# Circuitscape/Circuitscape.jl

Measured on NVIDIA H100. Metric: pair_solves_per_sec, higher is better.
Workload: dtype f64

## Files before the change

circuitscape_b200/_lib.py:

```python
from __future__ import annotations

import ctypes as C
import os

import numpy as np

_HERE = os.path.dirname(os.path.abspath(__file__))
LIB_PATH = os.path.join(_HERE, "lib", "libcsb200.so")

OK, ERR_ARG, ERR_CUDA, ERR_RESIDUAL, ERR_MAXITER, ERR_UNSUPPORTED = 0, -1, -2, -3, -4, -5
F32, F64 = 0, 1
PRECOND_JACOBI, PRECOND_AMG = 0, 1


class B200Unavailable(RuntimeError):
    pass


class B200Error(RuntimeError):
    def __init__(self, code, msg):
        super().__init__(msg)
        self.code = code


class Opts(C.Structure):
    _fields_ = [("precond", C.c_int32), ("panel_width", C.c_int32), ("check_every", C.c_int32),
                ("use_graph", C.c_int32), ("atol", C.c_double), ("resid_gate", C.c_double),
                ("log_transform", C.c_int32), ("window", C.c_int32), ("mixed", C.c_int32), ("setup", C.c_int32),
                ("stencil", C.c_int32), ("reserved", C.c_int32 * 3)]


class Stats(C.Structure):
    _fields_ = [("setup_ms", C.c_double), ("solve_ms", C.c_double), ("kernel_ms", C.c_double),
                ("iterations", C.c_int64), ("spmm_launches", C.c_int64),
                ("kernel_launches", C.c_int64), ("h2d_bytes", C.c_double), ("d2h_bytes", C.c_double)]

    def as_dict(self):
        return {k: getattr(self, k) for k, _ in self._fields_}


_H = C.c_void_p
_PROTOS = {
    "cs_b200_version": (C.c_int, []),
    "cs_b200_last_error": (C.c_char_p, [_H]),
    "cs_b200_create": (C.c_int, [C.c_int64, C.c_int64, C.c_void_p, C.c_void_p, C.c_void_p, C.c_int,
                                 C.c_int, C.c_int, C.c_int, C.POINTER(Opts), C.POINTER(_H)]),
    "cs_b200_create_from_device": (C.c_int, [C.c_int64, C.c_int64, C.c_void_p, C.c_void_p, C.c_void_p,
                                             C.c_int, C.c_int, C.POINTER(Opts), C.POINTER(_H)]),
    "cs_b200_create_from_raster": (C.c_int, [C.c_int64, C.c_int64, C.c_void_p, C.c_int, C.c_int, C.c_int, C.c_int,
                                             C.POINTER(Opts), C.POINTER(_H), C.POINTER(C.c_int64),
                                             C.POINTER(C.c_int64)]),
    "cs_b200_get_csr": (C.c_int, [_H, C.c_void_p, C.c_void_p, C.c_void_p]),
    "cs_b200_set_grounds": (C.c_int, [_H, C.c_void_p, C.c_void_p]),
    "cs_b200_level_info": (C.c_int, [_H, C.c_int, C.c_int, C.POINTER(C.c_int64), C.POINTER(C.c_int64),
                                     C.POINTER(C.c_int64), C.POINTER(C.c_double), C.POINTER(C.c_int)]),
    "cs_b200_level_csr": (C.c_int, [_H, C.c_int, C.c_int, C.c_void_p, C.c_void_p, C.c_void_p]),
    "cs_b200_level_stencil": (C.c_int, [_H, C.c_int, C.POINTER(C.c_int)]),
    "cs_b200_create_from_raster_poly": (C.c_int, [C.c_int64, C.c_int64, C.c_void_p, C.c_void_p, C.c_int, C.c_int, C.c_int,
                                                  C.c_int, C.POINTER(Opts), C.POINTER(_H), C.POINTER(C.c_int64),
                                                  C.POINTER(C.c_int64), C.c_void_p]),
    "cs_b200_get_dims": (C.c_int, [_H, C.POINTER(C.c_int64), C.POINTER(C.c_int64)]),
    "cs_b200_destroy": (None, [_H]),
    "cs_b200_spmv": (C.c_int, [_H, C.c_void_p, C.c_void_p, C.c_int, C.POINTER(C.c_double)]),
    "cs_b200_spmm": (C.c_int, [_H, C.c_int, C.c_void_p, C.c_void_p]),
    "cs_b200_apply_precond": (C.c_int, [_H, C.c_int, C.c_void_p, C.c_void_p, C.c_void_p]),
    "cs_b200_bench_spmm": (C.c_int, [_H, C.c_int, C.c_int, C.c_int, C.POINTER(C.c_double)]),
    "cs_b200_bench_cg_iter": (C.c_int, [_H, C.c_int, C.c_int, C.POINTER(C.c_double)]),
    "cs_b200_solve_rhs": (C.c_int, [_H, C.c_int64, C.c_void_p, C.c_void_p, C.c_double, C.c_int64,
                                    C.c_void_p, C.c_void_p]),
    "cs_b200_solve_pairs": (C.c_int, [_H, C.c_int64, C.c_void_p, C.c_void_p, C.c_void_p, C.c_double,
                                      C.c_int64, C.c_void_p, C.c_void_p, C.c_void_p, C.c_int,
                                      C.c_void_p, C.c_void_p]),
    "cs_b200_solve_pairs_superposed": (C.c_int, [_H, C.c_int64, C.c_void_p, C.c_int64, C.c_void_p, C.c_void_p,
                                                 C.c_void_p, C.c_double, C.c_int64, C.c_void_p, C.c_void_p,
                                                 C.c_void_p, C.c_int, C.c_void_p, C.c_void_p]),
    "cs_b200_solve_region_pairs": (C.c_int, [_H, C.c_int64, C.c_void_p, C.c_void_p, C.c_int64, C.c_void_p,
                                             C.c_void_p, C.c_void_p, C.c_double, C.c_int64, C.c_void_p,
                                             C.c_void_p, C.c_void_p, C.c_int, C.c_void_p, C.c_void_p]),
    "cs_b200_solve_grounded": (C.c_int, [_H, C.c_int64, C.c_void_p, C.c_void_p, C.c_int64, C.c_void_p,
                                         C.c_void_p, C.c_void_p, C.c_void_p, C.c_void_p, C.c_double,
                                         C.c_int64, C.c_void_p, C.c_void_p, C.c_void_p, C.c_int, C.c_void_p,
                                         C.c_void_p]),
    "cs_b200_solve_advanced": (C.c_int, [_H, C.c_int64, C.c_void_p, C.c_void_p, C.c_int64, C.c_void_p,
                                         C.c_void_p, C.c_void_p, C.c_void_p, C.c_void_p, C.c_double,
                                         C.c_int64, C.c_void_p, C.c_void_p, C.c_int, C.c_void_p, C.c_void_p]),
    "cs_b200_solve_sources": (C.c_int, [_H, C.c_int64, C.c_void_p, C.c_void_p, C.c_void_p, C.c_void_p,
                                        C.c_void_p, C.c_double, C.c_int64, C.c_int64, C.c_void_p,
                                        C.c_void_p, C.c_void_p, C.c_void_p, C.c_int, C.c_void_p,
                                        C.c_void_p]),
    "cs_b200_solve_advanced_batch": (C.c_int, [C.c_int64, C.c_int64, C.c_int64, C.c_void_p, C.c_void_p,
                                               C.c_void_p, C.c_int, C.c_int, C.c_int, C.c_double, C.c_int64,
                                               C.c_void_p, C.c_void_p, C.c_void_p, C.c_void_p,
                                               C.POINTER(C.c_int64)]),
    "cs_b200_solve_advanced_network": (C.c_int, [_H, C.c_int64, C.c_void_p, C.c_void_p, C.c_int64, C.c_void_p,
                                                 C.c_void_p, C.c_void_p, C.c_void_p, C.c_void_p, C.c_double,
                                                 C.c_int64, C.c_void_p, C.c_void_p, C.c_void_p, C.c_void_p,
                                                 C.c_void_p]),
    "cs_b200_solve_pairs_branch": (C.c_int, [_H, C.c_int64, C.c_void_p, C.c_void_p, C.c_void_p, C.c_double,
                                             C.c_int64, C.c_void_p, C.c_void_p, C.c_void_p, C.c_int, C.c_void_p,
                                             C.c_void_p, C.c_void_p]),
    "cs_b200_branch_index": (C.c_int, [_H, C.POINTER(C.c_int64), C.c_void_p, C.c_void_p]),
    "cs_b200_read_branch_currents": (C.c_int, [_H, C.c_void_p]),
    "cs_b200_components": (C.c_int, [_H, C.POINTER(C.c_int64), C.c_void_p]),
    "cs_b200_read_currents": (C.c_int, [_H, C.c_void_p, C.c_void_p]),
    "cs_b200_reset_currents": (C.c_int, [_H]),
    "cs_b200_currents_device_ptrs": (C.c_int, [_H, C.POINTER(C.c_void_p), C.POINTER(C.c_void_p)]),
    "cs_b200_get_stats": (C.c_int, [_H, C.POINTER(Stats)]),
    "cs_b200_stream": (C.c_int, [_H, C.POINTER(C.c_void_p)]),
    "cs_b200_profile_spmm": (C.c_int, [_H, C.c_int, C.POINTER(C.c_double), C.POINTER(C.c_int64)]),
    "cs_b200_profile_classes": (C.c_int, [_H, C.c_void_p, C.c_void_p, C.c_void_p]),
    "cs_b200_profile_bytes": (C.c_int, [_H, C.POINTER(C.c_double)]),
    "cs_b200_comm_unique_id": (C.c_int, [C.c_void_p]),
    "cs_b200_comm_init": (C.c_int, [C.c_int, C.c_int, C.c_int, C.c_void_p, C.POINTER(_H)]),
    "cs_b200_comm_destroy": (None, [_H]),
    "cs_b200_comm_last_error": (C.c_char_p, [_H]),
    "cs_b200_create_bcast": (C.c_int, [_H, C.c_int, C.c_int64, C.c_int64, C.c_void_p, C.c_void_p, C.c_void_p,
                                       C.c_int, C.c_int, C.c_int, C.POINTER(Opts), C.POINTER(_H)]),
    "cs_b200_comm_reduce_currents": (C.c_int, [_H, _H]),
    "cs_b200_comm_gather_pairs": (C.c_int, [_H, C.c_int64, C.c_void_p, C.c_int64, C.c_void_p, C.c_void_p]),
    "cs_b200_comm_max_double": (C.c_int, [_H, C.c_void_p, C.c_int]),
    "cs_b200_comm_barrier": (C.c_int, [_H]),
}
EXPORTED_SYMBOLS = tuple(_PROTOS)

_lib = None


def load():
    global _lib
    if _lib is not None:
        return _lib
    if not os.path.isfile(LIB_PATH):
        raise B200Unavailable(
            f"{LIB_PATH} not built -- run `python -c 'import __graft_entry__ as g; g.build()'` "
            "(the CUDA path has no CPU fallback)")
    lib = C.CDLL(LIB_PATH)
    for name, (res, args) in _PROTOS.items():
        fn = getattr(lib, name)
        fn.restype = res
        fn.argtypes = args
    _lib = lib
    return lib


def _ptr(a):
    return None if a is None else a.ctypes.data_as(C.c_void_p)


def np_dtype(dtype_code):
    return np.float64 if dtype_code == F64 else np.float32


def dtype_code(dt):
    dt = np.dtype(dt)
    if dt == np.float64:
        return F64
    if dt == np.float32:
        return F32
    raise TypeError(f"unsupported dtype {dt}")


def check(lib, h, rc, allow=()):
    if rc == OK or rc in allow:
        return rc
    msg = lib.cs_b200_last_error(h)
    msg = msg.decode() if msg else f"libcsb200 error {rc}"
    if rc == ERR_CUDA and "no CUDA device" in msg:
        raise B200Unavailable(msg)
    raise B200Error(rc, msg)
```

circuitscape_b200/csrc/cs_b200.cu:

```cuda
#include "../../include/cs_b200.h"

#include <cuda_runtime.h>
#include <cub/device/device_scan.cuh>

#include <algorithm>
#include <chrono>
#include <cmath>
#include <cstdarg>
#include <cstdio>
#include <cstdlib>
#include <cstring>
#include <limits>
#include <string>
#include <type_traits>
#include <vector>

#include "amg_host.hpp"
#include "win_host.hpp"
#include "kernels.cuh"
#include "raster_assembly.cuh"
#include "setup_device.hpp"

using namespace csb;

namespace {

thread_local std::string g_create_error;

constexpr int PROF_CLASSES = 18;
constexpr int PROF_CGF = 8;

struct GraphSlot {
  cudaGraphExec_t exec = nullptr;
  int chunk = 0;
  int64_t kernels = 0, spmms = 0;
  cudaGraphExec_t loop_exec = nullptr;
  int64_t loop_kernels = 0, loop_spmms = 0;
};

}

struct DevCsr {
  int* rowptr = nullptr;
  int* colidx = nullptr;
  void* vals = nullptr;
  int* bstart = nullptr;
  int nblocks = 0;
  int nrows = 0;
  int64_t nnz = 0;
  int lpr = 1;
  WinMeta* win_meta = nullptr;
  unsigned char* blob = nullptr;
  int has_dinv = 0;
  int64_t win_blocks = 0;
  int win_nblocks = 0;
  void* dia = nullptr;
  size_t dia_ld = 0;
  int dia_nr = 0;
  int dia_half = 0;
  int* ell_col = nullptr;
  void* ell_val = nullptr;
  size_t ell_ld = 0;
};

struct DevLevel {
  int64_t n = 0, n_pad = 0;
  DevCsr A, P, R;
  void* dinv = nullptr;
  double omega = 2.0 / 3.0;
  void *x = nullptr, *b = nullptr, *t = nullptr, *y = nullptr;
};

struct cs_b200_handle {
  int device = 0;
  int dtype = CS_B200_F64;
  int64_t n = 0, n_pad = 0, nnz = 0;
  int* d_rowptr = nullptr;
  int* d_colidx = nullptr;
  void* d_vals = nullptr;
  bool owns_matrix = true;
  void* d_vals0 = nullptr;
  void* d_fg = nullptr;
  void* d_dinv = nullptr;
  int* d_bstart = nullptr;
  int nblocks = 0;
  int ktmax = 8;
  void *X = nullptr, *R = nullptr, *P = nullptr, *AP = nullptr, *B = nullptr, *stage = nullptr;
  void* Z = nullptr;
  void* P2 = nullptr;
  DevCsr A0;
  std::vector<DevLevel> lv;
  double* d_pinv = nullptr;
  double amg_opc = 0.0;
  bool amg = false;
  bool mixed = false;
  std::vector<DevLevel> lv32;
  void *R32 = nullptr, *X32 = nullptr, *T32 = nullptr, *Z32 = nullptr;
  void *d_cum = nullptr, *d_max = nullptr;
  int* d_bptr = nullptr;
  int64_t nb = 0;
  void* d_cum_branch = nullptr;
  void* d_branch_stage = nullptr;
  PanelCtl* d_ctl = nullptr;
  PanelCtl* h_ctl = nullptr;
  double* d_partials = nullptr;
  float* d_flush = nullptr;
  size_t flush_elems = 0;
  cudaStream_t stream = nullptr;
  cudaEvent_t ev0 = nullptr, ev1 = nullptr, ev2 = nullptr, ev3 = nullptr;
  long long* d_sp_rows = nullptr;
  double* d_sp_vals = nullptr;
  int* d_sp_ptr = nullptr;
  size_t sp_cap = 0;
  long long* d_probe = nullptr;
  void* d_probe_out = nullptr;
  size_t probe_cap = 0;
  cudaStream_t s_in = nullptr, s_out = nullptr;
  void* io_in[2] = {nullptr, nullptr};
  void* io_out[2] = {nullptr, nullptr};
  cudaEvent_t ev_in[2] = {nullptr, nullptr}, ev_used[2] = {nullptr, nullptr};
  cudaEvent_t ev_ready[2] = {nullptr, nullptr}, ev_out[2] = {nullptr, nullptr};
  int num_sms = 132;
  int grid_spmm = 132, grid_ew = 132;
  cs_b200_opts opts{};
  cs_b200_stats stats{};
  GraphSlot graphs[4];
  bool rg_on = false;
  int* d_rg_seg = nullptr;
  int* d_rg_rows = nullptr;
  size_t rg_cap = 0;
  GraphSlot rgraphs[4];
  int profile = 0;
  std::vector<cudaEvent_t> prof_ev;
  size_t prof_used = 0;
  double prof_ms = 0.0;
  double prof_bytes = 0.0;
  int64_t prof_launches = 0;
  std::vector<int> prof_slot;
  std::vector<double> prof_pair_bytes;
  double prof_slot_ms[PROF_CLASSES] = {}, prof_slot_bytes[PROF_CLASSES] = {};
  int64_t prof_slot_launches[PROF_CLASSES] = {};
  std::string err;
  size_t esize() const { return dtype == CS_B200_F64 ? 8 : 4; }
};

namespace {

struct Tick {
  bool on = std::getenv("CS_B200_VERBOSE") != nullptr;
  std::chrono::steady_clock::time_point t0 = std::chrono::steady_clock::now();
  void operator()(const char* what) {
    if (!on) return;
    const auto t1 = std::chrono::steady_clock::now();
    std::fprintf(stderr, "[cs_b200 setup] %-28s %8.1f ms\n", what,
                 std::chrono::duration<double, std::milli>(t1 - t0).count());
    t0 = t1;
  }
};

int set_err(cs_b200_handle* h, int code, const char* fmt, ...) {
  char buf[1024];
  va_list ap;
  va_start(ap, fmt);
  vsnprintf(buf, sizeof buf, fmt, ap);
  va_end(ap);
  if (h) h->err = buf; else g_create_error = buf;
  return code;
}

#define CK(h, call)                                                                      \
  do {                                                                                   \
    cudaError_t _e = (call);                                                             \
    if (_e != cudaSuccess)                                                               \
      return set_err(h, CS_B200_ERR_CUDA, "CUDA error %s at %s:%d (%s)",                 \
                     cudaGetErrorString(_e), __FILE__, __LINE__, #call);                 \
  } while (0)

cudaError_t h2d(cs_b200_handle* h, void* dst, const void* src, size_t bytes) {
  if (bytes == 0) return cudaSuccess;
  cudaError_t e = cudaMemcpyAsync(dst, src, bytes, cudaMemcpyHostToDevice, h->stream);
  if (e != cudaSuccess) return e;
  return cudaStreamSynchronize(h->stream);
}

int kt_index(int kt) { return kt == 1 ? 0 : kt == 2 ? 1 : kt == 4 ? 2 : 3; }

void build_row_blocks(const std::vector<int>& rowptr, int64_t n, std::vector<int>& bstart,
                      int max_rows = NT) {
  bstart.clear();
  bstart.push_back(0);
  int64_t r = 0;
  while (r < n) {
    int64_t r1 = r + 1;
    const int64_t base = rowptr[r];
    while (r1 < n && (r1 - r) < max_rows && (int64_t)rowptr[r1 + 1] - base <= NNZ_CAP) ++r1;
    bstart.push_back((int)r1);
    r = r1;
  }
}

template <typename T>
int build_windowed(cs_b200_handle* h, DevCsr& d, const int* rowptr, const int* colidx, int64_t ncols_pad,
                   const T* d_dinv = nullptr);

int win_mask() {
  const char* e = getenv("CS_B200_WIN_MASK");
  return e ? atoi(e) : 15;
}

template <typename T>
int upload_csr(cs_b200_handle* h, const csb_amg::Csr& m, DevCsr& d, bool windowed, const T* d_dinv = nullptr) {
  d.nrows = (int)m.nrows;
  d.nnz = m.nnz();
  d.lpr = (m.nrows > 0 && (double)d.nnz / (double)m.nrows >= 20.0) ? 4 : 1;
  const int unit = d.lpr == 4 ? 8 : 32;
  int max_rows = (int)((m.nrows + 4 * h->num_sms - 1) / (4 * h->num_sms));
  max_rows = std::min(NT, std::max(unit, (max_rows + unit - 1) / unit * unit));
  std::vector<int> bstart;
  build_row_blocks(m.ptr, m.nrows, bstart, max_rows);
  d.nblocks = (int)bstart.size() - 1;
  std::vector<T> v(m.val.begin(), m.val.end());
  CK(h, cudaMalloc(&d.rowptr, (size_t)(m.nrows + 1) * sizeof(int)));
  CK(h, cudaMalloc(&d.colidx, std::max<size_t>(1, (size_t)d.nnz) * sizeof(int)));
  CK(h, cudaMalloc(&d.vals, std::max<size_t>(1, (size_t)d.nnz) * sizeof(T)));
  CK(h, cudaMalloc(&d.bstart, bstart.size() * sizeof(int)));
  CK(h, h2d(h, d.rowptr, m.ptr.data(), (size_t)(m.nrows + 1) * sizeof(int)));
  CK(h, h2d(h, d.colidx, m.idx.data(), (size_t)d.nnz * sizeof(int)));
  CK(h, h2d(h, d.vals, v.data(), (size_t)d.nnz * sizeof(T)));
  CK(h, h2d(h, d.bstart, bstart.data(), bstart.size() * sizeof(int)));
  if (h->opts.window >= 0 && windowed) {
    const int64_t ncols_pad = (m.ncols + 3) / 4 * 4;
    return build_windowed<T>(h, d, m.ptr.data(), m.idx.data(), ncols_pad, d_dinv);
  }
  return CS_B200_OK;
}

void free_win(DevCsr& d) {
  cudaFree(d.win_meta); cudaFree(d.blob); cudaFree(d.dia); cudaFree(d.ell_col); cudaFree(d.ell_val);
  d.win_meta = nullptr; d.blob = nullptr; d.dia = nullptr; d.ell_col = nullptr; d.ell_val = nullptr;
  d.dia_half = 0;
}

// ... 95 lines not shown
  tick("host hierarchy");
  h->amg_opc = hier.operator_complexity();
  const int nl = (int)hier.levels.size();
  h->mixed = nl > 1 && sizeof(T) == 8 && h->opts.mixed >= 0;
  int rc = h->mixed ? upload_levels<float>(h, hier, h->lv32, true) : CS_B200_OK;
  if (rc) return rc;
  tick("levels: windows + upload");
  if (h->mixed) {
    h->lv.resize(nl);
    for (int l = 0; l < nl; ++l) { h->lv[l].n = hier.levels[l].A.nrows; h->lv[l].omega = hier.levels[l].omega; }
    h->lv[0].A = h->A0;
    h->lv[0].dinv = h->d_dinv;
    const size_t pe = (size_t)h->n_pad * h->ktmax * sizeof(float);
    void** bufs[] = {&h->R32, &h->X32, &h->T32, &h->Z32};
    for (void** bp : bufs) {
      CK(h, cudaMalloc(bp, pe));
      CK(h, cudaMemsetAsync(*bp, 0, pe, h->stream));
    }
  } else {
    rc = upload_levels<T>(h, hier, h->lv, false);
    if (rc) return rc;
    const size_t pe = (size_t)h->n_pad * h->ktmax * sizeof(T);
    CK(h, cudaMalloc(&h->Z, pe));
    CK(h, cudaMemsetAsync(h->Z, 0, pe, h->stream));
  }
  const size_t nc = (size_t)hier.levels.back().A.nrows;
  if (hier.coarse_pinv.size() == nc * nc && nc > 0) {
    CK(h, cudaMalloc(&h->d_pinv, nc * nc * sizeof(double)));
    CK(h, h2d(h, h->d_pinv, hier.coarse_pinv.data(), nc * nc * sizeof(double)));
  }
  CK(h, cudaStreamSynchronize(h->stream));
  h->amg = nl > 1;
  return CS_B200_OK;
}

template <typename T>
int alloc_common(cs_b200_handle* h) {
  const size_t pe = (size_t)h->n_pad * h->ktmax;
  void** bufs[] = {&h->X, &h->R, &h->P, &h->AP, &h->B, &h->stage};
  const char* ve = std::getenv("CS_B200_VERBOSE");
  const bool v2 = ve && std::atoi(ve) >= 2;
  auto t0 = std::chrono::steady_clock::now();
  auto stamp = [&](const char* what) {
    if (!v2) return;
    cudaStreamSynchronize(h->stream);
    const auto t1 = std::chrono::steady_clock::now();
    std::fprintf(stderr, "[cs_b200 setup/stamp]        %-34s %8.2f ms\n", what,
                 std::chrono::duration<double, std::milli>(t1 - t0).count());
    t0 = t1;
  };
  stamp("alloc_common: entry (pending work)");
  for (void** b : bufs) {
    CK(h, cudaMalloc(b, pe * sizeof(T)));
    CK(h, cudaMemsetAsync(*b, 0, pe * sizeof(T), h->stream));
  }
  stamp("alloc_common: 6 panels");
  CK(h, cudaMalloc(&h->d_dinv, (size_t)h->n_pad * sizeof(T)));
  CK(h, cudaMalloc(&h->d_cum, (size_t)h->n_pad * sizeof(T)));
  CK(h, cudaMalloc(&h->d_max, (size_t)h->n_pad * sizeof(T)));
  CK(h, cudaMalloc(&h->d_ctl, sizeof(PanelCtl)));
  CK(h, cudaMemsetAsync(h->d_ctl, 0, sizeof(PanelCtl), h->stream));
  stamp("alloc_common: dinv/cum/max/ctl");
  CK(h, cudaMallocHost(&h->h_ctl, sizeof(PanelCtl)));
  stamp("alloc_common: cudaMallocHost");
  const int maxgrid = h->num_sms * 8;
  CK(h, cudaMalloc(&h->d_partials, (size_t)maxgrid * 2 * MAXKT * sizeof(double)));
  k_dinv<T><<<std::min<int64_t>((h->n_pad + 255) / 256, 4096), 256, 0, h->stream>>>(
      (int)h->n, (int)h->n_pad, h->d_rowptr, h->d_colidx, (const T*)h->d_vals, (T*)h->d_dinv);
  CK(h, cudaGetLastError());
  stamp("alloc_common: k_dinv");
  return CS_B200_OK;
}

template <typename T>
int finish_setup(cs_b200_handle* h, const std::vector<int>& h_rowptr, const std::vector<int>* h_colidx,
                 const T* h_vals) {
  std::vector<int> bstart;
  build_row_blocks(h_rowptr, h->n, bstart);
  h->nblocks = (int)bstart.size() - 1;
  CK(h, cudaMalloc(&h->d_bstart, bstart.size() * sizeof(int)));
  CK(h, cudaMemcpyAsync(h->d_bstart, bstart.data(), bstart.size() * sizeof(int),
                        cudaMemcpyHostToDevice, h->stream));
  h->A0 = DevCsr{h->d_rowptr, h->d_colidx, h->d_vals, h->d_bstart, h->nblocks, (int)h->n, h->nnz, 1};
  int rc0 = alloc_common<T>(h);
  if (rc0) return rc0;
  CK(h, cudaStreamSynchronize(h->stream));
  std::vector<int> ci_local;
  std::vector<T> v_local;
  const bool want_win = h->opts.window >= 0 && (h->opts.window > 0 || h->n >= 20000) && (win_mask() & 1);
  const bool want_amg = h->opts.precond == CS_B200_PRECOND_AMG;
  if (!h_colidx && (want_win || want_amg)) {
    ci_local.resize(h->nnz);
    CK(h, cudaMemcpy(ci_local.data(), h->d_colidx, (size_t)h->nnz * sizeof(int), cudaMemcpyDeviceToHost));
    h_colidx = &ci_local;
    if (want_amg) {
      v_local.resize(h->nnz);
      CK(h, cudaMemcpy(v_local.data(), h->d_vals, (size_t)h->nnz * sizeof(T), cudaMemcpyDeviceToHost));
      h_vals = v_local.data();
    }
  }
  Tick tick;
  if (want_win) {
    int rc = build_windowed<T>(h, h->A0, h_rowptr.data(), h_colidx->data(), h->n_pad, (const T*)h->d_dinv);
    if (rc) return rc;
    tick("finest operator: windows");
  }
  if (want_amg) {
    int rc = setup_amg<T>(h, h_rowptr, *h_colidx, h_vals);
    if (rc) return rc;
  }
  return cs_b200_reset_currents(h);
}

int rc_dev(cs_b200_handle* h, int rc) {
  (void)h;
  if (rc == 0) return CS_B200_OK;
  return rc == -5 ? CS_B200_ERR_UNSUPPORTED : CS_B200_ERR_CUDA;
}

int device_row_blocks(cs_b200_handle* h, DevCsr& d, int max_rows) {
  int* bs = nullptr;
  int nb = 0;
  int rc = csb_dev::row_blocks(h->stream, d.rowptr, d.nrows, max_rows, NNZ_CAP, &bs, &nb, h->err);
  if (rc) return rc_dev(h, rc);
  d.bstart = bs;
  d.nblocks = nb;
  return CS_B200_OK;
}

template <typename T>
int device_windows(cs_b200_handle* h, DevCsr& d, int64_t ncols_pad, const T* d_dinv) {
  csb_dev::DWin w;
  int rc = csb_dev::build_windowed<T>(h->stream, d.rowptr, d.colidx, (const T*)d.vals, d.nrows, ncols_pad,
                                      d.lpr == 4 ? W_WCAP_WIDE : W_WCAP, d_dinv, w, h->err);
  if (rc) return rc_dev(h, rc);
  d.has_dinv = d_dinv != nullptr ? 1 : 0;
  d.win_blocks = w.windowed_blocks;
  d.win_nblocks = w.nblocks;
  d.win_meta = reinterpret_cast<WinMeta*>(w.meta);
  d.blob = w.blob;
  return CS_B200_OK;
}

inline bool stencil_pipe() {
  static const bool off = std::getenv("CS_B200_NO_STENCIL_PIPE") != nullptr;
  return !off;
}

inline bool full_stencil() {
  static const bool on = std::getenv("CS_B200_FULL_STENCIL") != nullptr;
  return on || !stencil_pipe();
}

template <typename T>
DiaDev<T> dia_view(const DevCsr& m) {
  return DiaDev<T>{(const T*)m.dia, m.dia_ld, m.nrows, m.dia_nr, m.dia_half};
}

[[noreturn]] inline void refuse_half(const char* kernel) {
  std::fprintf(stderr, "cs_b200: %s was handed a half-form (5-slot) stencil; it reads 9 slots\n", kernel);
  std::abort();
}

template <typename T>
int device_stencil(cs_b200_handle* h, DevCsr& d) {
  static const bool env_off = std::getenv("CS_B200_NO_STENCIL") != nullptr;
  if (h->opts.stencil < 0 || env_off) return CS_B200_OK;
  if (h->opts.stencil == 0 && d.nrows < 20000) return CS_B200_OK;
  T* dia = nullptr;
  int nr = 0;
  size_t ld = 0;
  int rc = csb_dev::build_dia<T>(h->stream, d.rowptr, d.colidx, (const T*)d.vals, d.nrows, &dia, &nr, &ld, h->err);
  if (rc) return rc_dev(h, rc);
  if (dia && !full_stencil()) {
    rc = csb_dev::halve_dia<T>(h->stream, &dia, d.nrows, nr, ld, &d.dia_half, h->err);
    if (rc) { cudaFree(dia); return rc_dev(h, rc); }
  }
  d.dia = dia;
  d.dia_nr = nr;
  d.dia_ld = ld;
  return CS_B200_OK;
}

template <typename TV>
int adopt_csr(cs_b200_handle* h, csb_dev::DCsr& src, bool duplicate, DevCsr& d, bool windowed, const TV* d_dinv) {
  d.nrows = (int)src.nrows;
  d.nnz = src.nnz;
  d.lpr = (src.nrows > 0 && (double)d.nnz / (double)src.nrows >= 20.0) ? 4 : 1;
  const size_t np = (size_t)src.nrows + 1, ne = std::max<size_t>(1, (size_t)src.nnz);
  if (duplicate) {
    CK(h, cudaMalloc(&d.rowptr, np * sizeof(int)));
    CK(h, cudaMalloc(&d.colidx, ne * sizeof(int)));
    CK(h, cudaMemcpyAsync(d.rowptr, src.ptr, np * sizeof(int), cudaMemcpyDeviceToDevice, h->stream));
    CK(h, cudaMemcpyAsync(d.colidx, src.idx, (size_t)src.nnz * sizeof(int), cudaMemcpyDeviceToDevice, h->stream));
  } else {
    d.rowptr = src.ptr; src.ptr = nullptr;
    d.colidx = src.idx; src.idx = nullptr;
  }
  if (sizeof(TV) == 8 && !duplicate) {
    d.vals = src.val; src.val = nullptr;
  } else {
    CK(h, cudaMalloc(&d.vals, ne * sizeof(TV)));
    if (sizeof(TV) == 8) {
      CK(h, cudaMemcpyAsync(d.vals, src.val, (size_t)src.nnz * sizeof(double), cudaMemcpyDeviceToDevice, h->stream));
    } else if (csb_dev::convert_values(h->stream, src.val, (float*)d.vals, src.nnz)) {
      return set_err(h, CS_B200_ERR_CUDA, "value conversion launch failed");
    }
    if (!duplicate) {
      CK(h, cudaStreamSynchronize(h->stream));
      cudaFree(src.val); src.val = nullptr;
    }
  }
  const int unit = d.lpr == 4 ? 8 : 32;
  int max_rows = (int)((src.nrows + 4 * h->num_sms - 1) / (4 * h->num_sms));
  max_rows = std::min(NT, std::max(unit, (max_rows + unit - 1) / unit * unit));
  int rc = device_row_blocks(h, d, max_rows);
  if (rc) return rc;
  if (src.nrows == src.ncols && d_dinv != nullptr) {
    rc = device_stencil<TV>(h, d);
    if (rc) return rc;
    if (d.dia) return CS_B200_OK;
  }
  if (h->opts.window >= 0 && windowed) {
    const int64_t ncols_pad = (src.ncols + 3) / 4 * 4;
    return device_windows<TV>(h, d, ncols_pad, d_dinv);
  }
  return CS_B200_OK;
}

template <typename TV>
int adopt_levels(cs_b200_handle* h, csb_dev::DHierarchy& hier, std::vector<DevLevel>& lv, bool own0) {
  const int nl = (int)hier.levels.size();
  lv.resize(nl);
  Tick lt;
  auto mark = [&](int l, const char* what) {
    if (!lt.on) return;
    cudaStreamSynchronize(h->stream);
    char buf[64];
    snprintf(buf, sizeof buf, "  L%d %s", l, what);
    lt(buf);
  };
  for (int l = 0; l < nl; ++l) {
    csb_dev::DLevel& hl = hier.levels[l];
    DevLevel& L = lv[l];
    L.n = hl.A.nrows;
    L.n_pad = (L.n + 3) / 4 * 4;
    L.omega = hl.omega;
    if (l == 0 && !own0) {
      L.A = h->A0;
      L.dinv = h->d_dinv;
    } else {
      CK(h, cudaMalloc(&L.dinv, (size_t)L.n_pad * sizeof(TV)));
      CK(h, cudaMemsetAsync(L.dinv, 0, (size_t)L.n_pad * sizeof(TV), h->stream));
      if (sizeof(TV) == 8) {
        CK(h, cudaMemcpyAsync(L.dinv, hl.dinv, (size_t)L.n * sizeof(double), cudaMemcpyDeviceToDevice, h->stream));
      } else if (csb_dev::convert_values(h->stream, hl.dinv, (float*)L.dinv, L.n)) {
        return set_err(h, CS_B200_ERR_CUDA, "dinv conversion launch failed");
      }
      const bool win = h->opts.window > 0 || (L.n >= 20000 && (win_mask() & (l == 0 ? 1 : 2)));
      int rc = adopt_csr<TV>(h, hl.A, l == 0, L.A, win, (const TV*)L.dinv);
      if (rc) return rc;
      mark(l, "A: copy/convert, blocks, windows");
      if (l > 0) {
        const size_t pe = (size_t)L.n_pad * h->ktmax * sizeof(TV);
        void** bufs[] = {&L.x, &L.b, &L.t, &L.y};
        for (void** bp : bufs) {
          CK(h, cudaMalloc(bp, pe));
          CK(h, cudaMemsetAsync(*bp, 0, pe, h->stream));
        }
      }
    }
    if (l + 1 < nl) {
      int rc = adopt_csr<TV>(h, hl.P, false, L.P, L.n >= 20000 && (win_mask() & 4), (const TV*)nullptr);
      if (rc) return rc;
      if (L.A.dia) {
        int* ec = nullptr;
        TV* ev = nullptr;
        size_t eld = 0;
        int rce = csb_dev::build_ell4<TV>(h->stream, L.P.rowptr, L.P.colidx, (const TV*)L.P.vals, L.P.nrows, &ec, &ev, &eld, h->err);
        if (rce) return rc_dev(h, rce);
        L.P.ell_col = ec; L.P.ell_val = ev; L.P.ell_ld = eld;
      }
      mark(l, "P");
      rc = adopt_csr<TV>(h, hl.R, false, L.R, L.n >= 20000 && (win_mask() & 8), (const TV*)nullptr);
      if (rc) return rc;
      mark(l, "R");
    }
  }
  return CS_B200_OK;
}

template <typename T>
int setup_amg_device(cs_b200_handle* h, const csb_dev::HostPattern& hp, csb_dev::SeedJob* job,
                     const csb_dev::DeviceSeed* dseed) {
  const bool verbose = std::getenv("CS_B200_VERBOSE") != nullptr;
  csb_dev::DCsr a0;
  a0.nrows = a0.ncols = h->n;
  a0.nnz = h->nnz;
  a0.ptr = h->d_rowptr;
  a0.idx = h->d_colidx;
  double* tmp64 = nullptr;
  if (sizeof(T) == 8) {
    a0.val = (double*)h->d_vals;
  } else {
    cudaError_t e = cudaMalloc(&tmp64, std::max<size_t>(1, (size_t)h->nnz) * sizeof(double));
    if (e != cudaSuccess) {
      csb_dev::seed_discard(job);
      return set_err(h, CS_B200_ERR_CUDA, "CUDA error %s (fp64 copy of the matrix)", cudaGetErrorString(e));
    }
    csb_dev::convert_values(h->stream, (const float*)h->d_vals, tmp64, h->nnz);
    a0.val = tmp64;
  }
  Tick tick;
  csb_dev::DHierarchy hier;
  int rc = csb_dev::build_hierarchy(h->stream, a0, hp, job, dseed, 12, 200, hier, h->err, verbose);
  auto done = [&](int code) {
    cudaStreamSynchronize(h->stream);
    csb_dev::free_hierarchy(hier);
    cudaFree(tmp64);
    return code;
  };
  if (rc) return done(rc_dev(h, rc));
  tick("device hierarchy");
  h->amg_opc = hier.operator_complexity;
  const int nl = (int)hier.levels.size();
  h->mixed = nl > 1 && sizeof(T) == 8 && h->opts.mixed >= 0;
  if (h->mixed) {
    rc = adopt_levels<float>(h, hier, h->lv32, true);
    if (rc) return done(rc);
    h->lv.resize(nl);
    for (int l = 0; l < nl; ++l) { h->lv[l].n = hier.levels[l].A.nrows; h->lv[l].omega = hier.levels[l].omega; }
    h->lv[0].A = h->A0;
    h->lv[0].dinv = h->d_dinv;
    const size_t pe = (size_t)h->n_pad * h->ktmax * sizeof(float);
    void** bufs[] = {&h->R32, &h->X32, &h->T32, &h->Z32};
    for (void** bp : bufs) {
      cudaError_t e = cudaMalloc(bp, pe);
      if (e == cudaSuccess) e = cudaMemsetAsync(*bp, 0, pe, h->stream);
      if (e != cudaSuccess) return done(set_err(h, CS_B200_ERR_CUDA, "CUDA error %s (fp32 panels)", cudaGetErrorString(e)));
    }
  } else {
    rc = adopt_levels<T>(h, hier, h->lv, false);
    if (rc) return done(rc);
    const size_t pe = (size_t)h->n_pad * h->ktmax * sizeof(T);
    cudaError_t e = cudaMalloc(&h->Z, pe);
    if (e == cudaSuccess) e = cudaMemsetAsync(h->Z, 0, pe, h->stream);
    if (e != cudaSuccess) return done(set_err(h, CS_B200_ERR_CUDA, "CUDA error %s (Z panel)", cudaGetErrorString(e)));
  }
  tick("levels: row blocks + windows");
  csb_dev::coarse_pinv_wait(hier);
  tick("coarse pseudo-inverse (wait)");
  const size_t nc = (size_t)hier.levels.back().A.nrows;
  if (hier.coarse_pinv.size() == nc * nc && nc > 0) {
    cudaError_t e = cudaMalloc(&h->d_pinv, nc * nc * sizeof(double));
    if (e == cudaSuccess) e = h2d(h, h->d_pinv, hier.coarse_pinv.data(), nc * nc * sizeof(double));
    if (e != cudaSuccess) return done(set_err(h, CS_B200_ERR_CUDA, "CUDA error %s (coarse pseudo-inverse)", cudaGetErrorString(e)));
  }
  h->amg = nl > 1;
  return done(CS_B200_OK);
}

template <typename T>
int build_operators(cs_b200_handle* h, const csb_dev::HostPattern& hp, csb_dev::SeedJob* job,
                    const csb_dev::DeviceSeed* dseed);

template <typename T>
int finish_setup_device(cs_b200_handle* h, const csb_dev::HostPattern& hp, csb_dev::SeedJob* job,
                        const csb_dev::DeviceSeed* dseed = nullptr) {
  h->A0 = DevCsr{h->d_rowptr, h->d_colidx, h->d_vals, nullptr, 0, (int)h->n, h->nnz, 1};
  Tick tick0;
  int rc = device_row_blocks(h, h->A0, NT);
  if (rc) { csb_dev::seed_discard(job); return rc; }
  h->d_bstart = h->A0.bstart;
  h->nblocks = h->A0.nblocks;
  rc = alloc_common<T>(h);
  if (rc) { csb_dev::seed_discard(job); return rc; }
  if (tick0.on) { cudaStreamSynchronize(h->stream); tick0("row blocks + panels"); }
  rc = build_operators<T>(h, hp, job, dseed);
  if (rc) return rc;
  return cs_b200_reset_currents(h);
}

template <typename T>
int build_operators(cs_b200_handle* h, const csb_dev::HostPattern& hp, csb_dev::SeedJob* job,
                    const csb_dev::DeviceSeed* dseed) {
  int rc = CS_B200_OK;
  k_dinv<T><<<std::min<int64_t>((h->n_pad + 255) / 256, 4096), 256, 0, h->stream>>>(
      (int)h->n, (int)h->n_pad, h->d_rowptr, h->d_colidx, (const T*)h->d_vals, (T*)h->d_dinv);
  const bool want_win = h->opts.window >= 0 && (h->opts.window > 0 || h->n >= 20000) && (win_mask() & 1);
  const bool want_amg = h->opts.precond == CS_B200_PRECOND_AMG;
  Tick tick;
  if (want_win || h->opts.stencil > 0) {
    rc = device_stencil<T>(h, h->A0);
    if (!rc && !h->A0.dia && want_win) rc = device_windows<T>(h, h->A0, h->n_pad, (const T*)h->d_dinv);
    if (rc) { csb_dev::seed_discard(job); return rc; }
    tick(h->A0.dia ? "finest operator: stencil form" : "finest operator: windows");
  }
  if (want_amg) {
    rc = setup_amg_device<T>(h, hp, job, dseed);
    if (rc) return rc;
    if (h->amg && h->A0.dia && !h->P2) {
      const size_t pe = (size_t)h->n_pad * h->ktmax * sizeof(T);
      cudaError_t e = cudaMalloc(&h->P2, pe);
      if (e == cudaSuccess) e = cudaMemsetAsync(h->P2, 0, pe, h->stream);
      if (e != cudaSuccess) return set_err(h, CS_B200_ERR_CUDA, "CUDA error %s (second p panel)", cudaGetErrorString(e));
    }
  } else {
    csb_dev::seed_discard(job);
  }
  Tick tick1;
  csb_dev::trim_pool(h->device);
  tick1("scratch pool released");
  return CS_B200_OK;
}

int common_create(cs_b200_handle* h, const cs_b200_opts* opts) {
  if (opts) h->opts = *opts;
  if (h->opts.panel_width == 0) h->opts.panel_width = 8;
  if (h->opts.check_every <= 0) h->opts.check_every = 16;
  if (h->opts.resid_gate <= 0) h->opts.resid_gate = 1e-4;
  if (h->opts.use_graph == 0) h->opts.use_graph = 1;
  const int pw = h->opts.panel_width;
  if (pw != 1 && pw != 2 && pw != 4 && pw != 8)
    return set_err(h, CS_B200_ERR_ARG, "panel_width must be 1, 2, 4 or 8 (got %d)", pw);
  h->ktmax = pw;
  if (h->opts.precond != CS_B200_PRECOND_JACOBI && h->opts.precond != CS_B200_PRECOND_AMG)
    return set_err(h, CS_B200_ERR_UNSUPPORTED, "unknown preconditioner %d", h->opts.precond);
  int ndev = 0;
  cudaError_t e = cudaGetDeviceCount(&ndev);
  if (e != cudaSuccess || ndev == 0)
    return set_err(h, CS_B200_ERR_CUDA,
                   "no CUDA device available (%s): libcsb200 has no CPU fallback",
                   cudaGetErrorString(e));
  if (h->device < 0 || h->device >= ndev)
    return set_err(h, CS_B200_ERR_ARG, "device %d out of range (0..%d)", h->device, ndev - 1);
  CK(h, cudaSetDevice(h->device));
  cudaDeviceProp prop;
  CK(h, cudaGetDeviceProperties(&prop, h->device));
  h->num_sms = prop.multiProcessorCount;
  h->grid_spmm = h->num_sms * 8;
  h->grid_ew = h->num_sms * 4;
  CK(h, cudaStreamCreateWithFlags(&h->stream, cudaStreamNonBlocking));
  CK(h, cudaEventCreate(&h->ev0));
  CK(h, cudaEventCreate(&h->ev1));
  CK(h, cudaEventCreate(&h->ev2));
  CK(h, cudaEventCreate(&h->ev3));
  h->n_pad = (h->n + 3) / 4 * 4;
  return CS_B200_OK;
}

template <typename I>
void narrow_indices(const I* src, int64_t count, int base, std::vector<int>& dst) {
  dst.resize(count);
  for (int64_t i = 0; i < count; ++i) dst[i] = (int)(src[i] - base);
}

template <typename T>
CsrDev<T> view(const DevCsr& m) {
  return CsrDev<T>{m.rowptr, m.colidx, (const T*)m.vals, m.bstart, m.nblocks, m.nrows};
}

template <typename T, int KT, int MODE, bool HALF>
void launch_stencil_pipe(cs_b200_handle* h, const DiaDev<T>& a, const T* X, T* Y, const SpmmEpi<T>& ep, int sg) {
  constexpr int SMEM = StPipe<T, KT, MODE, HALF>::D::BYTES;
  static bool once[64] = {};
  bool& set = once[h->device & 63];
  if (!set) { cudaFuncSetAttribute(k_stencil_pipe<T, KT, MODE, HALF>, cudaFuncAttributeMaxDynamicSharedMemorySize, SMEM); set = true; }
  k_stencil_pipe<T, KT, MODE, HALF><<<sg, NT, SMEM, h->stream>>>(a, X, Y, ep);
}

template <typename T, int KT, int MODE>
void launch_stencil(cs_b200_handle* h, const DiaDev<T>& a, const T* X, T* Y, const SpmmEpi<T>& ep, int sg) {
  if (!stencil_pipe()) {
    if (a.half) refuse_half("k_stencil");
    k_stencil<T, KT, MODE><<<sg, NT, 0, h->stream>>>(a, X, Y, ep);
    return;
  }
  if (a.half) launch_stencil_pipe<T, KT, MODE, true>(h, a, X, Y, ep, sg);
  else launch_stencil_pipe<T, KT, MODE, false>(h, a, X, Y, ep, sg);
}

template <typename T, int KT, int MODE>
void launch_spmm_on(cs_b200_handle* h, const DevCsr& m, const T* X, T* Y, const T* B, const T* dinv,
                    double omega, bool timed) {
  const int grid = std::max(1, std::min(h->grid_spmm, m.nblocks));
  cudaEvent_t e0 = nullptr, e1 = nullptr;
  const bool prof = h->profile && timed;
  if (prof) {
    if (h->prof_used + 2 > h->prof_ev.size()) {
      for (int i = 0; i < 2; ++i) { cudaEvent_t e; cudaEventCreate(&e); h->prof_ev.push_back(e); }
    }
    e0 = h->prof_ev[h->prof_used++];
    e1 = h->prof_ev[h->prof_used++];
    double bytes = (double)m.nnz * (sizeof(T) + 4) + (double)(m.nrows + 1) * 4 +
                   2.0 * (double)m.nrows * KT * sizeof(T);
    if (MODE == SP_RESNORM || MODE == SP_RES || MODE == SP_JACOBI || MODE == SP_JACOBI_DOT)
      bytes += (double)m.nrows * KT * sizeof(T);
    if (MODE == SP_JACOBI || MODE == SP_JACOBI_DOT) bytes += (double)m.nrows * sizeof(T);
    h->prof_bytes += bytes;
    h->prof_slot.push_back(2 * MODE + (sizeof(T) == 4 ? 1 : 0));
    h->prof_pair_bytes.push_back(bytes);
    cudaEventRecord(e0, h->stream);
  }
  const SpmmEpi<T> ep{B, dinv, (T)omega, h->d_ctl, h->d_partials};
  if (m.dia && MODE != SP_ADD) {
    if constexpr (MODE != SP_ADD) {
      const DiaDev<T> a = dia_view<T>(m);
      constexpr int V16 = 16 / (int)sizeof(T);
      constexpr int CGn = KT / (KT < V16 ? KT : V16);
      const int rpp = NT / CGn;
      const long long ntiles = (long long)((m.dia_nr + rpp - 1) / rpp) *
                               ((((long long)m.nrows + m.dia_nr - 1) / m.dia_nr + ST_TC - 1) / ST_TC);
      const int sg = (int)std::max<long long>(1, std::min<long long>(h->grid_spmm, ntiles));
      launch_stencil<T, KT, MODE>(h, a, X, Y, ep, sg);
    }
  } else if (m.win_meta) {
    const WinCsr<T> w{m.win_meta, m.blob, m.has_dinv, m.rowptr, m.colidx, (const T*)m.vals, m.win_nblocks};
    if (m.lpr == 4) {
      constexpr int SMEM = WinSmem2<T, KT, MODE, true>::TOTAL;
      constexpr int SB = WinMap<T, KT, true>::SB;
      const int wg = std::max(1, std::min(h->num_sms, (m.win_nblocks + SB - 1) / SB));
      static bool once[64] = {};
      bool& set = once[h->device & 63];
      if (!set) { cudaFuncSetAttribute(k_spmm_win<T, KT, MODE, true>, cudaFuncAttributeMaxDynamicSharedMemorySize, SMEM); set = true; }
      k_spmm_win<T, KT, MODE, true><<<wg, WTT, SMEM, h->stream>>>(w, X, Y, ep);
    } else {
      constexpr int SMEM = WinSmem2<T, KT, MODE, false>::TOTAL;
      constexpr int SB = WinMap<T, KT, false>::SB;
      const int wg = std::max(1, std::min(h->num_sms, (m.win_nblocks + SB - 1) / SB));
      static bool once[64] = {};
      bool& set = once[h->device & 63];
      if (!set) { cudaFuncSetAttribute(k_spmm_win<T, KT, MODE, false>, cudaFuncAttributeMaxDynamicSharedMemorySize, SMEM); set = true; }
      k_spmm_win<T, KT, MODE, false><<<wg, WTT, SMEM, h->stream>>>(w, X, Y, ep);
    }
  } else if (m.lpr == 4 && KT * 4 <= 32) {
    k_spmm<T, KT, MODE, (KT * 4 <= 32 ? 4 : 1)><<<grid, NT, 0, h->stream>>>(view<T>(m), X, Y, ep);
  } else {
    k_spmm<T, KT, MODE, 1><<<grid, NT, 0, h->stream>>>(view<T>(m), X, Y, ep);
  }
  if (prof) cudaEventRecord(e1, h->stream);
  h->stats.kernel_launches++;
  if (timed) h->stats.spmm_launches++;
}

template <typename T, int KT, int MODE>
void launch_spmm(cs_b200_handle* h, const T* X, T* Y, const T* B) {
  launch_spmm_on<T, KT, MODE>(h, h->A0, X, Y, B, (const T*)h->d_dinv, 0.0, true);
}

void harvest_profile(cs_b200_handle* h) {
  for (size_t i = 0; i + 1 < h->prof_used; i += 2) {
    float ms = 0;
    if (cudaEventElapsedTime(&ms, h->prof_ev[i], h->prof_ev[i + 1]) == cudaSuccess) {
      h->prof_ms += ms;
      h->prof_launches++;
      if (i / 2 < h->prof_slot.size()) {
        const int sl = h->prof_slot[i / 2];
        h->prof_slot_ms[sl] += ms;
        h->prof_slot_bytes[sl] += h->prof_pair_bytes[i / 2];
        h->prof_slot_launches[sl]++;
      }
    }
  }
  h->prof_used = 0;
  h->prof_slot.clear();
  h->prof_pair_bytes.clear();
}

template <typename T, int KT>
int ew_grid(cs_b200_handle* h) {
  const size_t nelem = (size_t)h->n_pad * KT;
  const size_t per = (size_t)NT * Vec<T>::N;
  return (int)std::min<size_t>(h->grid_ew, (nelem + per - 1) / per);
}

template <typename T, int KT>
int ew_grid_n(cs_b200_handle* h, int64_t n_pad) {
  const size_t nelem = (size_t)n_pad * KT;
  const size_t per = (size_t)NT * Vec<T>::N;
  return (int)std::max<size_t>(1, std::min<size_t>(h->grid_ew, (nelem + per - 1) / per));
}

inline bool implicit_x0(const DevLevel& L) {
  static const bool off = std::getenv("CS_B200_NO_IMPLICIT_X0") != nullptr || std::getenv("CS_B200_NO_FUSED_PROLONG") != nullptr;
  return L.A.dia != nullptr && !off;
}

template <typename T, int KT>
void launch_stencil_res0(cs_b200_handle* h, DevLevel& L, const T* B, T* Tout, bool timed) {
  const DevCsr& m = L.A;
  const DiaDev<T> a = dia_view<T>(m);
  const SpmmEpi<T> ep{B, (const T*)L.dinv, (T)L.omega, h->d_ctl, h->d_partials};
  constexpr int V16 = 16 / (int)sizeof(T);
  constexpr int CGn = KT / (KT < V16 ? KT : V16);
  const int rpp = NT / CGn;
  const long long ntiles = (long long)((m.dia_nr + rpp - 1) / rpp) *
                           ((((long long)m.nrows + m.dia_nr - 1) / m.dia_nr + ST_TC - 1) / ST_TC);
  const int sg = (int)std::max<long long>(1, std::min<long long>(h->grid_spmm, ntiles));
  cudaEvent_t e0 = nullptr, e1 = nullptr;
  const bool prof = h->profile && timed;
  if (prof) {
    if (h->prof_used + 2 > h->prof_ev.size())
      for (int i = 0; i < 2; ++i) { cudaEvent_t e; cudaEventCreate(&e); h->prof_ev.push_back(e); }
    e0 = h->prof_ev[h->prof_used++];
    e1 = h->prof_ev[h->prof_used++];
    const double fb = (double)m.nnz * (sizeof(T) + 4) + (double)(m.nrows + 1) * 4 + 3.0 * (double)m.nrows * KT * sizeof(T);
    h->prof_bytes += fb;
    h->prof_slot.push_back(2 * (int)SP_RES + (sizeof(T) == 4 ? 1 : 0));
    h->prof_pair_bytes.push_back(fb);
    cudaEventRecord(e0, h->stream);
  }
  launch_stencil<T, KT, SP_RES0>(h, a, nullptr, Tout, ep, sg);
  if (prof) cudaEventRecord(e1, h->stream);
  h->stats.kernel_launches++;
  if (timed) h->stats.spmm_launches++;
}

template <typename T, int KT, int MODE>
void launch_prolong_jacobi(cs_b200_handle* h, DevLevel& L, const T* Yc, const T* X0, T* Yout, const T* B, bool timed) {
  const DevCsr& m = L.A;
  const DiaDev<T> a = dia_view<T>(m);
  const CsrP<T> p{L.P.rowptr, L.P.colidx, (const T*)L.P.vals, L.P.ell_col, (const T*)L.P.ell_val, L.P.ell_ld};
  const SpmmEpi<T> ep{B, (const T*)L.dinv, (T)L.omega, h->d_ctl, h->d_partials};
  using S = PjShape<T, KT>;
  constexpr int SMEM = S::SMEM;
  constexpr int MINB = sizeof(T) == 4 ? PJ_MINB_F32 : PJ_MINB_F64;
  static_assert(SMEM <= 48 * 1024, "the strip buffers fit the default dynamic shared memory");
  int occ = 0;
  cudaOccupancyMaxActiveBlocksPerMultiprocessor(&occ, k_stencil_prolong_jacobi<T, KT, MODE, MINB>, NT, SMEM);
  occ = std::max(1, occ);
  const long long nsteps = (long long)((m.dia_nr + S::RPS - 1) / S::RPS) *
                           (((long long)m.nrows + m.dia_nr - 1) / m.dia_nr);
  const int grid = (int)std::max<long long>(1, std::min<long long>(std::min(h->grid_spmm, h->num_sms * occ), nsteps));
  cudaEvent_t e0 = nullptr, e1 = nullptr;
  const bool prof = h->profile && timed;
  if (prof) {
    if (h->prof_used + 2 > h->prof_ev.size())
      for (int i = 0; i < 2; ++i) { cudaEvent_t e; cudaEventCreate(&e); h->prof_ev.push_back(e); }
    e0 = h->prof_ev[h->prof_used++];
    e1 = h->prof_ev[h->prof_used++];
    const double fb = (double)m.nnz * (sizeof(T) + 4) + (double)(m.nrows + 1) * 4 + 3.0 * (double)m.nrows * KT * sizeof(T) +
                      (double)m.nrows * sizeof(T) + (double)L.P.nnz * (sizeof(T) + 4) + (double)(m.nrows + 1) * 4 +
                      2.0 * (double)m.nrows * KT * sizeof(T);
    h->prof_bytes += fb;
    h->prof_slot.push_back(2 * 7 + (sizeof(T) == 4 ? 1 : 0));
    h->prof_pair_bytes.push_back(fb);
    cudaEventRecord(e0, h->stream);
  }
  k_stencil_prolong_jacobi<T, KT, MODE, MINB><<<grid, NT, SMEM, h->stream>>>(a, p, Yc, X0, Yout, ep);
  if (prof) cudaEventRecord(e1, h->stream);
  h->stats.kernel_launches++;
  if (timed) h->stats.spmm_launches++;
}

struct VcBufs { void *b0, *x0, *t0, *y0; };

template <typename T, int KT>
void launch_vcycle_on(cs_b200_handle* h, std::vector<DevLevel>& lv, const VcBufs& vb, bool level0_presmoothed) {
  const int nl = (int)lv.size();
  auto B = [&](int l) { return l == 0 ? (T*)vb.b0 : (T*)lv[l].b; };
  auto X = [&](int l) { return l == 0 ? (T*)vb.x0 : (T*)lv[l].x; };
  auto Tm = [&](int l) { return l == 0 ? (T*)vb.t0 : (T*)lv[l].t; };
  auto Y = [&](int l) { return l == 0 ? (T*)vb.y0 : (T*)lv[l].y; };
  for (int l = 0; l < nl - 1; ++l) {
    DevLevel& L = lv[l];
    const size_t nelem = (size_t)L.n_pad * KT;
    if (implicit_x0(L)) {
      launch_stencil_res0<T, KT>(h, L, B(l), Tm(l), l == 0);
    } else {
      if (!(l == 0 && level0_presmoothed)) {
        k_jacobi0<T, KT><<<ew_grid_n<T, KT>(h, L.n_pad), NT, 0, h->stream>>>(
            nelem, B(l), (const T*)L.dinv, (T)L.omega, X(l));
        h->stats.kernel_launches++;
      }
      launch_spmm_on<T, KT, SP_RES>(h, L.A, X(l), Tm(l), B(l), nullptr, 0.0, l == 0);
    }
    launch_spmm_on<T, KT, SP_PLAIN>(h, L.R, Tm(l), B(l + 1), nullptr, nullptr, 0.0, false);
  }
  {
    DevLevel& C = lv[nl - 1];
    if (h->d_pinv) {
      k_coarse_dense<T, KT><<<((int)C.n * KT + NT - 1) / NT, NT, 0, h->stream>>>((int)C.n, h->d_pinv, (const T*)B(nl - 1), Y(nl - 1));
      h->stats.kernel_launches++;
    } else {
      const int l = nl - 1;
      k_jacobi0<T, KT><<<ew_grid_n<T, KT>(h, C.n_pad), NT, 0, h->stream>>>(
          (size_t)C.n_pad * KT, B(l), (const T*)C.dinv, (T)C.omega, X(l));
      h->stats.kernel_launches++;
      launch_spmm_on<T, KT, SP_JACOBI>(h, C.A, X(l), Y(l), B(l), (const T*)C.dinv, C.omega, false);
      launch_spmm_on<T, KT, SP_JACOBI>(h, C.A, Y(l), X(l), B(l), (const T*)C.dinv, C.omega, false);
      launch_spmm_on<T, KT, SP_JACOBI>(h, C.A, X(l), Y(l), B(l), (const T*)C.dinv, C.omega, false);
    }
  }
  static const bool fuse_off = std::getenv("CS_B200_NO_FUSED_PROLONG") != nullptr;
  for (int l = nl - 2; l >= 0; --l) {
    DevLevel& L = lv[l];
    if (L.A.dia && !fuse_off) {
      const T* x0 = implicit_x0(L) ? nullptr : X(l);
      if (l == 0) launch_prolong_jacobi<T, KT, SP_JACOBI_DOT>(h, L, Y(l + 1), x0, Y(l), B(l), true);
      else launch_prolong_jacobi<T, KT, SP_JACOBI>(h, L, Y(l + 1), x0, Y(l), B(l), false);
      continue;
    }
    launch_spmm_on<T, KT, SP_ADD>(h, L.P, Y(l + 1), X(l), X(l) , nullptr, 0.0, false);
    if (l == 0)
      launch_spmm_on<T, KT, SP_JACOBI_DOT>(h, L.A, X(l), Y(l), B(l), (const T*)L.dinv, L.omega, true);
    else
      launch_spmm_on<T, KT, SP_JACOBI>(h, L.A, X(l), Y(l), B(l), (const T*)L.dinv, L.omega, false);
  }
}

template <typename T, int KT>
void launch_vcycle(cs_b200_handle* h, bool level0_presmoothed) {
  if (h->mixed) {
    const VcBufs vb{h->R32, h->X32, h->T32, h->Z32};
    launch_vcycle_on<float, KT>(h, h->lv32, vb, level0_presmoothed);
  } else {
    const VcBufs vb{h->R, h->stage, h->AP, h->Z};
    launch_vcycle_on<T, KT>(h, h->lv, vb, level0_presmoothed);
  }
}

template <typename T, int KT>
void launch_seg_set(cs_b200_handle* h, void* panel, int set_b_only, T v) {
  k_seg_set<T, KT><<<2 * KT, NT, 0, h->stream>>>((T*)panel, h->d_rg_seg, h->d_rg_rows, set_b_only, v);
  h->stats.kernel_launches++;
}

template <typename T, int KT>
void mask_z(cs_b200_handle* h) {
  if (!h->rg_on) return;
  if (h->mixed) launch_seg_set<float, KT>(h, h->Z32, 0, 0.0f);
  else launch_seg_set<T, KT>(h, h->Z, 0, T(0));
}

inline GraphSlot& graph_slot(cs_b200_handle* h, int kt) {
  return (h->rg_on ? h->rgraphs : h->graphs)[kt_index(kt)];
}

void drop_graphs(GraphSlot* slots) {
  for (int i = 0; i < 4; ++i) {
    if (slots[i].exec) cudaGraphExecDestroy(slots[i].exec);
    if (slots[i].loop_exec) cudaGraphExecDestroy(slots[i].loop_exec);
    slots[i] = GraphSlot{};
  }
}

inline bool fused_cg(const cs_b200_handle* h) {
  static const bool off = std::getenv("CS_B200_NO_FUSED_CG") != nullptr;
  return h->amg && h->A0.dia && h->P2 && !off;
}

template <typename T, int KT, typename TV, bool HALF>
void launch_stencil_cg_pipe(cs_b200_handle* h, const DiaDev<T>& a, const TV* Z, int sg) {
  constexpr int SMEM = StPipeCg<T, KT, TV, HALF>::D::BYTES;
  static bool once[64] = {};
  bool& set = once[h->device & 63];
  if (!set) { cudaFuncSetAttribute(k_stencil_cg_pipe<T, KT, TV, HALF>, cudaFuncAttributeMaxDynamicSharedMemorySize, SMEM); set = true; }
  k_stencil_cg_pipe<T, KT, TV, HALF><<<sg, NT, SMEM, h->stream>>>(a, Z, (T*)h->P2, (T*)h->P, (T*)h->X, (T*)h->AP,
                                                                  h->d_ctl, h->d_partials);
}

template <typename T, int KT, typename TV>
void launch_stencil_cg(cs_b200_handle* h, const TV* Z) {
  const DevCsr& m = h->A0;
  const DiaDev<T> a = dia_view<T>(m);
  constexpr int V16 = 16 / (int)sizeof(T);
  constexpr int CGn = KT / (KT < V16 ? KT : V16);
  const int rpp = NT / CGn;
  const long long ntiles = (long long)((m.dia_nr + rpp - 1) / rpp) *
                           ((((long long)m.nrows + m.dia_nr - 1) / m.dia_nr + ST_TC - 1) / ST_TC);
  const int sg = (int)std::max<long long>(1, std::min<long long>(h->grid_spmm, ntiles));
  cudaEvent_t e0 = nullptr, e1 = nullptr;
  if (h->profile) {
    if (h->prof_used + 2 > h->prof_ev.size())
      for (int i = 0; i < 2; ++i) { cudaEvent_t e; cudaEventCreate(&e); h->prof_ev.push_back(e); }
    e0 = h->prof_ev[h->prof_used++];
    e1 = h->prof_ev[h->prof_used++];
    const double pe = (double)m.nrows * KT * sizeof(T);
    const double fb = (double)m.nrows * 9 * sizeof(T) + (double)m.nrows * KT * sizeof(TV) + 3.0 * pe + 1.5 * pe;
    h->prof_bytes += fb;
    h->prof_slot.push_back(2 * PROF_CGF + (sizeof(T) == 4 ? 1 : 0));
    h->prof_pair_bytes.push_back(fb);
    cudaEventRecord(e0, h->stream);
  }
  if (stencil_pipe()) {
    if (a.half) launch_stencil_cg_pipe<T, KT, TV, true>(h, a, Z, sg);
    else launch_stencil_cg_pipe<T, KT, TV, false>(h, a, Z, sg);
  } else {
    if (a.half) refuse_half("k_stencil_cg");
    k_stencil_cg<T, KT, TV><<<sg, NT, 0, h->stream>>>(a, Z, (T*)h->P2, (T*)h->P, (T*)h->X, (T*)h->AP, h->d_ctl,
                                                       h->d_partials);
  }
  if (h->profile) cudaEventRecord(e1, h->stream);
  h->stats.kernel_launches++;
  h->stats.spmm_launches++;
}

template <typename T, int KT>
void launch_iteration(cs_b200_handle* h) {
  const size_t nelem = (size_t)h->n_pad * KT;
  const int g = ew_grid<T, KT>(h);
  const bool fused = fused_cg(h);
  if (fused) {
    if (h->mixed) launch_stencil_cg<T, KT, float>(h, (const float*)h->Z32);
    else launch_stencil_cg<T, KT, T>(h, (const T*)h->Z);
  } else {
    launch_spmm<T, KT, SP_CG>(h, (const T*)h->P, (T*)h->AP, nullptr);
  }
  if (h->rg_on) launch_seg_set<T, KT>(h, h->AP, 0, T(0));
  if (!h->amg) {
    k_cg_update_r<T, KT><<<g, NT, 0, h->stream>>>(nelem, (const T*)h->AP, (const T*)h->d_dinv,
                                                  (T*)h->R, h->d_ctl, h->d_partials);
    k_cg_update_xp<T, KT><<<g, NT, 0, h->stream>>>(nelem, (const T*)h->R, (const T*)h->d_dinv,
                                                   (T*)h->X, (T*)h->P, h->d_ctl);
    h->stats.kernel_launches += 2;
  } else {
    if (h->mixed) {
      k_cg_update_r0<T, KT, float><<<g, NT, 0, h->stream>>>(nelem, (const T*)h->AP, (const T*)h->d_dinv,
                                                            (T)h->lv[0].omega, (T*)h->R,
                                                            implicit_x0(h->lv32[0]) ? nullptr : (float*)h->X32,
                                                            (float*)h->R32, h->d_ctl);
      launch_vcycle<T, KT>(h, true);
      mask_z<T, KT>(h);
      if (!fused)
        k_cg_update_xp2<T, KT, float><<<g, NT, 0, h->stream>>>(nelem, (const float*)h->Z32, (T*)h->X, (T*)h->P,
                                                               h->d_ctl);
    } else {
      k_cg_update_r0<T, KT, T><<<g, NT, 0, h->stream>>>(nelem, (const T*)h->AP, (const T*)h->d_dinv,
                                                        (T)h->lv[0].omega, (T*)h->R,
                                                        implicit_x0(h->lv[0]) ? nullptr : (T*)h->stage, nullptr,
                                                        h->d_ctl);
      launch_vcycle<T, KT>(h, true);
      mask_z<T, KT>(h);
      if (!fused)
        k_cg_update_xp2<T, KT, T><<<g, NT, 0, h->stream>>>(nelem, (const T*)h->Z, (T*)h->X, (T*)h->P, h->d_ctl);
    }
    h->stats.kernel_launches += fused ? 1 : 2;
  }
}

template <typename T, int KT>
void finish_x(cs_b200_handle* h) {
  if (!fused_cg(h)) return;
  k_cg_x_tail<T, KT><<<ew_grid<T, KT>(h), NT, 0, h->stream>>>((size_t)h->n_pad * KT, (const T*)h->P2, (const T*)h->P,
                                                             (T*)h->X, h->d_ctl);
  h->stats.kernel_launches++;
}

template <typename T, int KT>
int run_chunk(cs_b200_handle* h, int chunk) {
  GraphSlot& gs = graph_slot(h, KT);
  if (h->opts.use_graph > 0 && !h->profile) {
    if (!gs.exec || gs.chunk != chunk) {
      if (gs.exec) cudaGraphExecDestroy(gs.exec);
      gs.exec = nullptr;
      cudaGraph_t graph;
      const int64_t kl = h->stats.kernel_launches, sl = h->stats.spmm_launches;
      CK(h, cudaStreamBeginCapture(h->stream, cudaStreamCaptureModeThreadLocal));
      for (int i = 0; i < chunk; ++i) launch_iteration<T, KT>(h);
      CK(h, cudaStreamEndCapture(h->stream, &graph));
      gs.kernels = h->stats.kernel_launches - kl;
      gs.spmms = h->stats.spmm_launches - sl;
      h->stats.kernel_launches = kl;
      h->stats.spmm_launches = sl;
      CK(h, cudaGraphInstantiate(&gs.exec, graph, 0));
      cudaGraphDestroy(graph);
      gs.chunk = chunk;
    }
    CK(h, cudaGraphLaunch(gs.exec, h->stream));
    h->stats.kernel_launches += gs.kernels;
    h->stats.spmm_launches += gs.spmms;
  } else {
    for (int i = 0; i < chunk; ++i) launch_iteration<T, KT>(h);
    CK(h, cudaGetLastError());
  }
  return CS_B200_OK;
}

template <typename T, int KT>
int run_loop(cs_b200_handle* h) {
  GraphSlot& gs = graph_slot(h, KT);
  if (!gs.loop_exec) {
    cudaGraph_t graph;
    CK(h, cudaGraphCreate(&graph, 0));
    cudaGraphConditionalHandle cond;
    CK(h, cudaGraphConditionalHandleCreate(&cond, graph, 0, cudaGraphCondAssignDefault));
    cudaGraphNode_t n_pre, n_while;
    PanelCtl* ctl = h->d_ctl;
    void* args[] = {&cond, &ctl};
    cudaKernelNodeParams kp = {};
    kp.func = (void*)k_loop_cond;
    kp.gridDim = dim3(1);
    kp.blockDim = dim3(1);
    kp.kernelParams = args;
    CK(h, cudaGraphAddKernelNode(&n_pre, graph, nullptr, 0, &kp));
    cudaGraphNodeParams cp = {cudaGraphNodeTypeConditional};
    cp.conditional.handle = cond;
    cp.conditional.type = cudaGraphCondTypeWhile;
    cp.conditional.size = 1;
    CK(h, cudaGraphAddNode(&n_while, graph, &n_pre, 1, &cp));
    cudaGraph_t body = cp.conditional.phGraph_out[0];
    const int64_t kl = h->stats.kernel_launches, sl = h->stats.spmm_launches;
    CK(h, cudaStreamBeginCaptureToGraph(h->stream, body, nullptr, nullptr, 0, cudaStreamCaptureModeThreadLocal));
    launch_iteration<T, KT>(h);
    k_loop_cond<<<1, 1, 0, h->stream>>>(cond, h->d_ctl);
    CK(h, cudaStreamEndCapture(h->stream, nullptr));
    gs.loop_kernels = h->stats.kernel_launches - kl + 1;
    gs.loop_spmms = h->stats.spmm_launches - sl;
    h->stats.kernel_launches = kl;
    h->stats.spmm_launches = sl;
    CK(h, cudaGraphInstantiate(&gs.loop_exec, graph, 0));
    cudaGraphDestroy(graph);
  }
  CK(h, cudaGraphLaunch(gs.loop_exec, h->stream));
  return CS_B200_OK;
}

template <typename T, int KT>
int solve_panel(cs_b200_handle* h, double rtol, int64_t itmax) {
  const size_t nelem = (size_t)h->n_pad * KT;
  const double atol = h->opts.atol > 0 ? h->opts.atol
                      : h->opts.atol < 0 ? 0.0
                      : std::sqrt(std::numeric_limits<double>::epsilon());
  const int g = ew_grid<T, KT>(h);
  const int imax = (int)std::min<int64_t>(itmax, std::numeric_limits<int>::max() - 1);
  CK(h, cudaEventRecord(h->ev2, h->stream));
  if (!h->amg) {
    k_set_stall<<<1, 1, 0, h->stream>>>(h->d_ctl, 2000);
    k_cg_init<T, KT><<<g, NT, 0, h->stream>>>(nelem, (const T*)h->B, (const T*)h->d_dinv, (T*)h->X,
                                              (T*)h->R, (T*)h->P, h->d_ctl, h->d_partials, rtol, atol,
                                              imax);
    h->stats.kernel_launches++;
  } else {
    const bool fused = fused_cg(h);
    CK(h, cudaMemsetAsync(h->X, 0, nelem * sizeof(T), h->stream));
    CK(h, cudaMemsetAsync(h->P, 0, nelem * sizeof(T), h->stream));
    CK(h, cudaMemcpyAsync(h->R, h->B, nelem * sizeof(T), cudaMemcpyDeviceToDevice, h->stream));
    k_set_ctl<<<1, 1, 0, h->stream>>>(h->d_ctl, rtol, atol, imax, 40);
    if (h->mixed) {
      k_convert<T, float><<<g, NT, 0, h->stream>>>(nelem, (const T*)h->R, (float*)h->R32);
      launch_vcycle<T, KT>(h, false);
      mask_z<T, KT>(h);
      if (!fused)
        k_cg_update_xp2<T, KT, float><<<g, NT, 0, h->stream>>>(nelem, (const float*)h->Z32, (T*)h->X, (T*)h->P,
                                                               h->d_ctl);
      h->stats.kernel_launches++;
    } else {
      launch_vcycle<T, KT>(h, false);
      mask_z<T, KT>(h);
      if (!fused)
        k_cg_update_xp2<T, KT, T><<<g, NT, 0, h->stream>>>(nelem, (const T*)h->Z, (T*)h->X, (T*)h->P, h->d_ctl);
    }
    h->stats.kernel_launches += fused ? 1 : 2;
  }
  CK(h, cudaGetLastError());
  const int chunk = h->amg ? std::min(h->opts.check_every, 4) : h->opts.check_every;
  const bool device_loop = h->opts.use_graph == 1 && !h->profile;
  if (device_loop) {
    int rc = run_loop<T, KT>(h);
    if (rc) return rc;
  }
  for (;;) {
    CK(h, cudaMemcpyAsync(h->h_ctl, h->d_ctl, sizeof(PanelCtl), cudaMemcpyDeviceToHost, h->stream));
    CK(h, cudaStreamSynchronize(h->stream));
    if (h->profile) harvest_profile(h);
    if (device_loop) {
      GraphSlot& gs = graph_slot(h, KT);
      h->stats.kernel_launches += 1 + gs.loop_kernels * h->h_ctl->iter;
      h->stats.spmm_launches += gs.loop_spmms * h->h_ctl->iter;
      break;
    }
    if (h->h_ctl->nactive == 0) break;
    int rc = run_chunk<T, KT>(h, chunk);
    if (rc) return rc;
  }
  if (h->amg) finish_x<T, KT>(h);
  if (h->rg_on) {
    launch_spmm<T, KT, SP_RES>(h, (const T*)h->X, (T*)h->AP, (const T*)h->B);
    launch_seg_set<T, KT>(h, h->AP, 0, T(0));
    k_resnorm<T, KT><<<g, NT, 0, h->stream>>>(nelem, (size_t)h->n * KT, (const T*)h->AP, (const T*)h->B, h->d_ctl, h->d_partials);
    h->stats.kernel_launches++;
  } else {
    launch_spmm<T, KT, 2>(h, (const T*)h->X, (T*)h->AP, (const T*)h->B);
  }
  CK(h, cudaGetLastError());
  CK(h, cudaEventRecord(h->ev3, h->stream));
  CK(h, cudaMemcpyAsync(h->h_ctl, h->d_ctl, sizeof(PanelCtl), cudaMemcpyDeviceToHost, h->stream));
  CK(h, cudaStreamSynchronize(h->stream));
  if (h->profile) harvest_profile(h);
  float ms = 0;
// ... 1075 lines not shown
  cudaSetDevice(h->device);
  CK(h, cudaStreamSynchronize(h->stream));
  if (rowptr) CK(h, cudaMemcpy(rowptr, h->d_rowptr, (size_t)(h->n + 1) * sizeof(int), cudaMemcpyDeviceToHost));
  if (colidx) CK(h, cudaMemcpy(colidx, h->d_colidx, (size_t)h->nnz * sizeof(int), cudaMemcpyDeviceToHost));
  if (vals) CK(h, cudaMemcpy(vals, h->d_vals, (size_t)h->nnz * h->esize(), cudaMemcpyDeviceToHost));
  return CS_B200_OK;
}

static const DevCsr* pick_level(cs_b200_handle* h, int level, int which, bool* is_f32, double* omega,
                                int64_t* ncols) {
  if (!h || level < 0 || which < 0 || which > 2) return nullptr;
  std::vector<DevLevel>& lv = h->mixed ? h->lv32 : h->lv;
  if (lv.empty() && level == 0 && which == 0) {
    *is_f32 = h->dtype == CS_B200_F32;
    *omega = 0.0;
    *ncols = h->n;
    return &h->A0;
  }
  if (level >= (int)lv.size()) return nullptr;
  if (which > 0 && level + 1 >= (int)lv.size()) return nullptr;
  *is_f32 = h->mixed || h->dtype == CS_B200_F32;
  *omega = lv[level].omega;
  const DevCsr* m = which == 0 ? &lv[level].A : which == 1 ? &lv[level].P : &lv[level].R;
  *ncols = which == 0 ? lv[level].n : which == 1 ? lv[level + 1].n : lv[level].n;
  if (which == 2) *ncols = lv[level].n;
  return m;
}

int cs_b200_level_info(cs_b200_handle* h, int level, int which, int64_t* nrows, int64_t* ncols,
                       int64_t* nnz, double* omega, int* windowed) {
  bool f32 = false;
  double om = 0.0;
  int64_t nc = 0;
  const DevCsr* m = pick_level(h, level, which, &f32, &om, &nc);
  if (!m) return CS_B200_ERR_ARG;
  if (nrows) *nrows = m->nrows;
  if (ncols) *ncols = nc;
  if (nnz) *nnz = m->nnz;
  if (omega) *omega = om;
  if (windowed) *windowed = m->dia ? 2 : (m->win_meta ? 1 : 0);
  return CS_B200_OK;
}

int cs_b200_level_stencil(cs_b200_handle* h, int level, int* slots) {
  bool f32 = false;
  double om = 0.0;
  int64_t nc = 0;
  const DevCsr* m = pick_level(h, level, 0, &f32, &om, &nc);
  if (!m || !slots) return CS_B200_ERR_ARG;
  *slots = !m->dia ? 0 : m->dia_half ? 5 : 9;
  return CS_B200_OK;
}

int cs_b200_level_csr(cs_b200_handle* h, int level, int which, int32_t* rowptr, int32_t* colidx,
                      double* vals) {
  bool f32 = false;
  double om = 0.0;
  int64_t nc = 0;
  const DevCsr* m = pick_level(h, level, which, &f32, &om, &nc);
  if (!m) return CS_B200_ERR_ARG;
  cudaSetDevice(h->device);
  CK(h, cudaStreamSynchronize(h->stream));
  if (rowptr) CK(h, cudaMemcpy(rowptr, m->rowptr, (size_t)(m->nrows + 1) * sizeof(int), cudaMemcpyDeviceToHost));
  if (colidx) CK(h, cudaMemcpy(colidx, m->colidx, (size_t)m->nnz * sizeof(int), cudaMemcpyDeviceToHost));
  if (vals) {
    if (f32) {
      std::vector<float> tmp((size_t)m->nnz);
      CK(h, cudaMemcpy(tmp.data(), m->vals, (size_t)m->nnz * sizeof(float), cudaMemcpyDeviceToHost));
      for (int64_t i = 0; i < m->nnz; ++i) vals[i] = (double)tmp[i];
    } else {
      CK(h, cudaMemcpy(vals, m->vals, (size_t)m->nnz * sizeof(double), cudaMemcpyDeviceToHost));
    }
  }
  return CS_B200_OK;
}

int cs_b200_set_grounds(cs_b200_handle* h, const void* finite_g, const uint8_t* dirichlet) {
  if (!h) return CS_B200_ERR_ARG;
  if (h->opts.setup == 1)
    return set_err(h, CS_B200_ERR_UNSUPPORTED, "cs_b200_set_grounds needs the device-side setup (opts.setup != 1)");
  if (!h->owns_matrix)
    return set_err(h, CS_B200_ERR_UNSUPPORTED, "cs_b200_set_grounds: the handle borrows its matrix (create_from_device)");
  cudaSetDevice(h->device);
  h->err.clear();
  const size_t es = h->esize();
  const size_t vb = std::max<size_t>(1, (size_t)h->nnz) * es;
  cudaEventRecord(h->ev0, h->stream);
  cudaFree(h->d_fg);
  h->d_fg = nullptr;
  if (!h->d_vals0) {
    CK(h, cudaMalloc(&h->d_vals0, vb));
    CK(h, cudaMemcpyAsync(h->d_vals0, h->d_vals, vb, cudaMemcpyDeviceToDevice, h->stream));
  } else {
    CK(h, cudaMemcpyAsync(h->d_vals, h->d_vals0, vb, cudaMemcpyDeviceToDevice, h->stream));
  }
  void* d_g = nullptr;
  unsigned char* d_m = nullptr;
  auto cleanup = [&]() { cudaFree(d_g); cudaFree(d_m); };
  if (finite_g) {
    cudaError_t e = cudaMalloc(&d_g, (size_t)h->n * es);
    if (e == cudaSuccess) e = h2d(h, d_g, finite_g, (size_t)h->n * es);
    if (e != cudaSuccess) { cleanup(); return set_err(h, CS_B200_ERR_CUDA, "CUDA error %s (finite grounds)", cudaGetErrorString(e)); }
  }
  if (dirichlet) {
    cudaError_t e = cudaMalloc(&d_m, (size_t)h->n);
    if (e == cudaSuccess) e = h2d(h, d_m, dirichlet, (size_t)h->n);
    if (e != cudaSuccess) { cleanup(); return set_err(h, CS_B200_ERR_CUDA, "CUDA error %s (Dirichlet mask)", cudaGetErrorString(e)); }
  }
  if (finite_g || dirichlet) {
    const int g = (int)std::min<int64_t>((h->n + 255) / 256, (int64_t)h->num_sms * 32);
    if (h->dtype == CS_B200_F64)
      k_apply_grounds<double><<<g, 256, 0, h->stream>>>((int)h->n, h->d_rowptr, h->d_colidx, (double*)h->d_vals,
                                                        (const double*)d_g, d_m);
    else
      k_apply_grounds<float><<<g, 256, 0, h->stream>>>((int)h->n, h->d_rowptr, h->d_colidx, (float*)h->d_vals,
                                                       (const float*)d_g, d_m);
  }
  cudaError_t e = cudaGetLastError();
  if (e == cudaSuccess) e = cudaStreamSynchronize(h->stream);
  if (e == cudaSuccess) {
    h->d_fg = d_g;
    d_g = nullptr;
  }
  cleanup();
  if (e != cudaSuccess) return set_err(h, CS_B200_ERR_CUDA, "CUDA error %s applying the grounds", cudaGetErrorString(e));
  teardown_operators(h);
  const csb_dev::HostPattern none{};
  int rc = h->dtype == CS_B200_F64 ? build_operators<double>(h, none, nullptr, nullptr)
                                   : build_operators<float>(h, none, nullptr, nullptr);
  if (rc) return rc;
  cudaEventRecord(h->ev1, h->stream);
  cudaEventSynchronize(h->ev1);
  float ms = 0;
  cudaEventElapsedTime(&ms, h->ev0, h->ev1);
  h->stats.setup_ms = ms;
  return CS_B200_OK;
}

int cs_b200_get_dims(const cs_b200_handle* h, int64_t* n, int64_t* nnz) {
  if (!h) return CS_B200_ERR_ARG;
  if (n) *n = h->n;
  if (nnz) *nnz = h->nnz;
  return CS_B200_OK;
}

void cs_b200_destroy(cs_b200_handle* h) {
  if (!h) return;
  cudaSetDevice(h->device);
  teardown_operators(h);
  if (h->owns_matrix) { cudaFree(h->d_rowptr); cudaFree(h->d_colidx); cudaFree(h->d_vals); }
  cudaFree(h->d_vals0);
  cudaFree(h->d_fg);
  cudaFree(h->d_bptr); cudaFree(h->d_cum_branch); cudaFree(h->d_branch_stage);
  void* bufs[] = {h->d_dinv, h->d_bstart, h->X, h->R, h->P, h->P2, h->AP, h->B, h->stage,
                  h->d_cum, h->d_max, h->d_ctl, h->d_partials, h->d_flush};
  for (void* b : bufs) if (b) cudaFree(b);
  if (h->h_ctl) cudaFreeHost(h->h_ctl);
  cudaFree(h->d_sp_rows); cudaFree(h->d_sp_vals); cudaFree(h->d_sp_ptr);
  cudaFree(h->d_probe); cudaFree(h->d_probe_out);
  cudaFree(h->d_rg_seg); cudaFree(h->d_rg_rows);
  for (int i = 0; i < 2; ++i) {
    cudaFree(h->io_in[i]); cudaFree(h->io_out[i]);
    cudaEvent_t evs[] = {h->ev_in[i], h->ev_used[i], h->ev_ready[i], h->ev_out[i]};
    for (cudaEvent_t e : evs) if (e) cudaEventDestroy(e);
  }
  if (h->s_in) cudaStreamDestroy(h->s_in);
  if (h->s_out) cudaStreamDestroy(h->s_out);
  for (cudaEvent_t e : h->prof_ev) cudaEventDestroy(e);
  if (h->ev0) cudaEventDestroy(h->ev0);
  if (h->ev1) cudaEventDestroy(h->ev1);
  if (h->ev2) cudaEventDestroy(h->ev2);
  if (h->ev3) cudaEventDestroy(h->ev3);
  if (h->stream) cudaStreamDestroy(h->stream);
  delete h;
}

int cs_b200_reset_currents(cs_b200_handle* h) {
  if (!h) return CS_B200_ERR_ARG;
  cudaSetDevice(h->device);
  CK(h, cudaMemsetAsync(h->d_cum, 0, (size_t)h->n_pad * h->esize(), h->stream));
  const int g = (int)std::min<int64_t>(4096, (h->n_pad + 255) / 256);
  if (h->dtype == CS_B200_F64)
    k_fill<double><<<g, 256, 0, h->stream>>>((double*)h->d_max, (size_t)h->n_pad, -9999.0);
  else
    k_fill<float><<<g, 256, 0, h->stream>>>((float*)h->d_max, (size_t)h->n_pad, -9999.0f);
  if (h->d_cum_branch)
    CK(h, cudaMemsetAsync(h->d_cum_branch, 0, (size_t)std::max<int64_t>(h->nb, 1) * h->esize(), h->stream));
  CK(h, cudaGetLastError());
  CK(h, cudaStreamSynchronize(h->stream));
  return CS_B200_OK;
}

int cs_b200_read_currents(cs_b200_handle* h, void* cum, void* max) {
  if (!h) return CS_B200_ERR_ARG;
  cudaSetDevice(h->device);
  if (cum) CK(h, cudaMemcpyAsync(cum, h->d_cum, (size_t)h->n * h->esize(), cudaMemcpyDeviceToHost, h->stream));
  if (max) CK(h, cudaMemcpyAsync(max, h->d_max, (size_t)h->n * h->esize(), cudaMemcpyDeviceToHost, h->stream));
  CK(h, cudaStreamSynchronize(h->stream));
  return CS_B200_OK;
}

int cs_b200_read_branch_currents(cs_b200_handle* h, void* cum_branch) {
  if (!h || !cum_branch) return set_err(h, CS_B200_ERR_ARG, "bad read_branch_currents arguments");
  cudaSetDevice(h->device);
  if (int rc = ensure_branch_index(h)) return rc;
  const size_t bytes = (size_t)h->nb * h->esize();
  if (h->d_cum_branch)
    CK(h, cudaMemcpyAsync(cum_branch, h->d_cum_branch, bytes, cudaMemcpyDeviceToHost, h->stream));
  else
    std::memset(cum_branch, 0, bytes);
  CK(h, cudaStreamSynchronize(h->stream));
  return CS_B200_OK;
}

int cs_b200_branch_index(cs_b200_handle* h, int64_t* nb, int64_t* lo, int64_t* hi) {
  if (!h || !nb) return set_err(h, CS_B200_ERR_ARG, "bad branch_index arguments");
  cudaSetDevice(h->device);
  if (int rc = ensure_branch_index(h)) return rc;
  *nb = h->nb;
  if ((!lo && !hi) || h->nb == 0) return CS_B200_OK;
  DevScratch ends;
  CK(h, cudaMalloc(&ends.p, (size_t)h->nb * 2 * sizeof(long long)));
  long long* d_lo = (long long*)ends.p;
  long long* d_hi = d_lo + h->nb;
  const int g = (int)std::min<int64_t>((h->n + 255) / 256, (int64_t)h->num_sms * 32);
  k_branch_ends<<<g, 256, 0, h->stream>>>((int)h->n, h->d_rowptr, h->d_colidx, h->d_bptr, d_lo, d_hi);
  CK(h, cudaGetLastError());
  if (lo) CK(h, cudaMemcpyAsync(lo, d_lo, (size_t)h->nb * sizeof(int64_t), cudaMemcpyDeviceToHost, h->stream));
  if (hi) CK(h, cudaMemcpyAsync(hi, d_hi, (size_t)h->nb * sizeof(int64_t), cudaMemcpyDeviceToHost, h->stream));
  CK(h, cudaStreamSynchronize(h->stream));
  return CS_B200_OK;
}

int cs_b200_components(cs_b200_handle* h, int64_t* ncomp, int32_t* comp_of) {
  if (!h || !ncomp) return set_err(h, CS_B200_ERR_ARG, "bad components arguments");
  cudaSetDevice(h->device);
  h->err.clear();
  const int n = (int)h->n;
  *ncomp = 0;
  if (n == 0) return CS_B200_OK;
  size_t tb = 0;
  CK(h, cub::DeviceScan::ExclusiveSum(nullptr, tb, (const int*)nullptr, (int*)nullptr, n, h->stream));
  const size_t ib = (size_t)n * sizeof(int), ia = (ib + 255) & ~(size_t)255;
  const size_t off_root = ia, off_idx = 2 * ia, off_lab = 3 * ia, off_tmp = 4 * ia;
  char* s = nullptr;
  CK(h, cudaMallocAsync((void**)&s, off_tmp + std::max<size_t>(tb, 1), h->stream));
  int* parent = (int*)s;
  int* root = (int*)(s + off_root);
  int* idx = (int*)(s + off_idx);
  int* lab = (int*)(s + off_lab);
  const int g = (int)std::min<int64_t>((h->n + 255) / 256, (int64_t)h->num_sms * 32);
  constexpr int CHUNK = 16;
  const int ge = (int)std::max<int64_t>(1, std::min<int64_t>((h->nnz / CHUNK + 255) / 256, (int64_t)h->num_sms * 32));
  const void* vals = h->d_vals0 ? h->d_vals0 : h->d_vals;
  k_cc_init<<<g, 256, 0, h->stream>>>(n, parent);
  if (h->dtype == CS_B200_F64)
    k_cc_hook<double><<<ge, 256, 0, h->stream>>>(n, (int)h->nnz, h->d_rowptr, h->d_colidx, (const double*)vals,
                                                 parent, CHUNK);
  else
    k_cc_hook<float><<<ge, 256, 0, h->stream>>>(n, (int)h->nnz, h->d_rowptr, h->d_colidx, (const float*)vals,
                                                parent, CHUNK);
  k_cc_compress<<<g, 256, 0, h->stream>>>(n, parent, lab, root);
  cudaError_t e = cub::DeviceScan::ExclusiveSum(s + off_tmp, tb, root, idx, n, h->stream);
  int total = 0, last_flag = 0;
  if (e == cudaSuccess) {
    if (comp_of) k_cc_label<<<g, 256, 0, h->stream>>>(n, lab, idx);
    e = cudaGetLastError();
  }
  if (e == cudaSuccess) e = cudaMemcpyAsync(&total, idx + n - 1, sizeof(int), cudaMemcpyDeviceToHost, h->stream);
  if (e == cudaSuccess) e = cudaMemcpyAsync(&last_flag, root + n - 1, sizeof(int), cudaMemcpyDeviceToHost, h->stream);
  if (e == cudaSuccess && comp_of) e = cudaMemcpyAsync(comp_of, lab, ib, cudaMemcpyDeviceToHost, h->stream);
  cudaFreeAsync(s, h->stream);
  if (e == cudaSuccess) e = cudaStreamSynchronize(h->stream);
  if (e != cudaSuccess) return set_err(h, CS_B200_ERR_CUDA, "CUDA error %s (components)", cudaGetErrorString(e));
  h->stats.kernel_launches += comp_of ? 5 : 4;
  *ncomp = (int64_t)total + last_flag;
  return CS_B200_OK;
}

int cs_b200_currents_device_ptrs(cs_b200_handle* h, void** d_cum, void** d_max) {
  if (!h) return CS_B200_ERR_ARG;
  if (d_cum) *d_cum = h->d_cum;
  if (d_max) *d_max = h->d_max;
  return CS_B200_OK;
}

int cs_b200_stream(cs_b200_handle* h, void** stream) {
  if (!h || !stream) return CS_B200_ERR_ARG;
  *stream = (void*)h->stream;
  return CS_B200_OK;
}

int cs_b200_profile_spmm(cs_b200_handle* h, int enable, double* total_ms, int64_t* launches) {
  if (!h) return CS_B200_ERR_ARG;
  if (total_ms) *total_ms = h->prof_ms;
  if (launches) *launches = h->prof_launches;
  if (enable >= 0) {
    h->profile = enable ? 1 : 0;
    h->prof_ms = 0.0;
    h->prof_launches = 0;
    h->prof_used = 0;
    h->prof_bytes = 0.0;
    h->prof_slot.clear();
    h->prof_pair_bytes.clear();
    for (int i = 0; i < PROF_CLASSES; ++i) { h->prof_slot_ms[i] = 0.0; h->prof_slot_bytes[i] = 0.0; h->prof_slot_launches[i] = 0; }
  }
  return CS_B200_OK;
}

int cs_b200_profile_classes(cs_b200_handle* h, double* ms18, double* bytes18, int64_t* launches18) {
  if (!h) return CS_B200_ERR_ARG;
  for (int i = 0; i < PROF_CLASSES; ++i) {
    if (ms18) ms18[i] = h->prof_slot_ms[i];
    if (bytes18) bytes18[i] = h->prof_slot_bytes[i];
    if (launches18) launches18[i] = h->prof_slot_launches[i];
  }
  return CS_B200_OK;
}

int cs_b200_profile_bytes(cs_b200_handle* h, double* algorithmic_bytes) {
  if (!h || !algorithmic_bytes) return CS_B200_ERR_ARG;
  *algorithmic_bytes = h->prof_bytes;
  return CS_B200_OK;
}

int cs_b200_get_stats(const cs_b200_handle* h, cs_b200_stats* out) {
  if (!h || !out) return CS_B200_ERR_ARG;
  *out = h->stats;
  return CS_B200_OK;
}

int cs_b200_spmv(cs_b200_handle* h, const void* x, void* y, int reps, double* ms_per_rep) {
  if (!h || !x || !y || reps < 1) return set_err(h, CS_B200_ERR_ARG, "bad spmv arguments");
  begin_call(h);
  const size_t bytes = (size_t)h->n * h->esize();
  CK(h, cudaMemcpyAsync(h->X, x, bytes, cudaMemcpyHostToDevice, h->stream));
  CK(h, cudaEventRecord(h->ev2, h->stream));
  for (int r = 0; r < reps; ++r) {
    if (h->dtype == CS_B200_F64)
      launch_spmm<double, 1, 0>(h, (const double*)h->X, (double*)h->AP, nullptr);
    else
      launch_spmm<float, 1, 0>(h, (const float*)h->X, (float*)h->AP, nullptr);
  }
  CK(h, cudaGetLastError());
  CK(h, cudaEventRecord(h->ev3, h->stream));
  CK(h, cudaMemcpyAsync(y, h->AP, bytes, cudaMemcpyDeviceToHost, h->stream));
  CK(h, cudaStreamSynchronize(h->stream));
  float ms = 0;
  CK(h, cudaEventElapsedTime(&ms, h->ev2, h->ev3));
  if (ms_per_rep) *ms_per_rep = ms / reps;
  h->stats.kernel_ms = ms;
  h->stats.h2d_bytes = h->stats.d2h_bytes = (double)bytes;
  end_call(h);
  return CS_B200_OK;
}

int cs_b200_spmm(cs_b200_handle* h, int k, const void* x, void* y) {
  const bool add = getenv("CS_B200_SPMM_ADD") != nullptr;
  if (!h || !x || !y || (k != 1 && k != 2 && k != 4 && k != 8) || k > h->ktmax)
    return set_err(h, CS_B200_ERR_ARG, "bad spmm arguments");
  begin_call(h);
  const size_t bytes = (size_t)h->n * k * h->esize();
  const size_t nelem = (size_t)h->n_pad * k;
  const int tg = (int)std::min<size_t>(4096, (nelem + 255) / 256);
  CK(h, cudaMemcpyAsync(h->stage, x, bytes, cudaMemcpyHostToDevice, h->stream));
  CK(h, cudaMemsetAsync(h->X, 0, nelem * h->esize(), h->stream));
  const bool f64 = h->dtype == CS_B200_F64;
  if (f64) { DISPATCH_KT(k, (k_cm_to_panel<double, KT><<<tg, 256, 0, h->stream>>>((int)h->n, (size_t)h->n, (const double*)h->stage, (double*)h->X, KT))); }
  else { DISPATCH_KT(k, (k_cm_to_panel<float, KT><<<tg, 256, 0, h->stream>>>((int)h->n, (size_t)h->n, (const float*)h->stage, (float*)h->X, KT))); }
  if (add) {
    CK(h, cudaMemcpyAsync(h->AP, h->X, nelem * h->esize(), cudaMemcpyDeviceToDevice, h->stream));
    if (f64) { DISPATCH_KT(k, (launch_spmm<double, KT, SP_ADD>(h, (const double*)h->X, (double*)h->AP, (const double*)h->AP))); }
    else { DISPATCH_KT(k, (launch_spmm<float, KT, SP_ADD>(h, (const float*)h->X, (float*)h->AP, (const float*)h->AP))); }
  } else {
  if (f64) { DISPATCH_KT(k, (launch_spmm<double, KT, SP_PLAIN>(h, (const double*)h->X, (double*)h->AP, nullptr))); }
  else { DISPATCH_KT(k, (launch_spmm<float, KT, SP_PLAIN>(h, (const float*)h->X, (float*)h->AP, nullptr))); }
  }
  if (f64) { DISPATCH_KT(k, (k_panel_to_cm<double, KT><<<tg, 256, 0, h->stream>>>((int)h->n, (size_t)h->n, (const double*)h->AP, (double*)h->stage, h->d_ctl, 0))); }
  else { DISPATCH_KT(k, (k_panel_to_cm<float, KT><<<tg, 256, 0, h->stream>>>((int)h->n, (size_t)h->n, (const float*)h->AP, (float*)h->stage, h->d_ctl, 0))); }
  CK(h, cudaGetLastError());
  CK(h, cudaMemcpyAsync(y, h->stage, bytes, cudaMemcpyDeviceToHost, h->stream));
  CK(h, cudaStreamSynchronize(h->stream));
  end_call(h);
  return CS_B200_OK;
}

int cs_b200_apply_precond(cs_b200_handle* h, int k, const void* r, void* z, double* rz) {
  if (!h || !r || !z || (k != 1 && k != 2 && k != 4 && k != 8) || k > h->ktmax)
    return set_err(h, CS_B200_ERR_ARG, "bad apply_precond arguments");
  if (!h->amg) return set_err(h, CS_B200_ERR_UNSUPPORTED, "apply_precond: the handle has no multigrid preconditioner");
  begin_call(h);
  int rc = CS_B200_OK;
  if (h->dtype == CS_B200_F64) { DISPATCH_KT(k, (rc = apply_precond_t<double, KT>(h, r, z, rz))); }
  else { DISPATCH_KT(k, (rc = apply_precond_t<float, KT>(h, r, z, rz))); }
  end_call(h);
  return rc;
}

int cs_b200_bench_spmm(cs_b200_handle* h, int k, int reps, int flush_l2, double* ms_per_rep) {
  if (!h || reps < 1 || (k != 1 && k != 2 && k != 4 && k != 8) || k > h->ktmax)
    return set_err(h, CS_B200_ERR_ARG, "bad bench_spmm arguments");
  begin_call(h);
  if (flush_l2) { int rc = ensure_flush(h); if (rc) return rc; }
  const size_t pe = (size_t)h->n_pad * k;
  const int g = (int)std::min<size_t>(4096, (pe + 255) / 256);
  if (h->dtype == CS_B200_F64) k_fill<double><<<g, 256, 0, h->stream>>>((double*)h->X, pe, 1.0);
  else k_fill<float><<<g, 256, 0, h->stream>>>((float*)h->X, pe, 1.0f);
  double total = 0;
  auto one = [&]() {
    if (h->dtype == CS_B200_F64) { DISPATCH_KT(k, (launch_spmm<double, KT, 0>(h, (const double*)h->X, (double*)h->AP, nullptr))); }
    else { DISPATCH_KT(k, (launch_spmm<float, KT, 0>(h, (const float*)h->X, (float*)h->AP, nullptr))); }
  };
  one();
  if (flush_l2) {
    for (int r = 0; r < reps; ++r) {
      k_flush<<<h->num_sms * 8, 256, 0, h->stream>>>(h->d_flush, h->flush_elems);
      CK(h, cudaEventRecord(h->ev2, h->stream));
      one();
      CK(h, cudaEventRecord(h->ev3, h->stream));
      CK(h, cudaEventSynchronize(h->ev3));
      float ms = 0;
      CK(h, cudaEventElapsedTime(&ms, h->ev2, h->ev3));
      total += ms;
    }
  } else {
    CK(h, cudaEventRecord(h->ev2, h->stream));
    for (int r = 0; r < reps; ++r) one();
    CK(h, cudaEventRecord(h->ev3, h->stream));
    CK(h, cudaEventSynchronize(h->ev3));
    float ms = 0;
    CK(h, cudaEventElapsedTime(&ms, h->ev2, h->ev3));
    total = ms;
  }
  CK(h, cudaGetLastError());
  if (ms_per_rep) *ms_per_rep = total / reps;
  h->stats.kernel_ms = total;
  end_call(h);
  return CS_B200_OK;
}

int cs_b200_bench_cg_iter(cs_b200_handle* h, int k, int reps, double* ms_per_rep) {
  if (!h || reps < 1 || (k != 1 && k != 2 && k != 4 && k != 8) || k > h->ktmax)
    return set_err(h, CS_B200_ERR_ARG, "bad bench_cg_iter arguments");
  begin_call(h);
  PanelCtl* hc = h->h_ctl;
  std::memset(hc, 0, sizeof(PanelCtl));
  for (int c = 0; c < k; ++c) {
    hc->src[c] = (c * 7919) % h->n;
    hc->dst[c] = h->n - 1 - (c * 104729) % (h->n / 2 + 1);
    if (hc->dst[c] == hc->src[c]) hc->dst[c] = (hc->src[c] + 1) % h->n;
    hc->weight[c] = 1.0;
  }
  CK(h, cudaMemcpyAsync(h->d_ctl, hc, sizeof(PanelCtl), cudaMemcpyHostToDevice, h->stream));
  const size_t nelem = (size_t)h->n_pad * k;
  CK(h, cudaMemsetAsync(h->B, 0, nelem * h->esize(), h->stream));
  const bool f64 = h->dtype == CS_B200_F64;
#define BOTH(CALLD, CALLF) do { if (f64) { DISPATCH_KT(k, CALLD); } else { DISPATCH_KT(k, CALLF); } } while (0)
  BOTH((k_pair_rhs<double, KT><<<1, 32, 0, h->stream>>>((double*)h->B, h->d_ctl)),
       (k_pair_rhs<float, KT><<<1, 32, 0, h->stream>>>((float*)h->B, h->d_ctl)));
  BOTH((k_cg_init<double, KT><<<ew_grid<double, KT>(h), NT, 0, h->stream>>>(nelem, (const double*)h->B, (const double*)h->d_dinv, (double*)h->X, (double*)h->R, (double*)h->P, h->d_ctl, h->d_partials, 0.0, 0.0, 1 << 30)),
       (k_cg_init<float, KT><<<ew_grid<float, KT>(h), NT, 0, h->stream>>>(nelem, (const float*)h->B, (const float*)h->d_dinv, (float*)h->X, (float*)h->R, (float*)h->P, h->d_ctl, h->d_partials, 0.0, 0.0, 1 << 30)));
  for (int w = 0; w < 3; ++w) BOTH((launch_iteration<double, KT>(h)), (launch_iteration<float, KT>(h)));
  CK(h, cudaEventRecord(h->ev2, h->stream));
  for (int r = 0; r < reps; ++r) BOTH((launch_iteration<double, KT>(h)), (launch_iteration<float, KT>(h)));
  CK(h, cudaEventRecord(h->ev3, h->stream));
  CK(h, cudaEventSynchronize(h->ev3));
  CK(h, cudaGetLastError());
  float ms = 0;
// ... 558 lines not shown
```

circuitscape_b200/csrc/kernels.cuh:

```cuda
#pragma once
#include <cuda_runtime.h>
#include <stdint.h>

namespace csb {

constexpr int NT = 256;
constexpr int NWARP = NT / 32;
constexpr int NNZ_CAP = 2304;
constexpr int MAXKT = 8;

struct PanelCtl {
  double rho[MAXKT];
  double pap[MAXKT];
  double alpha[MAXKT];
  double beta[MAXKT];
  double tol[MAXKT];
  double rho0[MAXKT];
  double resid[MAXKT];
  double bnorm[MAXKT];
  double xsrc[MAXKT];
  double xdst[MAXKT];
  double maxpos[MAXKT];
  double maxneg[MAXKT];
  double weight[MAXKT];
// ... 887 lines not shown
        } else if (MODE == SP_RES0) {
          out[i] = xo - acc[i];
        } else {
          const T yn = xo + dv * (bb[i] - acc[i]);
          out[i] = yn;
          if (MODE == SP_JACOBI_DOT) dot0[i] += (double)bb[i] * (double)yn;
        }
      }
      stvec<T, CPT>(Y + o, out);
    }
  }
  if (MODE == SP_CG) {
    CSB_REDUCE_SMEM(1, KT)
    double v[1][CPT];
#pragma unroll
    for (int i = 0; i < CPT; ++i) v[0][i] = dot0[i];
    if (grid_reduce<KT, CPT, 1, false>(v, ep.partials, &ep.ctl->ticket, s_warp, s_tree, s_out)) {
      if (tid < KT) {
        const double pap = s_out[tid];
        ep.ctl->pap[tid] = pap;
        ep.ctl->alpha[tid] = (ep.ctl->active[tid] && pap > 0.0) ? ep.ctl->rho[tid] / pap : 0.0;
      }
    }
  } else if (MODE == SP_RESNORM) {
    CSB_REDUCE_SMEM(2, KT)
    double v[2][CPT];
#pragma unroll
    for (int i = 0; i < CPT; ++i) { v[0][i] = dot0[i]; v[1][i] = dot1[i]; }
    if (grid_reduce<KT, CPT, 2, false>(v, ep.partials, &ep.ctl->ticket, s_warp, s_tree, s_out)) {
      if (tid < KT) {
        ep.ctl->resid[tid] = s_out[tid];
        ep.ctl->bnorm[tid] = s_out[KT + tid];
      }
    }
  } else if (MODE == SP_JACOBI_DOT) {
    CSB_REDUCE_SMEM(1, KT)
    double v[1][CPT];
#pragma unroll
    for (int i = 0; i < CPT; ++i) v[0][i] = dot0[i];
    if (grid_reduce<KT, CPT, 1, false>(v, ep.partials, &ep.ctl->ticket, s_warp, s_tree, s_out))
      cg_after_precond<KT>(ep.ctl, s_out);
  }
}

constexpr int CGF_MINB = 2;

template <typename T, int KT, typename TV>
__device__ __forceinline__ void stencil_cg_body(const DiaDev<T>& A, const TV* __restrict__ Z, const T* __restrict__ Pold,
                                                T* __restrict__ Pd, T* __restrict__ X, T* __restrict__ Y,
                                                PanelCtl* ctl, double* partials, int it) {
  constexpr int V16 = 16 / (int)sizeof(T);
  constexpr int CPT = KT < V16 ? KT : V16;
  constexpr int CG = KT / CPT;
  constexpr int RPP = NT / CG;
  const int tid = threadIdx.x;
  const int cg = tid % CG, rl = tid / CG, c0 = cg * CPT;
  const int n = A.n, nr = A.nr;
  const int ncol = (n + nr - 1) / nr;
  const int nrc = (nr + RPP - 1) / RPP;
  const int ntc = (ncol + ST_TC - 1) / ST_TC;
  const long long ntiles = (long long)nrc * ntc;
  const bool pair = it & 1;
  T be[CPT], a1[CPT], a2[CPT];
#pragma unroll
  for (int i = 0; i < CPT; ++i) {
    be[i] = (T)ctl->beta[c0 + i];
    a1[i] = (T)ctl->alpha_ring[(it + 2) % 3][c0 + i];
    a2[i] = (T)ctl->alpha_ring[(it + 1) % 3][c0 + i];
  }
  double dot0[CPT];
#pragma unroll
  for (int i = 0; i < CPT; ++i) dot0[i] = 0.0;

  for (long long t = blockIdx.x; t < ntiles; t += gridDim.x) {
    const int tc = (int)(t / nrc), rc = (int)(t % nrc);
    const int r = rc * RPP + rl;
    if (r >= nr) continue;
    const int cend = min(ncol, (tc + 1) * ST_TC);
    for (int c = tc * ST_TC; c < cend; ++c) {
      const long long row_l = (long long)c * nr + r;
      if (row_l >= n) break;
      const int row = (int)row_l;
      T v[9];
#pragma unroll
      for (int s = 0; s < 9; ++s) v[s] = __ldcs(A.vals + (size_t)s * A.ld + row);
      TV zv[9][CPT];
      T pv[9][CPT];
#pragma unroll
      for (int s = 0; s < 9; ++s) {
        int j = row + (s / 3 - 1) * nr + (s % 3 - 1);
        j = max(0, min(n - 1, j));
        ldvec<TV, CPT>(Z + (size_t)j * KT + c0, zv[s]);
        ldvec<T, CPT, true>(Pold + (size_t)j * KT + c0, pv[s]);
      }
      const size_t o = (size_t)row * KT + c0;
      T xo[CPT], pd[CPT], po[CPT];
      if (pair) {
        ldvec<T, CPT>(X + o, xo);
        ldvec<T, CPT>(Pd + o, pd);
      }
#pragma unroll
      for (int i = 0; i < CPT; ++i) po[i] = pv[4][i];
#pragma unroll
      for (int s = 0; s < 9; ++s)
#pragma unroll
        for (int i = 0; i < CPT; ++i) pv[s][i] = (T)zv[s][i] + be[i] * pv[s][i];
      T acc[CPT];
#pragma unroll
      for (int i = 0; i < CPT; ++i) acc[i] = T(0);
#pragma unroll
      for (int s = 0; s < 9; ++s)
#pragma unroll
        for (int i = 0; i < CPT; ++i) acc[i] += v[s] * pv[s][i];
#pragma unroll
      for (int i = 0; i < CPT; ++i) dot0[i] += (double)acc[i] * (double)pv[4][i];
      stvec<T, CPT>(Y + o, acc);
      stvec<T, CPT>(Pd + o, pv[4]);
      if (pair) {
#pragma unroll
        for (int i = 0; i < CPT; ++i) {
          xo[i] += a2[i] * pd[i];
          xo[i] += a1[i] * po[i];
        }
        stvec<T, CPT>(X + o, xo);
      }
    }
  }
  CSB_REDUCE_SMEM(1, KT)
  double v[1][CPT];
#pragma unroll
  for (int i = 0; i < CPT; ++i) v[0][i] = dot0[i];
  if (grid_reduce<KT, CPT, 1, false>(v, partials, &ctl->ticket, s_warp, s_tree, s_out)) {
    if (tid < KT) {
      const double pap = s_out[tid];
      const double al = (ctl->active[tid] && pap > 0.0) ? ctl->rho[tid] / pap : 0.0;
      ctl->pap[tid] = pap;
      ctl->alpha[tid] = al;
      ctl->alpha_ring[it % 3][tid] = al;
    }
  }
}

template <typename T, int KT, typename TV>
__global__ void __launch_bounds__(NT, CGF_MINB)
k_stencil_cg(const DiaDev<T> A, const TV* __restrict__ Z, T* Pb0, T* Pb1, T* __restrict__ X, T* __restrict__ Y,
             PanelCtl* ctl, double* partials) {
  const int it = ctl->iter;
  stencil_cg_body<T, KT, TV>(A, Z, (it & 1) ? Pb0 : Pb1, (it & 1) ? Pb1 : Pb0, X, Y, ctl, partials, it);
}

constexpr int ST_SMAX = 4;
constexpr int st_a16(int b) { return (b + 15) & ~15; }

template <int PANEL, int OWN, int MINB> struct StDepth {
  static constexpr int BUDGET = 228 * 1024 / MINB - 1024 - 3 * 1024;
  static constexpr int FIT = (BUDGET - 3 * PANEL - OWN) / (PANEL + OWN);
  static constexpr int S = FIT < 1 ? 1 : (FIT > ST_SMAX ? ST_SMAX : FIT);
  static constexpr int BYTES = (S + 3) * PANEL + (S + 1) * OWN;
};

template <int B>
__device__ __forceinline__ void cp_async_zfill(void* dst, const void* src, bool ok) {
  const int sz = ok ? B : 0;
  if constexpr (B == 16)
    asm volatile("cp.async.cg.shared.global [%0], [%1], 16, %2;" ::"r"(smem_u32(dst)), "l"(src), "r"(sz) : "memory");
  else
    asm volatile("cp.async.ca.shared.global [%0], [%1], %2, %3;" ::"r"(smem_u32(dst)), "l"(src), "n"(B), "r"(sz)
                 : "memory");
}
__device__ __forceinline__ void cp_async_commit() { asm volatile("cp.async.commit_group;" ::: "memory"); }
template <int N> __device__ __forceinline__ void cp_async_wait() {
  asm volatile("cp.async.wait_group %0;" ::"n"(N) : "memory");
}

template <typename U, int W, int NROWS>
__device__ __forceinline__ void cp_rows(U* dst, const U* src, long long g0, int n) {
  constexpr int RB = W * (int)sizeof(U);
  constexpr int CH = RB < 16 ? RB : 16;
  constexpr int CPR = RB / CH;
  constexpr int NCH = NROWS * CPR;
#pragma unroll 1
  for (int q0 = 0; q0 < NCH; q0 += NT) {
    const int q = q0 + (int)threadIdx.x;
    if (NCH % NT == 0 || q < NCH) {
      const long long g = g0 + q / CPR;
      const bool ok = g >= 0 && g < n;
      cp_async_zfill<CH>(reinterpret_cast<char*>(dst) + q * CH,
                         reinterpret_cast<const char*>(src + (ok ? g : 0) * W) + (q % CPR) * CH, ok);
    }
  }
}

template <typename T, int RPP>
__device__ __forceinline__ void cp_diag(T* dst, const DiaDev<T>& A, long long row0) {
  constexpr int NCH = 9 * RPP;
#pragma unroll 1
  for (int q0 = 0; q0 < NCH; q0 += NT) {
    const int q = q0 + (int)threadIdx.x;
    if (NCH % NT == 0 || q < NCH) {
      const long long g = row0 + q % RPP;
      const bool ok = g < A.n;
      cp_async_zfill<(int)sizeof(T)>(dst + q, A.run(q / RPP) + (ok ? g : 0), ok);
    }
  }
}

template <typename T, int RPP>
__device__ __forceinline__ void cp_diag_half(T* dst, const DiaDev<T>& A, long long g0, int u0, int u1) {
  constexpr int RW = RPP + 2;
  const int nch = (u1 - u0) * RW;
#pragma unroll 1
  for (int q = (int)threadIdx.x; q < nch; q += NT) {
    const int u = u0 + q / RW, rr = q % RW;
    const long long g = g0 + rr;
    const bool ok = g >= 0 && g < A.n;
    cp_async_zfill<(int)sizeof(T)>(dst + u * RW + rr, A.run(4 + u) + (ok ? g : 0), ok);
  }
}

struct StStep {
  long long t;
  int cs, ce, c, r0;
  __device__ __forceinline__ void start(long long t_, int nrc, int ncol, int rpp) {
    t = t_;
    r0 = (int)(t % nrc) * rpp;
    cs = (int)(t / nrc) * ST_TC;
    ce = min(ncol, cs + ST_TC);
    c = cs - 1;
  }
  __device__ __forceinline__ void next(int nrc, int ncol, int rpp) {
    if (++c > ce) start(t + gridDim.x, nrc, ncol, rpp);
  }
  __device__ __forceinline__ void half_runs(int& u0, int& u1) const {
    u0 = c >= cs ? 0 : 2;
    u1 = c < ce ? 5 : 2;
  }
};

template <typename T, int RPP>
__device__ __forceinline__ T st_half_val(const T* const (&ds)[3], int s9, int rl) {
  return s9 < 4 ? ds[s9 / 3][(4 - s9) * (RPP + 2) + rl + s9 % 3] : ds[1][(s9 - 4) * (RPP + 2) + rl + 1];
}

template <int S, int RPP, class Issue, class Compute>
__device__ __forceinline__ void stencil_pipe(int n, int nr, Issue&& issue, Compute&& compute) {
  constexpr int RP = S + 3, RO = S + 1;
  const int ncol = (n + nr - 1) / nr;
  const int nrc = (nr + RPP - 1) / RPP;
  const long long ntiles = (long long)nrc * ((ncol + ST_TC - 1) / ST_TC);
  StStep ld, st;
  ld.start(blockIdx.x, nrc, ncol, RPP);
  st = ld;
  int lp = 0, lo = 0, sp = 0, so = 0;
#pragma unroll 1
  for (int k = 0; k < S; ++k) {
    if (ld.t < ntiles) issue(ld, lp, lo);
    cp_async_commit();
    ld.next(nrc, ncol, RPP);
    lp = lp + 1 == RP ? 0 : lp + 1;
    lo = lo + 1 == RO ? 0 : lo + 1;
  }
#pragma unroll 1
  while (st.t < ntiles) {
    cp_async_wait<S - 1>();
    __syncthreads();
    if (ld.t < ntiles) issue(ld, lp, lo);
    cp_async_commit();
    ld.next(nrc, ncol, RPP);
    lp = lp + 1 == RP ? 0 : lp + 1;
    lo = lo + 1 == RO ? 0 : lo + 1;
    if (st.c > st.cs) compute(st, sp, so);
    st.next(nrc, ncol, RPP);
    sp = sp + 1 == RP ? 0 : sp + 1;
    so = so + 1 == RO ? 0 : so + 1;
  }
  cp_async_wait<0>();
}

template <typename T, int KT, int MODE, bool HALF> struct StPipe {
  static constexpr int V16 = 16 / (int)sizeof(T);
  static constexpr int CPT = KT < V16 ? KT : V16;
  static constexpr int RPP = NT / (KT / CPT);
  static constexpr bool NEEDB = (MODE == SP_RESNORM || MODE == SP_RES || MODE == SP_JACOBI || MODE == SP_JACOBI_DOT);
  static constexpr bool NEEDD = (MODE == SP_JACOBI || MODE == SP_JACOBI_DOT);
  static constexpr int PX = st_a16((RPP + 2) * KT * (int)sizeof(T));
  static constexpr int PDG = PX + (MODE == SP_RES0 ? st_a16((RPP + 2) * (int)sizeof(T)) : 0);
  static constexpr int PANEL = PDG + (HALF ? st_a16(5 * (RPP + 2) * (int)sizeof(T)) : 0);
  static constexpr int OD = HALF ? 0 : st_a16(9 * RPP * (int)sizeof(T));
  static constexpr int OB = NEEDB ? st_a16(RPP * KT * (int)sizeof(T)) : 0;
  static constexpr int OWN = OD + OB + (NEEDD ? st_a16(RPP * (int)sizeof(T)) : 0);
  using D = StDepth<PANEL, OWN, 3>;
};

template <typename T, int KT, int MODE, bool HALF>
__global__ void __launch_bounds__(NT, 3)
k_stencil_pipe(const DiaDev<T> A, const T* __restrict__ X, T* __restrict__ Y, const SpmmEpi<T> ep) {
  using SP = StPipe<T, KT, MODE, HALF>;
  constexpr int CPT = SP::CPT, RPP = SP::RPP, S = SP::D::S;
  constexpr int RP = S + 3;
  extern __shared__ __align__(128) unsigned char st_sm[];
  unsigned char* const pring = st_sm;
  unsigned char* const oring = st_sm + RP * SP::PANEL;
  const int tid = threadIdx.x;
  const int cg = tid % (KT / CPT), rl = tid / (KT / CPT), c0 = cg * CPT;
  const int n = A.n, nr = A.nr;
  double dot0[CPT], dot1[CPT];
#pragma unroll
  for (int i = 0; i < CPT; ++i) dot0[i] = dot1[i] = 0.0;

  const T* const G = MODE == SP_RES0 ? ep.B : X;
  auto issue = [&](const StStep& s, int lp, int lo) {
    unsigned char* ps = pring + lp * SP::PANEL;
    const long long g0 = (long long)s.c * nr + s.r0 - 1;
    cp_rows<T, KT, RPP + 2>(reinterpret_cast<T*>(ps), G, g0, n);
    if (MODE == SP_RES0) cp_rows<T, 1, RPP + 2>(reinterpret_cast<T*>(ps + SP::PX), ep.dinv, g0, n);
    if (HALF) {
      int u0, u1;
      s.half_runs(u0, u1);
      cp_diag_half<T, RPP>(reinterpret_cast<T*>(ps + SP::PDG), A, g0, u0, u1);
    }
    if (s.c > s.cs) {
      unsigned char* os = oring + lo * SP::OWN;
      const long long row0 = (long long)(s.c - 1) * nr + s.r0;
      if (!HALF) cp_diag<T, RPP>(reinterpret_cast<T*>(os), A, row0);
      if (SP::NEEDB) cp_rows<T, KT, RPP>(reinterpret_cast<T*>(os + SP::OD), ep.B, row0, n);
      if (SP::NEEDD) cp_rows<T, 1, RPP>(reinterpret_cast<T*>(os + SP::OD + SP::OB), ep.dinv, row0, n);
    }
  };
  auto compute = [&](const StStep& s, int sp, int so) {
    const int c = s.c - 1, r = s.r0 + rl;
    const long long row_l = (long long)c * nr + r;
    if (r >= nr || row_l >= n) return;
    const int row = (int)row_l;
    const T* xs[3];
    const T* ws[3];
    const T* ds[3];
#pragma unroll
    for (int d = 0; d < 3; ++d) {
      const int k = sp + d + RP - 2;
      const unsigned char* p = pring + (k >= RP ? k - RP : k) * SP::PANEL;
      xs[d] = reinterpret_cast<const T*>(p);
      ws[d] = reinterpret_cast<const T*>(p + SP::PX);
      ds[d] = reinterpret_cast<const T*>(p + SP::PDG);
    }
    const unsigned char* os = oring + so * SP::OWN;
    const T* dg = reinterpret_cast<const T*>(os);
    T acc[CPT], xo[CPT];
#pragma unroll
    for (int i = 0; i < CPT; ++i) acc[i] = T(0);
#pragma unroll
    for (int s9 = 0; s9 < 9; ++s9) {
      T xv[CPT];
      ldvec<T, CPT>(xs[s9 / 3] + (rl + s9 % 3) * KT + c0, xv);
      if (s9 == 4) {
#pragma unroll
        for (int i = 0; i < CPT; ++i) xo[i] = xv[i];
      }
      const T a9 = HALF ? st_half_val<T, RPP>(ds, s9, rl) : dg[s9 * RPP + rl];
      const T vs = MODE == SP_RES0 ? a9 * (ep.omega * ws[s9 / 3][rl + s9 % 3]) : a9;
#pragma unroll
      for (int i = 0; i < CPT; ++i) acc[i] += vs * xv[i];
    }
    const size_t o = (size_t)row * KT + c0;
    T out[CPT], bb[CPT];
    if (SP::NEEDB) ldvec<T, CPT>(reinterpret_cast<const T*>(os + SP::OD) + rl * KT + c0, bb);
    T dv = T(0);
    if (SP::NEEDD) dv = ep.omega * reinterpret_cast<const T*>(os + SP::OD + SP::OB)[rl];
#pragma unroll
    for (int i = 0; i < CPT; ++i) {
      if (MODE == SP_PLAIN) {
        out[i] = acc[i];
      } else if (MODE == SP_CG) {
        out[i] = acc[i];
        dot0[i] += (double)acc[i] * (double)xo[i];
      } else if (MODE == SP_RESNORM) {
        const T rr = bb[i] - acc[i];
        out[i] = rr;
        dot0[i] += (double)rr * (double)rr;
        dot1[i] += (double)bb[i] * (double)bb[i];
      } else if (MODE == SP_RES) {
        out[i] = bb[i] - acc[i];
      } else if (MODE == SP_RES0) {
        out[i] = xo[i] - acc[i];
      } else {
        const T yn = xo[i] + dv * (bb[i] - acc[i]);
        out[i] = yn;
        if (MODE == SP_JACOBI_DOT) dot0[i] += (double)bb[i] * (double)yn;
      }
    }
    stvec<T, CPT>(Y + o, out);
  };
  stencil_pipe<S, RPP>(n, nr, issue, compute);

  if (MODE == SP_CG) {
    CSB_REDUCE_SMEM(1, KT)
    double v[1][CPT];
#pragma unroll
    for (int i = 0; i < CPT; ++i) v[0][i] = dot0[i];
    if (grid_reduce<KT, CPT, 1, false>(v, ep.partials, &ep.ctl->ticket, s_warp, s_tree, s_out)) {
      if (tid < KT) {
        const double pap = s_out[tid];
        ep.ctl->pap[tid] = pap;
        ep.ctl->alpha[tid] = (ep.ctl->active[tid] && pap > 0.0) ? ep.ctl->rho[tid] / pap : 0.0;
      }
    }
  } else if (MODE == SP_RESNORM) {
    CSB_REDUCE_SMEM(2, KT)
    double v[2][CPT];
#pragma unroll
    for (int i = 0; i < CPT; ++i) { v[0][i] = dot0[i]; v[1][i] = dot1[i]; }
    if (grid_reduce<KT, CPT, 2, false>(v, ep.partials, &ep.ctl->ticket, s_warp, s_tree, s_out)) {
      if (tid < KT) {
        ep.ctl->resid[tid] = s_out[tid];
        ep.ctl->bnorm[tid] = s_out[KT + tid];
      }
    }
  } else if (MODE == SP_JACOBI_DOT) {
    CSB_REDUCE_SMEM(1, KT)
    double v[1][CPT];
#pragma unroll
    for (int i = 0; i < CPT; ++i) v[0][i] = dot0[i];
    if (grid_reduce<KT, CPT, 1, false>(v, ep.partials, &ep.ctl->ticket, s_warp, s_tree, s_out))
      cg_after_precond<KT>(ep.ctl, s_out);
  }
}

constexpr int CGP_MINB = 3;

template <typename T, int KT, typename TV, bool HALF> struct StPipeCg {
  static constexpr int V16 = 16 / (int)sizeof(T);
  static constexpr int CPT = KT < V16 ? KT : V16;
  static constexpr int RPP = NT / (KT / CPT);
  static constexpr int PP = st_a16((RPP + 2) * KT * (int)sizeof(T));
  static constexpr int PDG = PP + st_a16((RPP + 2) * KT * (int)sizeof(TV));
  static constexpr int PANEL = PDG + (HALF ? st_a16(5 * (RPP + 2) * (int)sizeof(T)) : 0);
  static constexpr int OD = HALF ? 0 : st_a16(9 * RPP * (int)sizeof(T));
  static constexpr int OX = st_a16(RPP * KT * (int)sizeof(T));
  static constexpr int OWN = OD + 2 * OX;
  using D = StDepth<PANEL, OWN, CGP_MINB>;
};

template <typename T, int KT, typename TV, bool HALF>
__global__ void __launch_bounds__(NT, CGP_MINB)
k_stencil_cg_pipe(const DiaDev<T> A, const TV* __restrict__ Z, T* Pb0, T* Pb1, T* __restrict__ X, T* __restrict__ Y,
                  PanelCtl* ctl, double* partials) {
  using SP = StPipeCg<T, KT, TV, HALF>;
  constexpr int CPT = SP::CPT, RPP = SP::RPP, S = SP::D::S;
  constexpr int RP = S + 3;
  extern __shared__ __align__(128) unsigned char st_sm[];
  unsigned char* const pring = st_sm;
  unsigned char* const oring = st_sm + RP * SP::PANEL;
  const int it = ctl->iter;
  const T* const Pold = (it & 1) ? Pb0 : Pb1;
  T* const Pd = (it & 1) ? Pb1 : Pb0;
  const int tid = threadIdx.x;
  const int cg = tid % (KT / CPT), rl = tid / (KT / CPT), c0 = cg * CPT;
  const int n = A.n, nr = A.nr;
  const bool pair = it & 1;
  T be[CPT], a1[CPT], a2[CPT];
#pragma unroll
  for (int i = 0; i < CPT; ++i) {
    be[i] = (T)ctl->beta[c0 + i];
    a1[i] = (T)ctl->alpha_ring[(it + 2) % 3][c0 + i];
    a2[i] = (T)ctl->alpha_ring[(it + 1) % 3][c0 + i];
  }
  double dot0[CPT];
#pragma unroll
  for (int i = 0; i < CPT; ++i) dot0[i] = 0.0;

  auto issue = [&](const StStep& s, int lp, int lo) {
    unsigned char* ps = pring + lp * SP::PANEL;
    const long long g0 = (long long)s.c * nr + s.r0 - 1;
    cp_rows<T, KT, RPP + 2>(reinterpret_cast<T*>(ps), Pold, g0, n);
    cp_rows<TV, KT, RPP + 2>(reinterpret_cast<TV*>(ps + SP::PP), Z, g0, n);
    if (HALF) {
      int u0, u1;
      s.half_runs(u0, u1);
      cp_diag_half<T, RPP>(reinterpret_cast<T*>(ps + SP::PDG), A, g0, u0, u1);
    }
    if (s.c > s.cs) {
      unsigned char* os = oring + lo * SP::OWN;
      const long long row0 = (long long)(s.c - 1) * nr + s.r0;
      if (!HALF) cp_diag<T, RPP>(reinterpret_cast<T*>(os), A, row0);
      if (pair) {
        cp_rows<T, KT, RPP>(reinterpret_cast<T*>(os + SP::OD), X, row0, n);
        cp_rows<T, KT, RPP>(reinterpret_cast<T*>(os + SP::OD + SP::OX), Pd, row0, n);
      }
    }
  };
  auto compute = [&](const StStep& s, int sp, int so) {
    const int c = s.c - 1, r = s.r0 + rl;
    const long long row_l = (long long)c * nr + r;
    if (r >= nr || row_l >= n) return;
    const int row = (int)row_l;
    const T* ps[3];
    const TV* zs[3];
    const T* ds[3];
#pragma unroll
    for (int d = 0; d < 3; ++d) {
      const int k = sp + d + RP - 2;
      const unsigned char* p = pring + (k >= RP ? k - RP : k) * SP::PANEL;
      ps[d] = reinterpret_cast<const T*>(p);
      zs[d] = reinterpret_cast<const TV*>(p + SP::PP);
      ds[d] = reinterpret_cast<const T*>(p + SP::PDG);
    }
    const unsigned char* os = oring + so * SP::OWN;
    const T* dg = reinterpret_cast<const T*>(os);
    T acc[CPT], po[CPT], pc[CPT];
#pragma unroll
    for (int i = 0; i < CPT; ++i) acc[i] = T(0);
#pragma unroll
    for (int s9 = 0; s9 < 9; ++s9) {
      T pv[CPT];
      TV zv[CPT];
      ldvec<T, CPT>(ps[s9 / 3] + (rl + s9 % 3) * KT + c0, pv);
      ldvec<TV, CPT>(zs[s9 / 3] + (rl + s9 % 3) * KT + c0, zv);
      if (s9 == 4) {
#pragma unroll
        for (int i = 0; i < CPT; ++i) po[i] = pv[i];
      }
#pragma unroll
      for (int i = 0; i < CPT; ++i) pv[i] = (T)zv[i] + be[i] * pv[i];
      if (s9 == 4) {
#pragma unroll
        for (int i = 0; i < CPT; ++i) pc[i] = pv[i];
      }
      const T vs = HALF ? st_half_val<T, RPP>(ds, s9, rl) : dg[s9 * RPP + rl];
#pragma unroll
      for (int i = 0; i < CPT; ++i) acc[i] += vs * pv[i];
    }
#pragma unroll
    for (int i = 0; i < CPT; ++i) dot0[i] += (double)acc[i] * (double)pc[i];
    const size_t o = (size_t)row * KT + c0;
    stvec<T, CPT>(Y + o, acc);
    stvec<T, CPT>(Pd + o, pc);
    if (pair) {
      T xo[CPT], pd[CPT];
      ldvec<T, CPT>(reinterpret_cast<const T*>(os + SP::OD) + rl * KT + c0, xo);
      ldvec<T, CPT>(reinterpret_cast<const T*>(os + SP::OD + SP::OX) + rl * KT + c0, pd);
#pragma unroll
      for (int i = 0; i < CPT; ++i) {
        xo[i] += a2[i] * pd[i];
        xo[i] += a1[i] * po[i];
      }
      stvec<T, CPT>(X + o, xo);
    }
  };
  stencil_pipe<S, RPP>(n, nr, issue, compute);

  CSB_REDUCE_SMEM(1, KT)
  double v[1][CPT];
#pragma unroll
  for (int i = 0; i < CPT; ++i) v[0][i] = dot0[i];
  if (grid_reduce<KT, CPT, 1, false>(v, partials, &ctl->ticket, s_warp, s_tree, s_out)) {
    if (tid < KT) {
      const double pap = s_out[tid];
      const double al = (ctl->active[tid] && pap > 0.0) ? ctl->rho[tid] / pap : 0.0;
      ctl->pap[tid] = pap;
      ctl->alpha[tid] = al;
      ctl->alpha_ring[it % 3][tid] = al;
    }
  }
}

constexpr int PJ_RING = 4;
constexpr int PJ_MINB_F32 = 3;
constexpr int PJ_MINB_F64 = 2;

template <typename T> struct CsrP {
  const int* rowptr;
  const int* colidx;
  const T* vals;
  const int* ell_col;
  const T* ell_val;
  size_t ell_ld;
};

template <typename T, int KT> struct PjShape {
  static constexpr int V16 = 16 / (int)sizeof(T);
  static constexpr int CPT = KT < V16 ? KT : V16;
  static constexpr int CG = KT / CPT;
  static constexpr int RH = NT / CG;
  static constexpr int RPS = RH - 2;
  static constexpr bool VSMEM = sizeof(T) == 4;
  static constexpr int SMEM = (PJ_RING * RH * KT + 2 * NT * CPT + 2 * NT + (VSMEM ? 2 * 9 * RH : 0)) * (int)sizeof(T);
};

template <typename T, int KT, int MODE, int MINB>
__global__ void __launch_bounds__(NT, MINB)
k_stencil_prolong_jacobi(const DiaDev<T> A, const CsrP<T> P, const T* __restrict__ Yc, const T* __restrict__ X0,
                         T* __restrict__ Z, const SpmmEpi<T> ep) {
  static_assert(MODE == SP_JACOBI || MODE == SP_JACOBI_DOT, "post-smoothing modes only");
  using S = PjShape<T, KT>;
  constexpr int CPT = S::CPT, CG = S::CG, RH = S::RH, RPS = S::RPS;
  extern __shared__ __align__(16) unsigned char pj_smem[];
  T* xs = reinterpret_cast<T*>(pj_smem);
  T* bsm = xs + PJ_RING * RH * KT;
  T* wsm = bsm + 2 * NT * CPT;
  T* vsm = wsm + 2 * NT;
  const int tid = threadIdx.x;
  const int g = tid % CG, rr = tid / CG, c0 = g * CPT;
  const bool inner = rr >= 1 && rr <= RPS;
  const int n = A.n, nr = A.nr;
  const int ncol = (n + nr - 1) / nr;
  const int nstrip = (nr + RPS - 1) / RPS;
  const int nstep = nstrip * ncol;
  const int per = (nstep + (int)gridDim.x - 1) / (int)gridDim.x;
  const int s_beg = (int)min((long long)nstep, (long long)blockIdx.x * per);
  const int s_end = (int)min((long long)nstep, ((long long)blockIdx.x + 1) * per);
  const bool ell = P.ell_col != nullptr;
  double dot0[CPT];
#pragma unroll
  for (int i = 0; i < CPT; ++i) dot0[i] = 0.0;

  for (int s0 = s_beg; s0 < s_end;) {
    const int strip = s0 / ncol, cb = s0 % ncol;
    const int ce = min(ncol, cb + (s_end - s0));
    s0 += ce - cb;
    const int r = strip * RPS + rr - 1;
    const bool rok = r >= 0 && r < nr;
    auto row_of = [&](int c, int& row) {
      const long long rl = (long long)c * nr + r;
      const bool ok = rok && c >= 0 && c < ncol && rl < n;
      row = ok ? (int)rl : 0;
      return ok;
    };
    auto ell_row = [&](int row, int (&cj)[4], T (&pv)[4]) {
#pragma unroll
      for (int q = 0; q < 4; ++q) {
        cj[q] = __ldg(P.ell_col + (size_t)q * P.ell_ld + row);
        pv[q] = __ldg(P.ell_val + (size_t)q * P.ell_ld + row);
      }
    };
    int rowc, rowp = 0;
    bool okc = row_of(cb - 1, rowc), okp = false;
    int cj[4] = {0, 0, 0, 0};
    T pv[4] = {T(0), T(0), T(0), T(0)};
    if (ell) ell_row(rowc, cj, pv);
    __syncthreads();
    for (int c = cb - 1; c <= ce; ++c) {
      const int rel = c - (cb - 1);
      const bool zdo = inner && c > cb && okp;
      T v[9];
      if constexpr (S::VSMEM) {
        if (A.half) {
          if (g == 0) {
            const int u0 = c > cb ? 0 : 2, u1 = c >= cb ? 5 : 2;
            for (int u = u0; u < u1; ++u)
              cp_async_zfill<(int)sizeof(T)>(vsm + ((rel % 3) * 5 + u) * RH + rr, A.run(4 + u) + rowp, okp);
          }
        } else if (zdo && g == 0) {
#pragma unroll
          for (int s = 0; s < 9; ++s)
            asm volatile("cp.async.ca.shared.global [%0], [%1], %2;" ::"r"(smem_u32(vsm + ((rel & 1) * 9 + s) * RH + rr)),
                         "l"(A.run(s) + rowp), "n"((int)sizeof(T)) : "memory");
        }
      } else {
#pragma unroll
        for (int s = 0; s < 9; ++s)
          v[s] = zdo ? (A.half && s < 4 ? A.at(s, rowp) : __ldcs(A.run(s) + rowp)) : T(0);
      }
      int rown;
      const bool okn = row_of(c + 1, rown);
      int cjn[4] = {0, 0, 0, 0};
      T pvn[4] = {T(0), T(0), T(0), T(0)};
      if (ell && c < ce) ell_row(rown, cjn, pvn);
      T bc[CPT], x1[CPT];
      ldvec<T, CPT>(ep.B + (size_t)rowc * KT + c0, bc);
      const T wc = ep.omega * ep.dinv[rowc];
      if (X0) {
        ldvec<T, CPT>(X0 + (size_t)rowc * KT + c0, x1);
      } else {
#pragma unroll
        for (int i = 0; i < CPT; ++i) x1[i] = bc[i] * wc;
      }
      if (ell) {
        T yv[4][CPT];
#pragma unroll
        for (int q = 0; q < 4; ++q) ldvec<T, CPT>(Yc + (size_t)cj[q] * KT + c0, yv[q]);
#pragma unroll
        for (int i = 0; i < CPT; ++i) {
          T a = x1[i];
#pragma unroll
          for (int q = 0; q < 4; ++q) a += pv[q] * yv[q][i];
          x1[i] = okc ? a : T(0);
        }
      } else if (okc) {
        const int a = P.rowptr[rowc], b = P.rowptr[rowc + 1];
        int cq[4];
        T pq[4];
#pragma unroll
        for (int q = 0; q < 4; ++q) {
          const bool ok = a + q < b;
          cq[q] = ok ? __ldg(P.colidx + a + q) : 0;
          pq[q] = ok ? __ldg(P.vals + a + q) : T(0);
        }
        T yv[4][CPT];
#pragma unroll
        for (int q = 0; q < 4; ++q) ldvec<T, CPT>(Yc + (size_t)cq[q] * KT + c0, yv[q]);
#pragma unroll
        for (int q = 0; q < 4; ++q)
#pragma unroll
          for (int i = 0; i < CPT; ++i) x1[i] += pq[q] * yv[q][i];
        for (int j = a + 4; j < b; ++j) {
          const T pw = P.vals[j];
          T yw[CPT];
          ldvec<T, CPT>(Yc + (size_t)P.colidx[j] * KT + c0, yw);
#pragma unroll
          for (int i = 0; i < CPT; ++i) x1[i] += pw * yw[i];
        }
      } else {
#pragma unroll
        for (int i = 0; i < CPT; ++i) x1[i] = T(0);
      }
// ... 876 lines not shown
```

circuitscape_b200/solver.py:

```python
from __future__ import annotations

import ctypes as C
from dataclasses import dataclass

import numpy as np
import scipy.sparse as sp

from . import _lib

CUDAB200 = ["cuda", "gpu", "b200", "cg+jacobi+cuda", "cg+amg+cuda"]


@dataclass
class CUDASolver:
    bs: int = 1000
    precision: str = "double"
    device: int = 0
    rtol: float = 1e-6
    itmax: int = 100_000
    precond: str = "amg"
    panel_width: int = 8
    check_every: int = 16
    use_graph: object = True
    window: str = "auto"
# ... 67 lines not shown
        _lib.check(lib, None, rc)

    def _bind(self, solver):
        self._lib = _lib.load()
        self._h = C.c_void_p()
        self.io_dtype = np.dtype(solver.dtype)
        self.dtype = np.dtype(solver.device_dtype)
        self.solver = solver

    @staticmethod
    def _opts(solver, log_transform=False):
        opts = _lib.Opts()
        opts.precond = _lib.PRECOND_AMG if solver.precond == "amg" else _lib.PRECOND_JACOBI
        opts.panel_width = solver.panel_width
        opts.check_every = solver.check_every
        opts.use_graph = 2 if solver.use_graph == "chunk" else (1 if solver.use_graph else -1)
        opts.log_transform = 1 if log_transform else 0
        opts.window = {"auto": 0, "on": 1, "off": -1}[solver.window]
        opts.mixed = 0 if solver.mixed else -1
        opts.setup = {"auto": 0, "host": 1, "device": 2}[solver.setup]
        opts.stencil = {"auto": 0, "on": 1, "off": -1}[solver.stencil]
        return opts

    @classmethod
    def from_raster_polygons(cls, conductance, polymap, solver: "CUDASolver", four_neighbors=False, avg_res=False,
                             log_transform=False):
        f = cls.__new__(cls)
        f._bind(solver)
        lib = f._lib
        g = np.asfortranarray(conductance, dtype=f.dtype)
        pm = None if polymap is None else np.asfortranarray(polymap, dtype=np.int32)
        nodemap = np.zeros(g.shape, dtype=np.int32, order="F")
        n, nnz = C.c_int64(), C.c_int64()
        opts = cls._opts(solver, log_transform)
        rc = lib.cs_b200_create_from_raster_poly(g.shape[0], g.shape[1], _lib._ptr(g), _lib._ptr(pm),
                                                 _lib.dtype_code(f.dtype), 1 if four_neighbors else 0,
                                                 1 if avg_res else 0, solver.device, C.byref(opts), C.byref(f._h),
                                                 C.byref(n), C.byref(nnz), _lib._ptr(nodemap))
        _lib.check(lib, None, rc)
        f.n = n.value
        return f, nodemap

    @classmethod
    def from_raster(cls, conductance, solver: "CUDASolver", four_neighbors=False, avg_res=False,
                    log_transform=False):
        f = cls.__new__(cls)
        f._bind(solver)
        lib = f._lib
        g = np.asfortranarray(conductance, dtype=f.dtype)
        n, nnz = C.c_int64(), C.c_int64()
        opts = cls._opts(solver, log_transform)
        rc = lib.cs_b200_create_from_raster(g.shape[0], g.shape[1], _lib._ptr(g), _lib.dtype_code(f.dtype),
                                            1 if four_neighbors else 0, 1 if avg_res else 0, solver.device,
                                            C.byref(opts), C.byref(f._h), C.byref(n), C.byref(nnz))
        _lib.check(lib, None, rc)
        f.n = n.value
        return f

    def get_csr(self):
        n, nnz = C.c_int64(), C.c_int64()
        _lib.check(self._lib, self._h, self._lib.cs_b200_get_dims(self._h, C.byref(n), C.byref(nnz)))
        rp = np.empty(n.value + 1, dtype=np.int32)
        ci = np.empty(nnz.value, dtype=np.int32)
        va = np.empty(nnz.value, dtype=self.dtype)
        _lib.check(self._lib, self._h, self._lib.cs_b200_get_csr(self._h, _lib._ptr(rp), _lib._ptr(ci), _lib._ptr(va)))
        return sp.csr_matrix((va, ci, rp), shape=(n.value, n.value))

    def levels(self):
        out = []
        l = 0
        while True:
            lev = {}
            for name, which in (("A", 0), ("P", 1), ("R", 2)):
                nr, nc, nnz = C.c_int64(), C.c_int64(), C.c_int64()
                om, win = C.c_double(), C.c_int()
                rc = self._lib.cs_b200_level_info(self._h, l, which, C.byref(nr), C.byref(nc), C.byref(nnz),
                                                  C.byref(om), C.byref(win))
                if rc != _lib.OK:
                    lev[name] = None
                    continue
                rp = np.empty(nr.value + 1, dtype=np.int32)
                ci = np.empty(nnz.value, dtype=np.int32)
                va = np.empty(nnz.value, dtype=np.float64)
                _lib.check(self._lib, self._h,
                           self._lib.cs_b200_level_csr(self._h, l, which, _lib._ptr(rp), _lib._ptr(ci), _lib._ptr(va)))
                lev[name] = sp.csr_matrix((va, ci, rp), shape=(nr.value, nc.value))
                lev["omega"] = om.value
                lev[name + "_windowed"] = bool(win.value)
                lev[name + "_stencil"] = win.value == 2
            if lev["A"] is None:
                break
            slots = C.c_int()
            _lib.check(self._lib, self._h, self._lib.cs_b200_level_stencil(self._h, l, C.byref(slots)))
            lev["A_stencil_slots"] = slots.value
            out.append(lev)
            l += 1
        return out

    def set_grounds(self, finite=None, dirichlet=None):
        g = None if finite is None else np.ascontiguousarray(finite, dtype=self.dtype)
        m = None if dirichlet is None else np.ascontiguousarray(np.asarray(dirichlet) != 0, dtype=np.uint8)
        assert g is None or len(g) == self.n
        assert m is None or len(m) == self.n
        _lib.check(self._lib, self._h, self._lib.cs_b200_set_grounds(self._h, _lib._ptr(g), _lib._ptr(m)))

    def operator_form(self):
        win = C.c_int()
        rc = self._lib.cs_b200_level_info(self._h, 0, 0, None, None, None, None, C.byref(win))
        _lib.check(self._lib, self._h, rc)
        return {2: "stencil", 1: "windowed"}.get(win.value, "csr")

    def close(self):
        if getattr(self, "_h", None) is not None and self._h.value:
            self._lib.cs_b200_destroy(self._h)
            self._h = C.c_void_p()

    __del__ = close

    def __enter__(self):
        return self

    def __exit__(self, *a):
        self.close()

    def _limits(self, rtol, itmax):
        return (self.solver.rtol if rtol is None else rtol, self.solver.itmax if itmax is None else itmax)

    def _columns(self, k, want_volt, want_curr):
        cols = lambda want: np.empty((self.n, k), dtype=self.dtype, order="F") if want else None
        return cols(want_volt), cols(want_curr), np.zeros(k, dtype=np.int64), np.zeros(k, dtype=np.float64)

    def _io(self, a):
        return a.astype(self.io_dtype) if a is not None and self.io_dtype != self.dtype else a

    def stats(self):
        st = _lib.Stats()
        self._lib.cs_b200_get_stats(self._h, C.byref(st))
        return st.as_dict()

    def stream_ptr(self):
        p = C.c_void_p()
        _lib.check(self._lib, self._h, self._lib.cs_b200_stream(self._h, C.byref(p)))
        return p.value or 0

    def profile_spmm(self, enable):
        ms, cnt = C.c_double(), C.c_int64()
        _lib.check(self._lib, self._h,
                   self._lib.cs_b200_profile_spmm(self._h, -1 if enable is None else int(bool(enable)),
                                                  C.byref(ms), C.byref(cnt)))
        return ms.value, cnt.value

    def profile_classes(self):
        names = ["plain", "cg", "residual_gate", "residual", "jacobi", "jacobi_dot", "prolong_add", "prolong_jacobi_fused",
                 "cg_step_fused"]
        ms = np.zeros(2 * len(names))
        by = np.zeros(2 * len(names))
        ln = np.zeros(2 * len(names), dtype=np.int64)
        _lib.check(self._lib, self._h, self._lib.cs_b200_profile_classes(self._h, _lib._ptr(ms), _lib._ptr(by), _lib._ptr(ln)))
        return {f"{names[i // 2]}_{'f32' if i % 2 else 'f64'}": (float(ms[i]), float(by[i]), int(ln[i]))
                for i in range(2 * len(names)) if ln[i]}

    def profile_bytes(self):
        b = C.c_double()
        _lib.check(self._lib, self._h, self._lib.cs_b200_profile_bytes(self._h, C.byref(b)))
        return b.value

    def spmv(self, x, reps=1):
        x = np.ascontiguousarray(x, dtype=self.dtype)
        y = np.empty_like(x)
        ms = C.c_double()
        rc = self._lib.cs_b200_spmv(self._h, _lib._ptr(x), _lib._ptr(y), reps, C.byref(ms))
        _lib.check(self._lib, self._h, rc)
        return y, ms.value

    def spmm(self, X):
        X = np.asfortranarray(X, dtype=self.dtype)
        Y = np.empty_like(X, order="F")
        rc = self._lib.cs_b200_spmm(self._h, X.shape[1], _lib._ptr(X), _lib._ptr(Y))
        _lib.check(self._lib, self._h, rc)
        return Y

    def apply_precond(self, R):
        R = np.asarray(R, dtype=self.dtype)
        vec = R.ndim == 1
        X = np.asfortranarray(R.reshape(self.n, -1))
        Z = np.empty_like(X, order="F")
        rz = np.zeros(X.shape[1])
        rc = self._lib.cs_b200_apply_precond(self._h, X.shape[1], _lib._ptr(X), _lib._ptr(Z), _lib._ptr(rz))
        _lib.check(self._lib, self._h, rc)
        return (Z[:, 0] if vec else Z), rz

    def bench_spmm(self, k, reps=20, flush_l2=False):
        ms = C.c_double()
        rc = self._lib.cs_b200_bench_spmm(self._h, k, reps, 1 if flush_l2 else 0, C.byref(ms))
        _lib.check(self._lib, self._h, rc)
        return ms.value

    def bench_cg_iter(self, k, reps=20):
        ms = C.c_double()
        rc = self._lib.cs_b200_bench_cg_iter(self._h, k, reps, C.byref(ms))
        _lib.check(self._lib, self._h, rc)
        return ms.value

    def solve_rhs(self, rhs, rtol=None, itmax=None, raise_on_residual=True, out=None):
        rhs = np.asarray(rhs, dtype=self.dtype)
        vec = rhs.ndim == 1
        b = np.asfortranarray(rhs.reshape(self.n, -1))
        k = b.shape[1]
        x = out if out is not None else np.empty_like(b, order="F")
        assert x.flags.f_contiguous and x.shape == b.shape and x.dtype == b.dtype
        iters = np.zeros(k, dtype=np.int64)
        relres = np.zeros(k, dtype=np.float64)
        rc = self._lib.cs_b200_solve_rhs(self._h, k, _lib._ptr(b), _lib._ptr(x), *self._limits(rtol, itmax),
                                         _lib._ptr(iters), _lib._ptr(relres))
        self._raise(rc, raise_on_residual)
        if out is None:
            x = self._io(x)
        return (x[:, 0] if vec else x), iters, relres

    def solve_pairs(self, src, dst, weight=None, want_volt=False, want_curr=False,
                    accumulate=False, rtol=None, itmax=None, raise_on_residual=True, want_branch=False):
        src = np.ascontiguousarray(src, dtype=np.int64)
        dst = np.ascontiguousarray(dst, dtype=np.int64)
        k = len(src)
        R = np.zeros(k, dtype=self.dtype)
        volt, curr, iters, relres = self._columns(k, want_volt, want_curr)
        args = (self._h, k, _lib._ptr(src), _lib._ptr(dst), _lib._ptr(_opt(weight, np.float64)),
                *self._limits(rtol, itmax), _lib._ptr(R), _lib._ptr(volt), _lib._ptr(curr), 1 if accumulate else 0,
                _lib._ptr(iters), _lib._ptr(relres))
        branch = None
        if want_branch:
            branch = np.empty((self._num_branches(), k), dtype=self.dtype, order="F")
            rc = self._lib.cs_b200_solve_pairs_branch(*args, _lib._ptr(branch))
        else:
            rc = self._lib.cs_b200_solve_pairs(*args)
        self._raise(rc, raise_on_residual)
        return dict(R=self._io(R), volt=self._io(volt), curr=self._io(curr), iters=iters, relres=relres,
                    branch=self._io(branch))

    def _num_branches(self):
        nb = C.c_int64()
        _lib.check(self._lib, self._h, self._lib.cs_b200_branch_index(self._h, C.byref(nb), None, None))
        return nb.value

    def branch_index(self):
        nb = self._num_branches()
        lo = np.empty(nb, dtype=np.int64)
        hi = np.empty(nb, dtype=np.int64)
        n_ = C.c_int64()
        _lib.check(self._lib, self._h,
                   self._lib.cs_b200_branch_index(self._h, C.byref(n_), _lib._ptr(lo), _lib._ptr(hi)))
        return lo, hi

    def components(self):
        nc = C.c_int64()
        comp_of = np.empty(self.n, dtype=np.int32)
        _lib.check(self._lib, self._h, self._lib.cs_b200_components(self._h, C.byref(nc), _lib._ptr(comp_of)))
        return nc.value, comp_of

    def read_branch_currents(self):
        cum = np.empty(self._num_branches(), dtype=self.dtype)
        _lib.check(self._lib, self._h, self._lib.cs_b200_read_branch_currents(self._h, _lib._ptr(cum)))
        return cum

    def solve_pairs_superposed(self, nodes, pi, pj, weight=None, want_volt=False, want_curr=False,
                               accumulate=False, rtol=None, itmax=None, raise_on_residual=True):
        nodes = np.ascontiguousarray(nodes, dtype=np.int64)
        pi = np.ascontiguousarray(pi, dtype=np.int64)
        pj = np.ascontiguousarray(pj, dtype=np.int64)
        k = len(pi)
        R = np.zeros(k, dtype=self.dtype)
        volt, curr, _, relres = self._columns(k, want_volt, want_curr)
        iters = np.zeros(max(len(nodes) - 1, 1), dtype=np.int64)
        rc = self._lib.cs_b200_solve_pairs_superposed(
            self._h, len(nodes), _lib._ptr(nodes), k, _lib._ptr(pi), _lib._ptr(pj),
            _lib._ptr(_opt(weight, np.float64)), *self._limits(rtol, itmax), _lib._ptr(R), _lib._ptr(volt),
            _lib._ptr(curr), 1 if accumulate else 0, _lib._ptr(iters), _lib._ptr(relres))
        self._raise(rc, raise_on_residual)
        return dict(R=self._io(R), volt=self._io(volt), curr=self._io(curr), iters=iters, relres=relres)

    def solve_region_pairs(self, sets, set_a, set_b, weight=None, want_volt=False, want_curr=False,
                           accumulate=False, rtol=None, itmax=None, raise_on_residual=True):
        ptr, rows = _csr(sets, np.int64)
        set_a = np.ascontiguousarray(set_a, dtype=np.int64)
        set_b = np.ascontiguousarray(set_b, dtype=np.int64)
        k = len(set_a)
        R = np.zeros(k, dtype=self.dtype)
        volt, curr, iters, relres = self._columns(k, want_volt, want_curr)
        rc = self._lib.cs_b200_solve_region_pairs(
            self._h, len(sets), _lib._ptr(ptr), _lib._ptr(rows), k, _lib._ptr(set_a), _lib._ptr(set_b),
            _lib._ptr(_opt(weight, np.float64)), *self._limits(rtol, itmax), _lib._ptr(R), _lib._ptr(volt),
            _lib._ptr(curr), 1 if accumulate else 0, _lib._ptr(iters), _lib._ptr(relres))
        self._raise(rc, raise_on_residual)
        return dict(R=self._io(R), volt=self._io(volt), curr=self._io(curr), iters=iters, relres=relres)

    def solve_grounded(self, sets, gset, sources, weight=None, want_volt=False, want_curr=False,
                       accumulate=False, rtol=None, itmax=None, raise_on_residual=True):
        ptr, rows, gset, sptr, srows, svals = _grounded_columns(sets, gset, sources)
        k = len(gset)
        sv = np.zeros(k, dtype=self.dtype)
        volt, curr, iters, relres = self._columns(k, want_volt, want_curr)
        rc = self._lib.cs_b200_solve_grounded(
            self._h, len(sets), _lib._ptr(ptr), _lib._ptr(rows), k, _lib._ptr(gset), _lib._ptr(sptr),
            _lib._ptr(srows), _lib._ptr(svals), _lib._ptr(_opt(weight, np.float64)), *self._limits(rtol, itmax),
            _lib._ptr(sv), _lib._ptr(volt), _lib._ptr(curr), 1 if accumulate else 0, _lib._ptr(iters),
            _lib._ptr(relres))
        self._raise(rc, raise_on_residual)
        return dict(src_volt=self._io(sv), volt=self._io(volt), curr=self._io(curr), iters=iters, relres=relres)

    def solve_advanced(self, sets, gset, sources, weight=None, want_volt=False, want_curr=False,
                       accumulate=False, rtol=None, itmax=None, raise_on_residual=True):
# ... 121 lines not shown
```

include/cs_b200.h:

```cpp
#ifndef CS_B200_H
#define CS_B200_H

#include <stdint.h>

#ifdef __cplusplus
extern "C" {
#endif

typedef struct cs_b200_handle cs_b200_handle;

enum cs_b200_status {
  CS_B200_OK = 0,
  CS_B200_ERR_ARG = -1,
  CS_B200_ERR_CUDA = -2,
  CS_B200_ERR_RESIDUAL = -3,
  CS_B200_ERR_MAXITER = -4,
  CS_B200_ERR_UNSUPPORTED = -5
};

enum cs_b200_dtype { CS_B200_F32 = 0, CS_B200_F64 = 1 };

enum cs_b200_precond {
  CS_B200_PRECOND_JACOBI = 0,
  CS_B200_PRECOND_AMG = 1
// ... 6 lines not shown
  int32_t use_graph;
  double atol;
  double resid_gate;
  int32_t log_transform;
  int32_t window;
  int32_t mixed;
  int32_t setup;
  int32_t stencil;
  int32_t reserved[3];
} cs_b200_opts;

typedef struct cs_b200_stats {
  double setup_ms;
  double solve_ms;
  double kernel_ms;
  int64_t iterations;
  int64_t spmm_launches;
  int64_t kernel_launches;
  double h2d_bytes, d2h_bytes;
} cs_b200_stats;

int cs_b200_create(int64_t n, int64_t nnz, const void* rowptr, const void* colidx,
                   const void* vals, int index_bits, int index_base, int dtype,
                   int device, const cs_b200_opts* opts, cs_b200_handle** out);

int cs_b200_create_from_device(int64_t n, int64_t nnz, const int32_t* d_rowptr,
                               const int32_t* d_colidx, const void* d_vals, int dtype,
                               int device, const cs_b200_opts* opts, cs_b200_handle** out);

int cs_b200_create_from_raster(int64_t nrows, int64_t ncols, const void* g, int dtype,
                               int four_neighbors, int avg_res, int device,
                               const cs_b200_opts* opts, cs_b200_handle** out,
                               int64_t* n_out, int64_t* nnz_out);

int cs_b200_create_from_raster_poly(int64_t nrows, int64_t ncols, const void* g, const int32_t* polymap,
                                    int dtype, int four_neighbors, int avg_res, int device,
                                    const cs_b200_opts* opts, cs_b200_handle** out, int64_t* n_out,
                                    int64_t* nnz_out, int32_t* nodemap_out);

int cs_b200_get_csr(cs_b200_handle* h, int32_t* rowptr, int32_t* colidx, void* vals);

int cs_b200_set_grounds(cs_b200_handle* h, const void* finite_g, const uint8_t* dirichlet);

int cs_b200_level_info(cs_b200_handle* h, int level, int which, int64_t* nrows, int64_t* ncols,
                       int64_t* nnz, double* omega, int* windowed);
int cs_b200_level_csr(cs_b200_handle* h, int level, int which, int32_t* rowptr, int32_t* colidx,
                      double* vals);
int cs_b200_level_stencil(cs_b200_handle* h, int level, int* slots);

int cs_b200_get_dims(const cs_b200_handle* h, int64_t* n, int64_t* nnz);

void cs_b200_destroy(cs_b200_handle* h);

const char* cs_b200_last_error(const cs_b200_handle* h);

int cs_b200_spmv(cs_b200_handle* h, const void* x, void* y, int reps, double* ms_per_rep);

int cs_b200_spmm(cs_b200_handle* h, int k, const void* x, void* y);

int cs_b200_apply_precond(cs_b200_handle* h, int k, const void* r, void* z, double* rz);

int cs_b200_bench_spmm(cs_b200_handle* h, int k, int reps, int flush_l2, double* ms_per_rep);

int cs_b200_bench_cg_iter(cs_b200_handle* h, int k, int reps, double* ms_per_rep);

int cs_b200_solve_rhs(cs_b200_handle* h, int64_t k, const void* rhs, void* lhs,
                      double rtol, int64_t itmax, int64_t* iters, double* relres);

int cs_b200_solve_pairs(cs_b200_handle* h, int64_t k, const int64_t* src, const int64_t* dst,
                        const double* weight, double rtol, int64_t itmax, void* R,
                        void* volt, void* curr, int accumulate, int64_t* iters,
                        double* relres);

int cs_b200_branch_index(cs_b200_handle* h, int64_t* nb, int64_t* lo, int64_t* hi);

int cs_b200_components(cs_b200_handle* h, int64_t* ncomp, int32_t* comp_of);

int cs_b200_solve_pairs_branch(cs_b200_handle* h, int64_t k, const int64_t* src, const int64_t* dst,
                               const double* weight, double rtol, int64_t itmax, void* R, void* volt,
                               void* curr, int accumulate, int64_t* iters, double* relres, void* branch);

int cs_b200_solve_pairs_superposed(cs_b200_handle* h, int64_t np, const int64_t* nodes, int64_t k,
                                   const int64_t* pi, const int64_t* pj, const double* weight,
                                   double rtol, int64_t itmax, void* R, void* volt, void* curr,
                                   int accumulate, int64_t* point_iters, double* relres);

int cs_b200_solve_region_pairs(cs_b200_handle* h, int64_t nsets, const int64_t* set_ptr,
                               const int64_t* set_rows, int64_t k, const int64_t* set_a,
                               const int64_t* set_b, const double* weight, double rtol, int64_t itmax,
                               void* R, void* volt, void* curr, int accumulate,
                               int64_t* iters, double* relres);

int cs_b200_solve_grounded(cs_b200_handle* h, int64_t nsets, const int64_t* set_ptr, const int64_t* set_rows,
                           int64_t k, const int64_t* gset, const int64_t* src_ptr, const int64_t* src_rows,
                           const double* src_vals, const double* weight, double rtol, int64_t itmax,
                           void* src_volt, void* volt, void* curr, int accumulate, int64_t* iters,
                           double* relres);

int cs_b200_solve_advanced(cs_b200_handle* h, int64_t nsets, const int64_t* set_ptr, const int64_t* set_rows,
                           int64_t k, const int64_t* gset, const int64_t* src_ptr, const int64_t* src_rows,
                           const double* src_vals, const double* weight, double rtol, int64_t itmax, void* volt,
                           void* curr, int accumulate, int64_t* iters, double* relres);

int cs_b200_solve_advanced_network(cs_b200_handle* h, int64_t nsets, const int64_t* set_ptr,
                                   const int64_t* set_rows, int64_t k, const int64_t* gset, const int64_t* src_ptr,
                                   const int64_t* src_rows, const double* src_vals, const int64_t* owner,
                                   double rtol, int64_t itmax, void* volt, void* curr, void* branch,
                                   int64_t* iters, double* relres);

int cs_b200_solve_sources(cs_b200_handle* h, int64_t k, const int64_t* colptr, const int64_t* rows,
                          const double* vals, const int64_t* ref, const double* weight,
                          double rtol, int64_t itmax, int64_t nprobe, const int64_t* probe,
                          void* probe_volt, void* volt, void* curr, int accumulate,
                          int64_t* iters, double* relres);

int cs_b200_solve_advanced_batch(int64_t nwin, int64_t nrows, int64_t ncols, const void* g, const void* src,
                                 const void* gnd, int dtype, int four_neighbors, int device, double rtol,
                                 int64_t itmax, void* cur, void* volt, int64_t* iters, double* relres,
                                 int64_t* first_failed);

int cs_b200_read_currents(cs_b200_handle* h, void* cum, void* max);
int cs_b200_reset_currents(cs_b200_handle* h);
int cs_b200_read_branch_currents(cs_b200_handle* h, void* cum_branch);
int cs_b200_currents_device_ptrs(cs_b200_handle* h, void** d_cum, void** d_max);

int cs_b200_get_stats(const cs_b200_handle* h, cs_b200_stats* out);

int cs_b200_stream(cs_b200_handle* h, void** stream);

int cs_b200_profile_spmm(cs_b200_handle* h, int enable, double* total_ms, int64_t* launches);

int cs_b200_profile_bytes(cs_b200_handle* h, double* algorithmic_bytes);

typedef struct cs_b200_comm cs_b200_comm;

int cs_b200_comm_unique_id(void* id128);
int cs_b200_comm_init(int device, int rank, int nranks, const void* id128, cs_b200_comm** out);
void cs_b200_comm_destroy(cs_b200_comm* c);
const char* cs_b200_comm_last_error(const cs_b200_comm* c);

int cs_b200_create_bcast(cs_b200_comm* c, int root, int64_t n, int64_t nnz, const void* rowptr,
                         const void* colidx, const void* vals, int index_bits, int index_base,
                         int dtype, const cs_b200_opts* opts, cs_b200_handle** out);

int cs_b200_comm_reduce_currents(cs_b200_comm* c, cs_b200_handle* h);

int cs_b200_comm_gather_pairs(cs_b200_comm* c, int64_t k_total, const int64_t* my_idx,
                              int64_t k_mine, const double* my_R, double* R_all);

int cs_b200_comm_max_double(cs_b200_comm* c, double* v, int count);
int cs_b200_comm_barrier(cs_b200_comm* c);

int cs_b200_profile_classes(cs_b200_handle* h, double* ms18, double* bytes18, int64_t* launches18);

int cs_b200_version(void);

#ifdef __cplusplus
}
#endif
#endif
```

profiles/run_iteration_breakdown.py:

```python
#!/usr/bin/env python
import argparse
import ctypes as C
import json
import os
import re
import subprocess
import sys
from collections import defaultdict

sys.path.insert(0, os.path.dirname(os.path.dirname(os.path.abspath(__file__))))
import numpy as np

PEAK_GBS = 3350.0
KT = 8


def card():
    try:
        out = subprocess.run(["nvidia-smi", "--query-gpu=name,power.limit", "--format=csv,noheader"],
                             capture_output=True, text=True, timeout=30).stdout.strip().splitlines()
        name, pl = [s.strip() for s in out[0].split(",")]
        return {"name": name, "power_limit": pl}
    except Exception as e:
        return {"name": None, "power_limit": None, "error": str(e)}


def level_dims(f):
    out = []
    for l in range(64):
        lev = {}
        for name, which in (("A", 0), ("P", 1), ("R", 2)):
            nr, nc, nnz = C.c_int64(), C.c_int64(), C.c_int64()
            om, win = C.c_double(), C.c_int()
            rc = f._lib.cs_b200_level_info(f._h, l, which, C.byref(nr), C.byref(nc), C.byref(nnz),
                                           C.byref(om), C.byref(win))
            lev[name] = (nr.value, nc.value, nnz.value, win.value) if rc == 0 else None
        if lev["A"] is None:
            break
        slots = C.c_int()
        f._lib.cs_b200_level_stencil(f._h, l, C.byref(slots))
        lev["A_stencil_slots"] = slots.value
        out.append(lev)
    return out


def short(name):
    name = name.replace("(anonymous namespace)::", "").replace("csb::", "")
    name = re.sub(r"^void ", "", name)
    depth, cut = 0, len(name)
    for i, ch in enumerate(name):
        if ch == "<":
            depth += 1
        elif ch == ">":
            depth -= 1
        elif ch == "(" and depth == 0:
            cut = i
            break
    return name[:cut].replace(" ", "")


def finest_bytes(levels, prolong_form):
    n = levels[0]["A"][0]
    n1 = levels[1]["A"][0] if len(levels) > 1 else 0
    nnz_r = levels[0]["R"][2] if levels[0]["R"] else 0
    d64, d32 = 8 * KT, 4 * KT
    rps = 256 // 2 - 2
    half = levels[0].get("A_stencil_slots") == 5
    dg64 = (5 + 3 / 16) * 66 / 64 if half else 9
    dg32 = (5 + 3 / 16) * 130 / 128 if half else 9
    if prolong_form == "tile":
        halo = (130 * 10) / (128 * 8)
        prol = n * (halo * (d32 + 4 + 32 + d32) + 9 * 4 + d32 + 4 + d32)
    else:
        halo = (rps + 2) / rps
        prol = n * (halo * (d32 + 4 + 32 + d32) + (5 * halo if half else 9) * 4 + d32)
    cg_step = n * (dg64 * 8 + d32 + 3 * d64 + 1.5 * d64)
    res0 = n * (dg32 * 4 + d32 + 4 + d32)
    return {
        "k_stencil<double,8,1>": n * (9 * 8 + d64 + d64),
        "k_stencil_pipe<double,8,1,*>": n * (dg64 * 8 + d64 + d64),
        "k_stencil<double,8,2>": n * (9 * 8 + 3 * d64),
        "k_stencil_pipe<double,8,2,*>": n * (dg64 * 8 + 3 * d64),
        "k_stencil_cg<double,8,float>": cg_step,
        "k_stencil_cg_pipe<double,8,float,*>": cg_step,
        "k_cg_update_r0<double,8,float>": n * (d64 + 8 + 2 * d64 + d32),
        "k_stencil<float,8,7>#1": res0,
        "k_stencil_pipe<float,8,7,*>#1": res0,
        "k_spmm_win<float,8,0,*>#1": nnz_r * 6 + n1 * 2 + n * d32 + n1 * d32,
        "k_stencil_prolong_jacobi<float,8,5,*>": prol,
        "k_cg_update_xp2<double,8,float>": n * (d32 + 4 * d64),
    }, {"n": n, "n1": n1, "nnz_R0": nnz_r, "prolong_halo_factor": halo,
        "level0_stencil_slots": levels[0].get("A_stencil_slots")}


def match_bytes(key, table):
    for pat, b in table.items():
        base, _, occ = pat.partition("#")
        rx = "^" + re.escape(base).replace(r"\*", r"[^,>]+") + "$"
        name, _, slot = key.partition("#")
        if re.match(rx, name) and (not occ or (slot or "1").split("/")[0] == occ):
            return b
    return None


def main():
    ap = argparse.ArgumentParser()
    ap.add_argument("--rows", type=int, default=3163)
    ap.add_argument("--reps", type=int, default=20)
    ap.add_argument("--prolong-form", default="strip", choices=["strip", "tile"])
    ap.add_argument("--out", default="")
    a = ap.parse_args()

    import torch
    from torch.profiler import ProfilerActivity, profile
    import circuitscape_b200 as cb
    from circuitscape_b200 import graph
    if not torch.cuda.is_available():
        raise SystemExit("needs a CUDA device")
    L, _ = graph.synthetic_raster_laplacian(a.rows, a.rows, seed=42)
    with cb.construct_cholesky_factor(L, cb.CUDASolver()) as f:
        levels = level_dims(f)
        f.bench_cg_iter(KT, reps=5)
        ms_iter = f.bench_cg_iter(KT, reps=a.reps)
        torch.cuda.synchronize()
        with profile(activities=[ProfilerActivity.CUDA]) as prof:
            f.bench_cg_iter(KT, reps=a.reps)
            torch.cuda.synchronize()
    evs = [e for e in prof.events() if e.device_type.name == "CUDA" and "memcpy" not in e.name.lower()
           and "memset" not in e.name.lower()]
    evs.sort(key=lambda e: e.time_range.start)
    starts = [i for i, e in enumerate(evs) if short(e.name).startswith(("k_stencil<double,8,1>", "k_stencil_cg<double,8,",
                                                                        "k_stencil_pipe<double,8,1,",
                                                                        "k_stencil_cg_pipe<double,8,",
                                                                        "k_spmm_win<double,8,1,"))]
    iters = [evs[starts[j]:starts[j + 1]] for j in range(len(starts) - 1)]
    iters = iters[3:] if len(iters) > a.reps else iters
    if len(starts) > 1:
        last = evs[starts[-1]:]
        iters.append(last[:len(iters[0])] if iters else last)
    agg = defaultdict(lambda: [0, 0.0])
    for it in iters:
        names = [short(e.name) for e in it]
        tot = defaultdict(int)
        for nm in names:
            tot[nm] += 1
        seen = defaultdict(int)
        for e, nm in zip(it, names):
            seen[nm] += 1
            key = nm if tot[nm] == 1 else f"{nm}#{seen[nm]}/{tot[nm]}"
            agg[key][0] += 1
            agg[key][1] += e.time_range.elapsed_us()
    niter = max(1, len(iters))
    table, shape = finest_bytes(levels, a.prolong_form)
    sum_us = sum(v[1] for v in agg.values()) / niter
    rows = {}
    for key, (cnt, us) in sorted(agg.items(), key=lambda kv: -kv[1][1]):
        avg = us / cnt
        r = {"launches_per_iter": cnt / niter, "avg_us": avg, "share": (us / niter) / sum_us}
        b = match_bytes(key, table)
        if b is not None:
            r.update({"bytes": b, "GB/s": b / (avg * 1e-6) / 1e9, "frac_of_peak": b / (avg * 1e-6) / 1e9 / PEAK_GBS})
        rows[key] = r
    res = {"card": card(), "rows": a.rows, "k": KT, "iterations_profiled": niter,
           "iter_ms_events": ms_iter, "iter_ms_kernel_sum": sum_us / 1e3, "peak_GBs": PEAK_GBS,
           "peak_source": "H100 SXM data sheet (HBM3)", "prolong_form": a.prolong_form, "shape": shape,
           "levels": [{k: v for k, v in lev.items()} for lev in levels], "kernels": rows}
    line = json.dumps(res)
    print(line)
    if a.out:
        os.makedirs(os.path.dirname(os.path.abspath(a.out)), exist_ok=True)
        with open(a.out, "w") as fh:
            fh.write(line + "\n")


if __name__ == "__main__":
    main()
```

Before: 139.4.

## Fuse CG residual update with level-0 smoother residual into one stencil sweep

Adds a k_stencil_res_update kernel that recomputes A·p from the stencil, updates the residual R into a ping-pong buffer, writes the fp32 residual, and performs the level-0 implicit-x0 Jacobi residual sweep in the same pass. The fused CG step no longer stores AP, and the separate k_cg_update_r0 and level-0 res0 launches are skipped. The goal is to cut memory traffic and launches per iteration. In exchange it recomputes the stencil product, adds a second R buffer, and is gated by a one-time device check that the fp32 stencil coefficients are exact roundings of the fp64 ones.

Result: faster. 145.1, median of 6 (+4.1%).

```diff
diff --git a/circuitscape_b200/_lib.py b/circuitscape_b200/_lib.py
--- a/circuitscape_b200/_lib.py
+++ b/circuitscape_b200/_lib.py
@@ -109,6 +109,7 @@
     "cs_b200_stream": (C.c_int, [_H, C.POINTER(C.c_void_p)]),
     "cs_b200_profile_spmm": (C.c_int, [_H, C.c_int, C.POINTER(C.c_double), C.POINTER(C.c_int64)]),
     "cs_b200_profile_classes": (C.c_int, [_H, C.c_void_p, C.c_void_p, C.c_void_p]),
+    "cs_b200_profile_classes_n": (C.c_int, [_H, C.c_int, C.c_void_p, C.c_void_p, C.c_void_p]),
     "cs_b200_profile_bytes": (C.c_int, [_H, C.POINTER(C.c_double)]),
     "cs_b200_comm_unique_id": (C.c_int, [C.c_void_p]),
     "cs_b200_comm_init": (C.c_int, [C.c_int, C.c_int, C.c_int, C.c_void_p, C.POINTER(_H)]),
diff --git a/circuitscape_b200/csrc/cs_b200.cu b/circuitscape_b200/csrc/cs_b200.cu
--- a/circuitscape_b200/csrc/cs_b200.cu
+++ b/circuitscape_b200/csrc/cs_b200.cu
@@ -27,8 +27,9 @@
 
 thread_local std::string g_create_error;
 
-constexpr int PROF_CLASSES = 18;
+constexpr int PROF_CLASSES = 20;
 constexpr int PROF_CGF = 8;
+constexpr int PROF_RSW = 9;
 
 struct GraphSlot {
   cudaGraphExec_t exec = nullptr;
@@ -88,6 +89,7 @@
   void *X = nullptr, *R = nullptr, *P = nullptr, *AP = nullptr, *B = nullptr, *stage = nullptr;
   void* Z = nullptr;
   void* P2 = nullptr;
+  void* R2 = nullptr;
   DevCsr A0;
   std::vector<DevLevel> lv;
   double* d_pinv = nullptr;
@@ -489,6 +491,17 @@
   return on || !stencil_pipe();
 }
 
+inline bool implicit_x0(const DevLevel& L) {
+  static const bool off = std::getenv("CS_B200_NO_IMPLICIT_X0") != nullptr || std::getenv("CS_B200_NO_FUSED_PROLONG") != nullptr;
+  return L.A.dia != nullptr && !off;
+}
+
+inline bool fused_res_form(const cs_b200_handle* h) {
+  static const bool off = std::getenv("CS_B200_NO_FUSED_RES") != nullptr;
+  return !off && h->mixed && stencil_pipe() && h->A0.dia && h->A0.dia_half && !h->lv32.empty() &&
+         h->lv32[0].A.dia_half && implicit_x0(h->lv32[0]);
+}
+
 template <typename T>
 DiaDev<T> dia_view(const DevCsr& m) {
   return DiaDev<T>{(const T*)m.dia, m.dia_ld, m.nrows, m.dia_nr, m.dia_half};
@@ -742,6 +755,28 @@
       if (e == cudaSuccess) e = cudaMemsetAsync(h->P2, 0, pe, h->stream);
       if (e != cudaSuccess) return set_err(h, CS_B200_ERR_CUDA, "CUDA error %s (second p panel)", cudaGetErrorString(e));
     }
+    if (h->P2 && fused_res_form(h)) {
+      int* d_diff = nullptr;
+      int diff = 1;
+      cudaError_t e = cudaMalloc(&d_diff, sizeof(int));
+      if (e == cudaSuccess) e = cudaMemsetAsync(d_diff, 0, sizeof(int), h->stream);
+      if (e == cudaSuccess) {
+        k_dia_rounds<T, float><<<std::min<int64_t>((5 * h->n + 255) / 256, 4096), 256, 0, h->stream>>>(
+            dia_view<T>(h->A0), dia_view<float>(h->lv32[0].A), d_diff);
+        e = cudaMemcpyAsync(&diff, d_diff, sizeof(int), cudaMemcpyDeviceToHost, h->stream);
+      }
+      if (e == cudaSuccess) e = cudaStreamSynchronize(h->stream);
+      cudaFree(d_diff);
+      if (e == cudaSuccess && diff == 0 && !h->R2) {
+        const size_t pe = (size_t)h->n_pad * h->ktmax * sizeof(T);
+        e = cudaMalloc(&h->R2, pe);
+        if (e == cudaSuccess) e = cudaMemsetAsync(h->R2, 0, pe, h->stream);
+      } else if (diff != 0) {
+        cudaFree(h->R2);
+        h->R2 = nullptr;
+      }
+      if (e != cudaSuccess) return set_err(h, CS_B200_ERR_CUDA, "CUDA error %s (second r panel)", cudaGetErrorString(e));
+    }
   } else {
     csb_dev::seed_discard(job);
   }
@@ -918,11 +953,6 @@
   return (int)std::max<size_t>(1, std::min<size_t>(h->grid_ew, (nelem + per - 1) / per));
 }
 
-inline bool implicit_x0(const DevLevel& L) {
-  static const bool off = std::getenv("CS_B200_NO_IMPLICIT_X0") != nullptr || std::getenv("CS_B200_NO_FUSED_PROLONG") != nullptr;
-  return L.A.dia != nullptr && !off;
-}
-
 template <typename T, int KT>
 void launch_stencil_res0(cs_b200_handle* h, DevLevel& L, const T* B, T* Tout, bool timed) {
   const DevCsr& m = L.A;
@@ -993,7 +1023,8 @@
 struct VcBufs { void *b0, *x0, *t0, *y0; };
 
 template <typename T, int KT>
-void launch_vcycle_on(cs_b200_handle* h, std::vector<DevLevel>& lv, const VcBufs& vb, bool level0_presmoothed) {
+void launch_vcycle_on(cs_b200_handle* h, std::vector<DevLevel>& lv, const VcBufs& vb, bool level0_presmoothed,
+                      bool level0_residual) {
   const int nl = (int)lv.size();
   auto B = [&](int l) { return l == 0 ? (T*)vb.b0 : (T*)lv[l].b; };
   auto X = [&](int l) { return l == 0 ? (T*)vb.x0 : (T*)lv[l].x; };
@@ -1003,7 +1034,7 @@
     DevLevel& L = lv[l];
     const size_t nelem = (size_t)L.n_pad * KT;
     if (implicit_x0(L)) {
-      launch_stencil_res0<T, KT>(h, L, B(l), Tm(l), l == 0);
+      if (!(l == 0 && level0_residual)) launch_stencil_res0<T, KT>(h, L, B(l), Tm(l), l == 0);
     } else {
       if (!(l == 0 && level0_presmoothed)) {
         k_jacobi0<T, KT><<<ew_grid_n<T, KT>(h, L.n_pad), NT, 0, h->stream>>>(
@@ -1047,13 +1078,13 @@
 }
 
 template <typename T, int KT>
-void launch_vcycle(cs_b200_handle* h, bool level0_presmoothed) {
+void launch_vcycle(cs_b200_handle* h, bool level0_presmoothed, bool level0_residual = false) {
   if (h->mixed) {
     const VcBufs vb{h->R32, h->X32, h->T32, h->Z32};
-    launch_vcycle_on<float, KT>(h, h->lv32, vb, level0_presmoothed);
+    launch_vcycle_on<float, KT>(h, h->lv32, vb, level0_presmoothed, level0_residual);
   } else {
     const VcBufs vb{h->R, h->stage, h->AP, h->Z};
-    launch_vcycle_on<T, KT>(h, h->lv, vb, level0_presmoothed);
+    launch_vcycle_on<T, KT>(h, h->lv, vb, level0_presmoothed, level0_residual);
   }
 }
 
@@ -1087,18 +1118,25 @@
   return h->amg && h->A0.dia && h->P2 && !off;
 }
 
-template <typename T, int KT, typename TV, bool HALF>
+inline bool fused_res(const cs_b200_handle* h) {
+  return fused_cg(h) && h->R2 && !h->rg_on && fused_res_form(h);
+}
+
+template <typename T, int KT, typename TV, bool HALF, bool STORE_AP>
 void launch_stencil_cg_pipe(cs_b200_handle* h, const DiaDev<T>& a, const TV* Z, int sg) {
   constexpr int SMEM = StPipeCg<T, KT, TV, HALF>::D::BYTES;
   static bool once[64] = {};
   bool& set = once[h->device & 63];
-  if (!set) { cudaFuncSetAttribute(k_stencil_cg_pipe<T, KT, TV, HALF>, cudaFuncAttributeMaxDynamicSharedMemorySize, SMEM); set = true; }
-  k_stencil_cg_pipe<T, KT, TV, HALF><<<sg, NT, SMEM, h->stream>>>(a, Z, (T*)h->P2, (T*)h->P, (T*)h->X, (T*)h->AP,
-                                                                  h->d_ctl, h->d_partials);
+  if (!set) {
+    cudaFuncSetAttribute(k_stencil_cg_pipe<T, KT, TV, HALF, STORE_AP>, cudaFuncAttributeMaxDynamicSharedMemorySize, SMEM);
+    set = true;
+  }
+  k_stencil_cg_pipe<T, KT, TV, HALF, STORE_AP><<<sg, NT, SMEM, h->stream>>>(a, Z, (T*)h->P2, (T*)h->P, (T*)h->X,
+                                                                            (T*)h->AP, h->d_ctl, h->d_partials);
 }
 
 template <typename T, int KT, typename TV>
-void launch_stencil_cg(cs_b200_handle* h, const TV* Z) {
+void launch_stencil_cg(cs_b200_handle* h, const TV* Z, bool store_ap) {
   const DevCsr& m = h->A0;
   const DiaDev<T> a = dia_view<T>(m);
   constexpr int V16 = 16 / (int)sizeof(T);
@@ -1114,20 +1152,62 @@
     e0 = h->prof_ev[h->prof_used++];
     e1 = h->prof_ev[h->prof_used++];
     const double pe = (double)m.nrows * KT * sizeof(T);
-    const double fb = (double)m.nrows * 9 * sizeof(T) + (double)m.nrows * KT * sizeof(TV) + 3.0 * pe + 1.5 * pe;
+    const double fb = (double)m.nrows * 9 * sizeof(T) + (double)m.nrows * KT * sizeof(TV) + (store_ap ? 3.0 : 2.0) * pe +
+                      1.5 * pe;
     h->prof_bytes += fb;
     h->prof_slot.push_back(2 * PROF_CGF + (sizeof(T) == 4 ? 1 : 0));
     h->prof_pair_bytes.push_back(fb);
     cudaEventRecord(e0, h->stream);
   }
   if (stencil_pipe()) {
-    if (a.half) launch_stencil_cg_pipe<T, KT, TV, true>(h, a, Z, sg);
-    else launch_stencil_cg_pipe<T, KT, TV, false>(h, a, Z, sg);
+    if (!store_ap) {
+      if constexpr (sizeof(T) == 8 && sizeof(TV) == 4) launch_stencil_cg_pipe<T, KT, TV, true, false>(h, a, Z, sg);
+    } else if (a.half) launch_stencil_cg_pipe<T, KT, TV, true, true>(h, a, Z, sg);
+    else launch_stencil_cg_pipe<T, KT, TV, false, true>(h, a, Z, sg);
   } else {
     if (a.half) refuse_half("k_stencil_cg");
     k_stencil_cg<T, KT, TV><<<sg, NT, 0, h->stream>>>(a, Z, (T*)h->P2, (T*)h->P, (T*)h->X, (T*)h->AP, h->d_ctl,
                                                        h->d_partials);
   }
+  if (h->profile) cudaEventRecord(e1, h->stream);
+  h->stats.kernel_launches++;
+  h->stats.spmm_launches++;
+}
+
+template <typename T, int KT>
+void launch_res_update(cs_b200_handle* h) {
+  const DevCsr& m = h->A0;
+  DevLevel& L = h->lv32[0];
+  using SH = RuShape<T, float, KT>;
+  constexpr int SMEM = SH::D::BYTES;
+  static bool once[64] = {};
+  bool& set = once[h->device & 63];
+  if (!set) {
+    cudaFuncSetAttribute(k_stencil_res_update<T, float, KT>, cudaFuncAttributeMaxDynamicSharedMemorySize, SMEM);
+    set = true;
+  }
+  int occ = 0;
+  cudaOccupancyMaxActiveBlocksPerMultiprocessor(&occ, k_stencil_res_update<T, float, KT>, NT, SMEM);
+  occ = std::max(1, occ);
+  const long long nsteps = (long long)((m.dia_nr + SH::RPS - 1) / SH::RPS) *
+                           (((long long)m.nrows + m.dia_nr - 1) / m.dia_nr);
+  const int grid = (int)std::max<long long>(1, std::min<long long>(std::min(h->grid_spmm, h->num_sms * occ), nsteps));
+  cudaEvent_t e0 = nullptr, e1 = nullptr;
+  if (h->profile) {
+    if (h->prof_used + 2 > h->prof_ev.size())
+      for (int i = 0; i < 2; ++i) { cudaEvent_t e; cudaEventCreate(&e); h->prof_ev.push_back(e); }
+    e0 = h->prof_ev[h->prof_used++];
+    e1 = h->prof_ev[h->prof_used++];
+    const double nr = (double)m.nrows;
+    const double fb = nr * KT * (3.0 * sizeof(T) + 2.0 * sizeof(float)) + nr * 5 * sizeof(T) + nr * sizeof(float);
+    h->prof_bytes += fb;
+    h->prof_slot.push_back(2 * PROF_RSW + (sizeof(T) == 4 ? 1 : 0));
+    h->prof_pair_bytes.push_back(fb);
+    cudaEventRecord(e0, h->stream);
+  }
+  k_stencil_res_update<T, float, KT><<<grid, NT, SMEM, h->stream>>>(
+      dia_view<T>(m), (const float*)L.dinv, (float)L.omega, (const T*)h->P2, (const T*)h->P,
+      (T*)h->R, (T*)h->R2, (float*)h->R32, (float*)h->T32, h->d_ctl);
   if (h->profile) cudaEventRecord(e1, h->stream);
   h->stats.kernel_launches++;
   h->stats.spmm_launches++;
@@ -1138,9 +1218,10 @@
   const size_t nelem = (size_t)h->n_pad * KT;
   const int g = ew_grid<T, KT>(h);
   const bool fused = fused_cg(h);
+  const bool fres = sizeof(T) == 8 && fused_res(h);
   if (fused) {
-    if (h->mixed) launch_stencil_cg<T, KT, float>(h, (const float*)h->Z32);
-    else launch_stencil_cg<T, KT, T>(h, (const T*)h->Z);
+    if (h->mixed) launch_stencil_cg<T, KT, float>(h, (const float*)h->Z32, !fres);
+    else launch_stencil_cg<T, KT, T>(h, (const T*)h->Z, true);
   } else {
     launch_spmm<T, KT, SP_CG>(h, (const T*)h->P, (T*)h->AP, nullptr);
   }
@@ -1153,11 +1234,16 @@
     h->stats.kernel_launches += 2;
   } else {
     if (h->mixed) {
-      k_cg_update_r0<T, KT, float><<<g, NT, 0, h->stream>>>(nelem, (const T*)h->AP, (const T*)h->d_dinv,
-                                                            (T)h->lv[0].omega, (T*)h->R,
-                                                            implicit_x0(h->lv32[0]) ? nullptr : (float*)h->X32,
-                                                            (float*)h->R32, h->d_ctl);
-      launch_vcycle<T, KT>(h, true);
+      if (fres) {
+        if constexpr (sizeof(T) == 8) launch_res_update<T, KT>(h);
+      } else {
+        k_cg_update_r0<T, KT, float><<<g, NT, 0, h->stream>>>(nelem, (const T*)h->AP, (const T*)h->d_dinv,
+                                                              (T)h->lv[0].omega, (T*)h->R,
+                                                              implicit_x0(h->lv32[0]) ? nullptr : (float*)h->X32,
+                                                              (float*)h->R32, h->d_ctl);
+        h->stats.kernel_launches++;
+      }
+      launch_vcycle<T, KT>(h, true, fres);
       mask_z<T, KT>(h);
       if (!fused)
         k_cg_update_xp2<T, KT, float><<<g, NT, 0, h->stream>>>(nelem, (const float*)h->Z32, (T*)h->X, (T*)h->P,
@@ -1167,12 +1253,13 @@
                                                         (T)h->lv[0].omega, (T*)h->R,
                                                         implicit_x0(h->lv[0]) ? nullptr : (T*)h->stage, nullptr,
                                                         h->d_ctl);
+      h->stats.kernel_launches++;
       launch_vcycle<T, KT>(h, true);
       mask_z<T, KT>(h);
       if (!fused)
         k_cg_update_xp2<T, KT, T><<<g, NT, 0, h->stream>>>(nelem, (const T*)h->Z, (T*)h->X, (T*)h->P, h->d_ctl);
     }
-    h->stats.kernel_launches += fused ? 1 : 2;
+    if (!fused) h->stats.kernel_launches++;
   }
 }
 
@@ -2554,7 +2641,7 @@
   cudaFree(h->d_vals0);
   cudaFree(h->d_fg);
   cudaFree(h->d_bptr); cudaFree(h->d_cum_branch); cudaFree(h->d_branch_stage);
-  void* bufs[] = {h->d_dinv, h->d_bstart, h->X, h->R, h->P, h->P2, h->AP, h->B, h->stage,
+  void* bufs[] = {h->d_dinv, h->d_bstart, h->X, h->R, h->R2, h->P, h->P2, h->AP, h->B, h->stage,
                   h->d_cum, h->d_max, h->d_ctl, h->d_partials, h->d_flush};
   for (void* b : bufs) if (b) cudaFree(b);
   if (h->h_ctl) cudaFreeHost(h->h_ctl);
@@ -2711,11 +2798,15 @@
 }
 
 int cs_b200_profile_classes(cs_b200_handle* h, double* ms18, double* bytes18, int64_t* launches18) {
-  if (!h) return CS_B200_ERR_ARG;
-  for (int i = 0; i < PROF_CLASSES; ++i) {
-    if (ms18) ms18[i] = h->prof_slot_ms[i];
-    if (bytes18) bytes18[i] = h->prof_slot_bytes[i];
-    if (launches18) launches18[i] = h->prof_slot_launches[i];
+  return cs_b200_profile_classes_n(h, 18, ms18, bytes18, launches18);
+}
+
+int cs_b200_profile_classes_n(cs_b200_handle* h, int nslots, double* ms, double* bytes, int64_t* launches) {
+  if (!h || nslots < 0) return CS_B200_ERR_ARG;
+  for (int i = 0; i < std::min(nslots, PROF_CLASSES); ++i) {
+    if (ms) ms[i] = h->prof_slot_ms[i];
+    if (bytes) bytes[i] = h->prof_slot_bytes[i];
+    if (launches) launches[i] = h->prof_slot_launches[i];
   }
   return CS_B200_OK;
 }
diff --git a/circuitscape_b200/csrc/kernels.cuh b/circuitscape_b200/csrc/kernels.cuh
--- a/circuitscape_b200/csrc/kernels.cuh
+++ b/circuitscape_b200/csrc/kernels.cuh
@@ -1063,11 +1063,11 @@
 constexpr int ST_SMAX = 4;
 constexpr int st_a16(int b) { return (b + 15) & ~15; }
 
-template <int PANEL, int OWN, int MINB> struct StDepth {
-  static constexpr int BUDGET = 228 * 1024 / MINB - 1024 - 3 * 1024;
+template <int PANEL, int OWN, int MINB, int EXTRA = 0> struct StDepth {
+  static constexpr int BUDGET = 228 * 1024 / MINB - 1024 - 3 * 1024 - EXTRA;
   static constexpr int FIT = (BUDGET - 3 * PANEL - OWN) / (PANEL + OWN);
   static constexpr int S = FIT < 1 ? 1 : (FIT > ST_SMAX ? ST_SMAX : FIT);
-  static constexpr int BYTES = (S + 3) * PANEL + (S + 1) * OWN;
+  static constexpr int BYTES = (S + 3) * PANEL + (S + 1) * OWN + EXTRA;
 };
 
 template <int B>
@@ -1151,6 +1151,20 @@
 template <typename T, int RPP>
 __device__ __forceinline__ T st_half_val(const T* const (&ds)[3], int s9, int rl) {
   return s9 < 4 ? ds[s9 / 3][(4 - s9) * (RPP + 2) + rl + s9 % 3] : ds[1][(s9 - 4) * (RPP + 2) + rl + 1];
+}
+
+template <typename T, int CPT, class Val, class Coef>
+__device__ __forceinline__ void stencil_row(T (&acc)[CPT], Val&& val, Coef&& coef) {
+#pragma unroll
+  for (int i = 0; i < CPT; ++i) acc[i] = T(0);
+#pragma unroll
+  for (int s9 = 0; s9 < 9; ++s9) {
+    T v[CPT];
+    val(s9, v);
+    const T a = coef(s9);
+#pragma unroll
+    for (int i = 0; i < CPT; ++i) acc[i] += a * v[i];
+  }
 }
 
 template <int S, int RPP, class Issue, class Compute>
@@ -1351,7 +1365,7 @@
   using D = StDepth<PANEL, OWN, CGP_MINB>;
 };
 
-template <typename T, int KT, typename TV, bool HALF>
+template <typename T, int KT, typename TV, bool HALF, bool STORE_AP>
 __global__ void __launch_bounds__(NT, CGP_MINB)
 k_stencil_cg_pipe(const DiaDev<T> A, const TV* __restrict__ Z, T* Pb0, T* Pb1, T* __restrict__ X, T* __restrict__ Y,
                   PanelCtl* ctl, double* partials) {
@@ -1418,32 +1432,28 @@
     const unsigned char* os = oring + so * SP::OWN;
     const T* dg = reinterpret_cast<const T*>(os);
     T acc[CPT], po[CPT], pc[CPT];
-#pragma unroll
-    for (int i = 0; i < CPT; ++i) acc[i] = T(0);
-#pragma unroll
-    for (int s9 = 0; s9 < 9; ++s9) {
-      T pv[CPT];
-      TV zv[CPT];
-      ldvec<T, CPT>(ps[s9 / 3] + (rl + s9 % 3) * KT + c0, pv);
-      ldvec<TV, CPT>(zs[s9 / 3] + (rl + s9 % 3) * KT + c0, zv);
-      if (s9 == 4) {
-#pragma unroll
-        for (int i = 0; i < CPT; ++i) po[i] = pv[i];
-      }
-#pragma unroll
-      for (int i = 0; i < CPT; ++i) pv[i] = (T)zv[i] + be[i] * pv[i];
-      if (s9 == 4) {
-#pragma unroll
-        for (int i = 0; i < CPT; ++i) pc[i] = pv[i];
-      }
-      const T vs = HALF ? st_half_val<T, RPP>(ds, s9, rl) : dg[s9 * RPP + rl];
-#pragma unroll
-      for (int i = 0; i < CPT; ++i) acc[i] += vs * pv[i];
-    }
+    stencil_row<T, CPT>(
+        acc,
+        [&](int s9, T (&pv)[CPT]) {
+          TV zv[CPT];
+          ldvec<T, CPT>(ps[s9 / 3] + (rl + s9 % 3) * KT + c0, pv);
+          ldvec<TV, CPT>(zs[s9 / 3] + (rl + s9 % 3) * KT + c0, zv);
+          if (s9 == 4) {
+#pragma unroll
+            for (int i = 0; i < CPT; ++i) po[i] = pv[i];
+          }
+#pragma unroll
+          for (int i = 0; i < CPT; ++i) pv[i] = (T)zv[i] + be[i] * pv[i];
+          if (s9 == 4) {
+#pragma unroll
+            for (int i = 0; i < CPT; ++i) pc[i] = pv[i];
+          }
+        },
+        [&](int s9) { return HALF ? st_half_val<T, RPP>(ds, s9, rl) : dg[s9 * RPP + rl]; });
 #pragma unroll
     for (int i = 0; i < CPT; ++i) dot0[i] += (double)acc[i] * (double)pc[i];
     const size_t o = (size_t)row * KT + c0;
-    stvec<T, CPT>(Y + o, acc);
+    if (STORE_AP) stvec<T, CPT>(Y + o, acc);
     stvec<T, CPT>(Pd + o, pc);
     if (pair) {
       T xo[CPT], pd[CPT];
@@ -1471,6 +1481,199 @@
       ctl->alpha[tid] = al;
       ctl->alpha_ring[it % 3][tid] = al;
     }
+  }
+}
+
+constexpr int RU_MINB = 3;
+constexpr int RU_RING = 4;
+
+template <typename T, typename TV, int KT> struct RuShape {
+  static constexpr int V16 = 16 / (int)sizeof(T);
+  static constexpr int CPT = KT < V16 ? KT : V16;
+  static constexpr int CG = KT / CPT;
+  static constexpr int RH = NT / CG;
+  static constexpr int RPS = RH - 2;
+  static constexpr int PDG = st_a16((RH + 2) * KT * (int)sizeof(T));
+  static constexpr int PW32 = PDG + st_a16(5 * (RH + 2) * (int)sizeof(T));
+  static constexpr int PANEL = PW32 + st_a16(RH * (int)sizeof(TV));
+  static constexpr int OWN = st_a16(RH * KT * (int)sizeof(T));
+  static constexpr int RING = RU_RING * RH * KT * (int)sizeof(TV);
+  static constexpr int DRING = RU_RING * 5 * RH * (int)sizeof(TV);
+  using D = StDepth<PANEL, OWN, RU_MINB, RING + DRING>;
+};
+
+struct RuStep {
+  int s0, s_end, ncol, strip, cb, ce, x;
+  __device__ __forceinline__ void start(int s) {
+    s0 = s;
+    if (s >= s_end) return;
+    strip = s / ncol;
+    cb = s % ncol;
+    ce = min(ncol, cb + (s_end - s));
+    x = cb - 2;
+  }
+  __device__ __forceinline__ bool valid() const { return s0 < s_end; }
+  __device__ __forceinline__ void next() {
+    if (++x > ce + 2) start(s0 + (ce - cb));
+  }
+};
+
+template <typename T, typename TV, int KT>
+__global__ void __launch_bounds__(NT, RU_MINB)
+k_stencil_res_update(const DiaDev<T> A, const TV* __restrict__ dinv32, TV omega,
+                     const T* __restrict__ Pb0, const T* __restrict__ Pb1, T* Rb0, T* Rb1, TV* __restrict__ R32,
+                     TV* __restrict__ T32, const PanelCtl* __restrict__ ctl) {
+  using SH = RuShape<T, TV, KT>;
+  constexpr int CPT = SH::CPT, CG = SH::CG, RH = SH::RH, RPS = SH::RPS, S = SH::D::S;
+  constexpr int RP = S + 3, RO = S + 1;
+  extern __shared__ __align__(128) unsigned char st_sm[];
+  unsigned char* const pring = st_sm;
+  unsigned char* const oring = st_sm + RP * SH::PANEL;
+  TV* const xring = reinterpret_cast<TV*>(oring + RO * SH::OWN);
+  TV* const dring = xring + RU_RING * RH * KT;
+  const int it = ctl->iter;
+  const T* const Pk = (it & 1) ? Pb1 : Pb0;
+  const T* const Rin = (it & 1) ? Rb1 : Rb0;
+  T* const Rout = (it & 1) ? Rb0 : Rb1;
+  const int tid = threadIdx.x;
+  const int g = tid % CG, rr = tid / CG, c0 = g * CPT;
+  const bool inner = rr >= 1 && rr <= RPS;
+  const int n = A.n, nr = A.nr;
+  const int ncol = (n + nr - 1) / nr;
+  const int nstrip = (nr + RPS - 1) / RPS;
+  const int nstep = nstrip * ncol;
+  const int per = (nstep + (int)gridDim.x - 1) / (int)gridDim.x;
+  const int s_beg = (int)min((long long)nstep, (long long)blockIdx.x * per);
+  const int s_end = (int)min((long long)nstep, ((long long)blockIdx.x + 1) * per);
+  T al[CPT];
+#pragma unroll
+  for (int i = 0; i < CPT; ++i) al[i] = (T)ctl->alpha[c0 + i];
+
+  auto issue = [&](const RuStep& s, int lp, int lo) {
+    unsigned char* ps = pring + lp * SH::PANEL;
+    const long long r0 = (long long)s.strip * RPS;
+    if (s.x <= s.ce + 1) {
+      const long long g0 = (long long)s.x * nr + r0 - 2;
+      cp_rows<T, KT, RH + 2>(reinterpret_cast<T*>(ps), Pk, g0, n);
+      cp_diag_half<T, RH>(reinterpret_cast<T*>(ps + SH::PDG), A, g0, 0, 5);
+    }
+    if (s.x - 2 >= s.cb - 1)
+      cp_rows<TV, 1, RH>(reinterpret_cast<TV*>(ps + SH::PW32), dinv32, (long long)(s.x - 2) * nr + r0 - 1, n);
+    if (s.x - 1 >= s.cb - 1 && s.x - 1 <= s.ce)
+      cp_rows<T, KT, RH>(reinterpret_cast<T*>(oring + lo * SH::OWN), Rin, (long long)(s.x - 1) * nr + r0 - 1, n);
+  };
+  auto compute = [&](const RuStep& s, int sp, int so, int q) {
+    const unsigned char* pk[3];
+#pragma unroll
+    for (int d = 0; d < 3; ++d) {
+      const int k = sp + d + RP - 2;
+      pk[d] = pring + (k >= RP ? k - RP : k) * SH::PANEL;
+    }
+    const int r = s.strip * RPS + rr - 1;
+    const int ca = s.x - 1;
+    if (ca >= s.cb - 1 && ca <= s.ce) {
+      const T* ps[3];
+      const T* ds[3];
+#pragma unroll
+      for (int d = 0; d < 3; ++d) {
+        ps[d] = reinterpret_cast<const T*>(pk[d]);
+        ds[d] = reinterpret_cast<const T*>(pk[d] + SH::PDG);
+      }
+      T acc[CPT], rv[CPT];
+      TV r32[CPT];
+      stencil_row<T, CPT>(
+          acc, [&](int s9, T (&pv)[CPT]) { ldvec<T, CPT>(ps[s9 / 3] + (rr + s9 % 3) * KT + c0, pv); },
+          [&](int s9) { return st_half_val<T, RH>(ds, s9, rr); });
+      ldvec<T, CPT>(reinterpret_cast<const T*>(oring + so * SH::OWN) + rr * KT + c0, rv);
+#pragma unroll
+      for (int i = 0; i < CPT; ++i) {
+        rv[i] -= al[i] * acc[i];
+        r32[i] = (TV)rv[i];
+      }
+      stvec<TV, CPT>(xring + (q * RH + rr) * KT + c0, r32);
+      if (g == 0) {
+#pragma unroll
+        for (int u = 0; u < 5; ++u) dring[(q * 5 + u) * RH + rr] = (TV)ds[1][u * (RH + 2) + rr + 1];
+      }
+      const long long row = (long long)ca * nr + r;
+      if (inner && r < nr && ca >= s.cb && ca < s.ce && row < n) {
+        stvec<T, CPT>(Rout + (size_t)row * KT + c0, rv);
+        stvec<TV, CPT>(R32 + (size_t)row * KT + c0, r32);
+      }
+    }
+    const int ct = s.x - 3;
+    const long long row = (long long)ct * nr + r;
+    if (ct >= s.cb && ct < s.ce && inner && r < nr && row < n) {
+      const TV* xs[3];
+      const TV* ws[3];
+      const TV* ds[3];
+#pragma unroll
+      for (int d = 0; d < 3; ++d) {
+        xs[d] = xring + ((q + 1 + d) & (RU_RING - 1)) * RH * KT;
+        ws[d] = reinterpret_cast<const TV*>(pk[d] + SH::PW32);
+        ds[d] = dring + ((q + 1 + d) & (RU_RING - 1)) * 5 * RH;
+      }
+      const int rl = rr - 1;
+      TV acc[CPT], xo[CPT], out[CPT];
+      stencil_row<TV, CPT>(
+          acc,
+          [&](int s9, TV (&xv)[CPT]) {
+            ldvec<TV, CPT>(xs[s9 / 3] + (rl + s9 % 3) * KT + c0, xv);
+            if (s9 == 4) {
+#pragma unroll
+              for (int i = 0; i < CPT; ++i) xo[i] = xv[i];
+            }
+          },
+          [&](int s9) { return st_half_val<TV, RPS>(ds, s9, rl) * (omega * ws[s9 / 3][rl + s9 % 3]); });
+#pragma unroll
+      for (int i = 0; i < CPT; ++i) out[i] = xo[i] - acc[i];
+      stvec<TV, CPT>(T32 + (size_t)row * KT + c0, out);
+    }
+  };
+
+  RuStep ld, st;
+  ld.s_end = s_end;
+  ld.ncol = ncol;
+  ld.start(s_beg);
+  st = ld;
+  int lp = 0, lo = 0, sp = 0, so = 0, q = 0;
+#pragma unroll 1
+  for (int k = 0; k < S; ++k) {
+    if (ld.valid()) issue(ld, lp, lo);
+    cp_async_commit();
+    if (ld.valid()) ld.next();
+    lp = lp + 1 == RP ? 0 : lp + 1;
+    lo = lo + 1 == RO ? 0 : lo + 1;
+  }
+#pragma unroll 1
+  while (st.valid()) {
+    cp_async_wait<S - 1>();
+    __syncthreads();
+    if (ld.valid()) issue(ld, lp, lo);
+    cp_async_commit();
+    if (ld.valid()) ld.next();
+    lp = lp + 1 == RP ? 0 : lp + 1;
+    lo = lo + 1 == RO ? 0 : lo + 1;
+    compute(st, sp, so, q);
+    st.next();
+    sp = sp + 1 == RP ? 0 : sp + 1;
+    so = so + 1 == RO ? 0 : so + 1;
+    q = (q + 1) & (RU_RING - 1);
+  }
+  cp_async_wait<0>();
+}
+
+template <typename T, typename TV>
+__global__ void k_dia_rounds(const DiaDev<T> A, const DiaDev<TV> A32, int* differs) {
+  const long long tot = 5LL * A.n;
+  for (long long i = (long long)blockIdx.x * blockDim.x + threadIdx.x; i < tot; i += (long long)gridDim.x * blockDim.x) {
+    const int u = (int)(i / A.n), row = (int)(i % A.n);
+    const TV a = (TV)A.run(4 + u)[row], b = A32.run(4 + u)[row];
+    static_assert(sizeof(TV) == 4, "fp32 copies");
+    unsigned ua, ub;
+    memcpy(&ua, &a, 4);
+    memcpy(&ub, &b, 4);
+    if (ua != ub) *differs = 1;
   }
 }
 
diff --git a/circuitscape_b200/solver.py b/circuitscape_b200/solver.py
--- a/circuitscape_b200/solver.py
+++ b/circuitscape_b200/solver.py
@@ -243,11 +243,12 @@
 
     def profile_classes(self):
         names = ["plain", "cg", "residual_gate", "residual", "jacobi", "jacobi_dot", "prolong_add", "prolong_jacobi_fused",
-                 "cg_step_fused"]
+                 "cg_step_fused", "residual_sweep_fused"]
         ms = np.zeros(2 * len(names))
         by = np.zeros(2 * len(names))
         ln = np.zeros(2 * len(names), dtype=np.int64)
-        _lib.check(self._lib, self._h, self._lib.cs_b200_profile_classes(self._h, _lib._ptr(ms), _lib._ptr(by), _lib._ptr(ln)))
+        _lib.check(self._lib, self._h, self._lib.cs_b200_profile_classes_n(self._h, len(ms), _lib._ptr(ms), _lib._ptr(by),
+                                                                           _lib._ptr(ln)))
         return {f"{names[i // 2]}_{'f32' if i % 2 else 'f64'}": (float(ms[i]), float(by[i]), int(ln[i]))
                 for i in range(2 * len(names)) if ln[i]}
 
diff --git a/include/cs_b200.h b/include/cs_b200.h
--- a/include/cs_b200.h
+++ b/include/cs_b200.h
@@ -182,6 +182,7 @@
 int cs_b200_comm_barrier(cs_b200_comm* c);
 
 int cs_b200_profile_classes(cs_b200_handle* h, double* ms18, double* bytes18, int64_t* launches18);
+int cs_b200_profile_classes_n(cs_b200_handle* h, int nslots, double* ms, double* bytes, int64_t* launches);
 
 int cs_b200_version(void);
 
diff --git a/profiles/run_iteration_breakdown.py b/profiles/run_iteration_breakdown.py
--- a/profiles/run_iteration_breakdown.py
+++ b/profiles/run_iteration_breakdown.py
@@ -75,14 +75,18 @@
         halo = (rps + 2) / rps
         prol = n * (halo * (d32 + 4 + 32 + d32) + (5 * halo if half else 9) * 4 + d32)
     cg_step = n * (dg64 * 8 + d32 + 3 * d64 + 1.5 * d64)
+    cg_step_no_ap = cg_step - n * d64
     res0 = n * (dg32 * 4 + d32 + 4 + d32)
+    ru = n * ((d64 + 5 * 8) * 66 / 62 + (d64 + 4) * 64 / 62 + d64 + d32 + d32)
     return {
         "k_stencil<double,8,1>": n * (9 * 8 + d64 + d64),
         "k_stencil_pipe<double,8,1,*>": n * (dg64 * 8 + d64 + d64),
         "k_stencil<double,8,2>": n * (9 * 8 + 3 * d64),
         "k_stencil_pipe<double,8,2,*>": n * (dg64 * 8 + 3 * d64),
         "k_stencil_cg<double,8,float>": cg_step,
-        "k_stencil_cg_pipe<double,8,float,*>": cg_step,
+        "k_stencil_cg_pipe<double,8,float,*,true>": cg_step,
+        "k_stencil_cg_pipe<double,8,float,*,false>": cg_step_no_ap,
+        "k_stencil_res_update<double,float,8>": ru,
         "k_cg_update_r0<double,8,float>": n * (d64 + 8 + 2 * d64 + d32),
         "k_stencil<float,8,7>#1": res0,
         "k_stencil_pipe<float,8,7,*>#1": res0,
@@ -152,6 +156,8 @@
             agg[key][1] += e.time_range.elapsed_us()
     niter = max(1, len(iters))
     table, shape = finest_bytes(levels, a.prolong_form)
+    if any(k.startswith("k_stencil_res_update<") for k in agg):
+        table = {k: v for k, v in table.items() if not k.startswith(("k_stencil<float,8,7>", "k_stencil_pipe<float,8,7,"))}
     sum_us = sum(v[1] for v in agg.values()) / niter
     rows = {}
     for key, (cnt, us) in sorted(agg.items(), key=lambda kv: -kv[1][1]):
```
